# xinntao/EDVR

Hardware: AMD Instinct MI355X
Metric: EDVR-L x4 5-frame 720p clips/sec (higher is better)
Workload: dtype fp32 emulated as 2xf16 (hi+lo, 22-bit operands, 4 cross products), fp32 accumulate; 1 GPU; EDVR-L x4, 5 frames, 180x320 LR -> 720x1280, batch 10/GPU, inference; clips_per_gpu=10, global_clips=10, parallelism=clip-sharded x1, no data-path collective, world_size=1, backend=single process

## Files before the change

edvr_amd/_lib.py:

```python
import ctypes
import os

_HERE = os.path.dirname(os.path.abspath(__file__))
LIB_PATH = os.environ.get('EDVR_AMD_LIB') or os.path.join(_HERE, 'lib', 'libedvr_amd.so')

c_float_p = ctypes.c_void_p
i32, i64, f32, sz, u32 = ctypes.c_int, ctypes.c_int64, ctypes.c_float, ctypes.c_size_t, ctypes.c_uint32
vp = ctypes.c_void_p


class ConvDesc(ctypes.Structure):
    _fields_ = [
        ('x1', vp), ('x2', vp), ('c1', i32), ('c2', i32), ('x1_img_stride', i64), ('x2_img_stride', i64),
        ('x2_div', i32), ('x2_mul', i32), ('x2_add', i32), ('n', i32), ('h', i32), ('w', i32), ('wpk', vp),
        ('bias', vp), ('co', i32), ('ks', i32), ('stride', i32), ('act', i32), ('act_from', i32), ('res1', vp),
        ('res2', vp), ('res1_img_stride', i64), ('res2_img_stride', i64), ('y', vp), ('y_img_stride', i64),
        ('out_mode', i32), ('algo', i32), ('gate', vp), ('gate_img_stride', i64), ('gate_slope', f32), ('y_scale', f32),
        ('wpk_f4', vp), ('abs_sum', vp), ('abs_sum_channels', i32), ('wpk_f4s', vp), ('x_amax', vp), ('y_amax', vp),
        ('pre', vp), ('pre_img_stride', i64), ('pre_div', i32), ('pre_mul', i32), ('pre_add', i32), ('pre_n', i32), ('wpk_ds', vp),
    ]


PROTOTYPES = {
    'edvr_version': (ctypes.c_char_p, []),
    'edvr_last_error': (ctypes.c_char_p, []),
    'edvr_check_device': (i32, []),
    'edvr_conv2d_packed_weight_elems': (sz, [i32, i32, i32]),
    'edvr_conv2d_pack_weight_f32': (i32, [vp, vp, i32, i32, i32, i32, vp]),
    'edvr_conv2d_packed_weight_f4_elems': (sz, [i32, i32]),
    'edvr_conv2d_pack_weight_f4_f32': (i32, [vp, vp, i32, i32, i32, vp]),
    'edvr_conv2d_packed_weight_f4s_elems': (sz, [i32, i32]),
    'edvr_conv2d_pack_weight_f4s_f32': (i32, [vp, vp, i32, i32, i32, vp]),
    'edvr_conv2d_packed_weight_1x1s_elems': (sz, [i32, i32]),
    'edvr_conv2d_pack_weight_1x1s_f32': (i32, [vp, vp, i32, i32, vp]),
    'edvr_conv2d_packed_weight_ds_elems': (sz, [i32, i32, i32]),
    'edvr_conv2d_pack_weight_ds_f32': (i32, [vp, vp, i32, i32, i32, vp]),
    'edvr_amax_f32': (i32, [vp, vp, i32, i64, i64, vp]),
    'edvr_pack_job_bytes': (sz, []),
    'edvr_conv2d_pack_weights_multi': (i32, [vp, i32, i32, i32, vp]),
    'edvr_conv2d_f32': (i32, [ctypes.POINTER(ConvDesc), vp]),
    'edvr_conv2d_kernel': (i32, [ctypes.POINTER(ConvDesc)]),
    'edvr_conv2d_gate_supported': (i32, [ctypes.POINTER(ConvDesc)]),
    'edvr_conv2d_abs_sum_supported': (i32, [ctypes.POINTER(ConvDesc)]),
    'edvr_conv2d_y_amax_supported': (i32, [ctypes.POINTER(ConvDesc)]),
    'edvr_conv2d_pre_supported': (i32, [ctypes.POINTER(ConvDesc)]),
    'edvr_conv2d_f4s_set_lean': (i32, [i32]),
    'edvr_conv2d_f4s_lean_items': (i32, [ctypes.POINTER(ConvDesc)]),
    'edvr_conv2d_kernel_name': (i32, [ctypes.POINTER(ConvDesc), ctypes.c_char_p, sz]),
    'edvr_conv2d_executed_flops': (i32, [ctypes.POINTER(ConvDesc), ctypes.POINTER(ctypes.c_double)]),
    'edvr_dcnv2_fwd_ws_bytes': (sz, [i32] * 12),
    'edvr_dcnv2_fwd_f32': (i32, [vp] * 6 + [i32] * 12 + [i64, i64, i32, i32, vp, sz, vp]),
    'edvr_dcnv2_fwd_split_f32': (i32, [vp] * 6 + [i32] * 12 + [i64, i64, i32, i32, vp, sz, vp, vp]),
    'edvr_dcnv2_fwd_split_applies': (i32, [vp] + [i32] * 13),
    'edvr_dcnv2_fwd_kernel_name': (i32, [vp] + [i32] * 13 + [ctypes.c_char_p, sz]),
    'edvr_dcnv2_bwd_ws_bytes': (sz, [i32] * 12),
    'edvr_dcnv2_any_ws_bytes': (sz, [i32] * 13),
    'edvr_dcnv2_fwd_any': (i32, [i32] + [vp] * 6 + [i32] * 12 + [i64, i64, vp, sz, vp]),
    'edvr_dcnv2_bwd_any': (i32, [i32] + [vp] * 10 + [i32] * 12 + [i64, i64, i64, i64, vp, sz, vp]),
    'edvr_psnr_sse_f32': (i32, [vp, vp, vp, i32, i32, i32, i32, i64, i64, i32, i32, i32, vp]),
    'edvr_ssim_partials': (sz, [i32, i32, i32]),
    'edvr_ssim_f32': (i32, [vp, vp, vp, i32, i32, i32, i32, i64, i64, i32, i32, vp]),
    'edvr_niqe_blocks': (sz, [i32, i32, i32]),
    'edvr_niqe_moments_f32': (i32, [vp, vp, i32, i32, i32, i32, i64, i32, vp]),
    'edvr_niqe_moments_u8': (i32, [vp, vp, i32, i32, i32, i64, i32, vp]),
    'edvr_frames_u8_to_f32': (i32, [vp, vp, i32, i32, i32, i32, vp, i32, vp]),
    'edvr_gather_images_f32': (i32, [vp, vp, vp, vp, i32, vp, i32, i32, vp]),
    'edvr_upsample4x_add_u8': (i32, [vp, vp, vp, i32, i32, i32, vp]),
    'edvr_f32_to_u8_hwc': (i32, [vp, vp, i32, i32, i32, i64, vp]),
    'edvr_crop_pad_frames_u8': (i32, [vp, vp, i32, i32, i32, i32, i32, i32, i32, i32, vp]),
    'edvr_crop_pad_frames_f32': (i32, [vp, vp, i32, i32, i32, i64, i32, i32, i32, i32, i32, vp]),
    'edvr_upsample4x_add_rect_f32': (i32, [vp, vp, vp, i32, i32, i32, i32, i32, i32, i32, i64, i64, i64, vp]),
    'edvr_upsample4x_add_rect_u8': (i32, [vp, vp, vp, i32, i32, i32, i32, i32, i32, i32, i64, i64, vp]),
    'edvr_f32_to_u8_hwc_rect': (i32, [vp, vp, i32, i32, i32, i64, i32, i32, i32, i32, i64, i64, vp]),
    'edvr_copy_rect_f32': (i32, [vp, vp, i32, i32, i32, i64, i32, i32, i32, i32, i64, i64, i64, vp]),
    'edvr_crop_pad_frames_d4_u8': (i32, [vp, vp, i32, i32, i32, i32, i32, i32, i32, i32, i32, vp]),
    'edvr_crop_pad_frames_d4_f32': (i32, [vp, vp, i32, i32, i32, i64, i32, i32, i32, i32, i32, i32, vp]),
    'edvr_upsample4x_add_rect_d4_f32': (i32, [vp, vp, vp, i32, i32, i32, i32, i32, i32, i32, i64, i64, i64, i32, i32, f32, vp]),
    'edvr_upsample4x_add_rect_d4_u8': (i32, [vp, vp, vp, vp, i32, i32, i32, i32, i32, i32, i32, i64, i64, i64, i64, i64, i32, i32, f32, vp]),
    'edvr_f32_to_u8_hwc_rect_d4': (i32, [vp, vp, vp, i32, i32, i32, i64, i32, i32, i32, i32, i64, i64, i64, i64, i64, i32, i32, f32, vp]),
    'edvr_copy_rect_d4_f32': (i32, [vp, vp, i32, i32, i32, i64, i32, i32, i32, i32, i64, i64, i64, i32, i32, f32, vp]),
    'edvr_upsample4x_add_rect_blend_f32': (i32, [vp, vp, vp, i32, i32, i32, i32, i32, i32, i32, i64, i64, i64, i32, i32, f32, i32, i32, i32, i32, vp]),
    'edvr_upsample4x_add_rect_blend_u8': (i32, [vp, vp, vp, vp, i32, i32, i32, i32, i32, i32, i32, i64, i64, i64, i64, i64, i32, i32, f32, i32, i32, i32, i32, vp]),
    'edvr_f32_to_u8_hwc_rect_blend': (i32, [vp, vp, vp, i32, i32, i32, i64, i32, i32, i32, i32, i64, i64, i64, i64, i64, i32, i32, f32, i32, i32, i32, i32, vp]),
    'edvr_copy_rect_blend_f32': (i32, [vp, vp, i32, i32, i32, i64, i32, i32, i32, i32, i64, i64, i64, i32, i32, f32, i32, i32, i32, i32, vp]),
    'edvr_imresize_bicubic_u8': (i32, [vp, vp, i32, i32, i32, i32, i32, ctypes.c_double, i32, i32, vp]),
    'edvr_imresize_bicubic_f32': (i32, [vp, vp, i32, i32, i32, i64, i32, i32, ctypes.c_double, i32, i32, vp]),
    'edvr_bd_downsample_u8': (i32, [vp, vp, i32, i32, i32, i32, i32, i32, i32, vp]),
    'edvr_bd_downsample_f32': (i32, [vp, vp, i32, i32, i32, i64, i32, i32, i32, i32, vp]),
    'edvr_imresize_bicubic_u8_windows': (i32, [vp, vp, vp, vp, i32, i32, i32, i32, i32, i32, vp]),
    'edvr_bd_downsample_u8_windows': (i32, [vp, vp, vp, vp, i32, i32, i32, i32, i32, i32, vp]),
    'edvr_yuv420_to_rgb_f32': (i32, [vp, vp, i32, i32, i32, i64, i64, vp, i32, vp]),
    'edvr_yuv420_to_rgb_u8': (i32, [vp, vp, i32, i32, i32, i64, vp, i32, vp]),
    'edvr_rgb_to_yuv420_f32': (i32, [vp, vp, i32, i32, i32, i64, i64, vp, vp]),
    'edvr_rgb_to_yuv420_u8': (i32, [vp, vp, i32, i32, i32, i64, vp, vp]),
    'edvr_yuv_to_rgb_f32': (i32, [vp, vp, i32, i32, i32, i32, i32, i32, i64, i64, vp, i32, vp]),
    'edvr_rgb_to_yuv_f32': (i32, [vp, vp, i32, i32, i32, i32, i32, i32, i64, i64, vp, vp]),
    'edvr_yuv_to_rgb_sited_f32': (i32, [vp, vp, i32, i32, i32, i32, i32, i32, i64, i64, vp, i32, i32, i32, vp]),
    'edvr_rgb_to_yuv_sited_f32': (i32, [vp, vp, i32, i32, i32, i32, i32, i32, i64, i64, vp, i32, i32, vp]),
    'edvr_yuv420_to_rgb_sited_u8': (i32, [vp, vp, i32, i32, i32, i64, vp, i32, i32, i32, vp]),
    'edvr_rgb_to_yuv420_sited_u8': (i32, [vp, vp, i32, i32, i32, i64, vp, i32, i32, vp]),
    'edvr_frame_sad_rgb_u8': (i32, [vp, vp, vp, i32, i32, i32, i64, vp]),
    'edvr_frame_sad_rgb_f32': (i32, [vp, vp, vp, i32, i32, i32, i64, vp]),
    'edvr_jpeg_roundtrip_u8': (i32, [vp, vp, vp, i32, i32, i32, i32, i64, i64, i32, vp]),
    'edvr_mpeg_roundtrip_workspace': (sz, [i32, i32, i32, i32]),
    'edvr_mpeg_roundtrip_u8': (i32, [vp, vp, vp, i32, i32, i32, i32, i32, i64, i64, i64, i64, i32, i32, vp, sz, vp]),
    'edvr_degrade_u8': (i32, [vp, vp, vp, vp, i32, i32, i32, i64, i64, vp]),
    'edvr_philox_words_u32': (i32, [vp, u32, u32, u32, i32, i32, vp]),
    'edvr_adam_chunk_bytes': (sz, []),
    'edvr_adam_multi_f32': (i32, [vp, i32, ctypes.c_float, ctypes.c_float, ctypes.c_float, vp]),
    'edvr_dcnv1_fwd_ws_bytes': (sz, [i32] * 12),
    'edvr_dcnv1_fwd_f32': (i32, [vp] * 4 + [i32] * 12 + [i64, i32, vp, sz, vp]),
    'edvr_dcnv1_bwd_ws_bytes': (sz, [i32] * 12),
    'edvr_dcnv1_bwd_f32': (i32, [vp] * 7 + [i32] * 12 + [i64, i64, i32, vp, sz, vp]),
    'edvr_dcnv2_bwd_f32': (i32, [vp] * 10 + [i32] * 12 + [i64, i64, i64, i64, i32, vp, sz, vp]),
    'edvr_dcnv2_bwd_split_f32': (i32, [vp] * 10 + [i32] * 12 + [i64, i64, i64, i64, i32, vp, sz, vp, vp, vp]),
    'edvr_dcnv2_bwd_split_applies': (i32, []),
    'edvr_tsa_temporal_f32': (i32, [vp] * 5 + [i32] * 4 + [vp]),
    'edvr_tsa_temporal_pair_f32': (i32, [vp] * 5 + [i32] * 4 + [vp]),
    'edvr_pool_maxavg_3x3s2_f32': (i32, [vp, vp, i32, i32, i32, i32, vp]),
    'edvr_upsample2x_f32': (i32, [vp, vp, i32, i32, i32, f32, vp]),
    'edvr_tsa_combine_f32': (i32, [vp, vp, vp, vp, i64, vp]),
    'edvr_upsample4x_add_f32': (i32, [vp, vp, i32, i32, i32, vp]),
    'edvr_add_f32': (i32, [vp, vp, vp, i64, vp]),
    'edvr_act_bwd_f32': (i32, [vp, vp, vp, vp, vp, i32, i32, i64, i32, i32, vp]),
    'edvr_conv2d_wgrad_ws_bytes': (sz, [i32] * 7),
    'edvr_conv2d_wgrad_algo': (i32, [i32]),
    'edvr_conv2d_wgrad_kernel_name': (i32, [i32] * 8 + [ctypes.c_char_p, sz]),
    'edvr_conv2d_wgrad_f32': (i32, [vp] * 4 + [i32] * 8 + [i64, i64, i32, i32, i32, i64, i32, vp, vp, sz, vp]),
    'edvr_conv2d_wgrad_split_f32': (i32, [vp] * 4 + [i32] * 8 + [i64, i64, i32, i32, i32, i64, i32, vp, vp, sz, vp, vp, vp]),
    'edvr_conv2d_wgrad_split_applies': (i32, [i32] * 8),
    'edvr_conv2d_wgrad_split_is_direct': (i32, [i32] * 2),
    'edvr_channel_sum_f32': (i32, [vp, vp, i32, i32, i64, i64, vp, sz, vp]),
    'edvr_pixel_unshuffle2_f32': (i32, [vp, vp, i32, i32, i32, i32, vp]),
    'edvr_pixel_unshuffle2_act_bwd_f32': (i32, [vp, vp, vp, i32, i32, i32, i32, i32, vp]),
    'edvr_zero_stuff2_f32': (i32, [vp, vp, i32, i32, i32, i32, i32, vp]),
    'edvr_frame_reduce_add_f32': (i32, [vp, vp, i32, i32, i32, i64, vp]),
    'edvr_upsample2x_bwd_f32': (i32, [vp, vp, i32, i32, i32, f32, vp]),
    'edvr_pool_maxavg_3x3s2_bwd_f32': (i32, [vp, vp, vp, i32, i32, i32, i32, vp]),
    'edvr_tsa_temporal_bwd_f32': (i32, [vp] * 7 + [i32] * 4 + [vp, vp]),
    'edvr_tsa_combine_bwd_f32': (i32, [vp] * 5 + [i64, vp]),
    'edvr_charbonnier_f32': (i32, [vp, vp, vp, vp, i64, f32, f32, vp]),
    'edvr_abs_sum_f32': (i32, [vp, vp, i32, i64, i64, vp]),
    'edvr_abs_stats_f32': (i32, [vp, vp, i32, i64, i32, i64, vp]),
}

ACT_NONE, ACT_RELU, ACT_LRELU, ACT_SIGMOID = 0, 1, 2, 3
OUT_NCHW, OUT_PIXEL_SHUFFLE2 = 0, 1
CONV_AUTO, CONV_DIRECT, CONV_WINOGRAD, CONV_WINOGRAD_F4, CONV_WINOGRAD_F4S = 0, 1, 2, 3, 4
(CONV_KERNEL_SMALL, CONV_KERNEL_F4S, CONV_KERNEL_F4, CONV_KERNEL_F2, CONV_KERNEL_1X1_SPLIT, CONV_KERNEL_1X1_STREAM,
 CONV_KERNEL_DIRECT_SPLIT, CONV_KERNEL_DIRECT) = range(8)
DTYPE_F32, DTYPE_F64, DTYPE_F16 = 0, 1, 2
DCN_HALO_TAPWIN = 16
JPEG_SUBSAMPLINGS = {'420': 420, '444': 444}
DEGRADE_TILE, DEGRADE_MAX_KSIZE, DEGRADE_RECORD_INTS, DEGRADE_GRAY = 64, 21, 8, 1

_lib = None


class ExtensionMissing(RuntimeError):
    pass


def lib():
    global _lib
    if _lib is None:
        if not os.path.exists(LIB_PATH):
            raise ExtensionMissing(
                f'{LIB_PATH} not found: the HIP extension is not built (run `python -m edvr_amd.build`). '
                'edvr_amd has no CPU/PyTorch fallback.')
        handle = ctypes.CDLL(LIB_PATH)
        for name, (res, args) in PROTOTYPES.items():
            fn = getattr(handle, name)
            fn.restype, fn.argtypes = res, args
        _lib = handle
    return _lib


def check(rc, what):
    if rc != 0:
        msg = lib().edvr_last_error().decode()
        raise RuntimeError(f'{what} failed (code {rc}): {msg}')
```

edvr_amd/build.py:

```python
import os
import shutil
import subprocess
import sys
from concurrent.futures import ThreadPoolExecutor

HERE = os.path.dirname(os.path.abspath(__file__))
CSRC = os.path.join(HERE, 'csrc')
LIBDIR = os.path.join(HERE, 'lib')
LIB = os.path.join(LIBDIR, 'libedvr_amd.so')
OBJDIR = os.path.join(HERE, 'build')
SOURCES = ['api.hip', 'pack.hip', 'conv2d.hip', 'conv2d_s.hip', 'dcn.hip', 'dcn_any.hip', 'elementwise.hip', 'wgrad.hip', 'backward.hip', 'dcn_fused.hip', 'dcn_tapwin.hip', 'dcn_tapwin_s.hip', 'dcn_bwd_fused.hip', 'winograd.hip', 'winograd_f4.hip', 'winograd_f4s.hip', 'winograd_wgrad.hip', 'winograd_wgrad_s.hip', 'wgrad_direct_s.hip', 'gemm_nt_s.hip', 'optim.hip', 'metrics.hip', 'conv_small.hip', 'conv1x1.hip', 'conv1x1_s.hip', 'data.hip', 'video.hip', 'resize.hip', 'bd.hip', 'ensemble.hip', 'yuv.hip', 'niqe.hip', 'shots.hip', 'jpeg.hip', 'degrade.hip', 'mpeg.hip']
LINK = []
FLAGS = ['--offload-arch=gfx950', '-O3', '-std=c++17', '-fPIC', '-munsafe-fp-atomics', '-ffp-contract=fast']


def _hipcc():
    exe = shutil.which('hipcc') or '/opt/rocm/bin/hipcc'
    if not os.path.exists(exe):
        raise RuntimeError('hipcc not found: the HIP extension cannot be built')
    return exe


def _deps():
    return [os.path.join(CSRC, 'common.h'), os.path.join(CSRC, 'pack.h'), os.path.join(CSRC, 'conv_launch.h'), os.path.join(CSRC, 'dcn_tap.h'), os.path.join(CSRC, 'pixel.h'), os.path.join(CSRC, 'lq_window.h'), os.path.join(CSRC, 'jpeg_dct.h'), os.path.join(HERE, '..', 'include', 'edvr_amd.h')]


def _stale(target, sources):
    if not os.path.exists(target):
        return True
    t = os.path.getmtime(target)
    return any(os.path.getmtime(s) > t for s in sources)


def source_hash():
    import hashlib
    h = hashlib.sha256()
    files = sorted(os.path.join(CSRC, f) for f in os.listdir(CSRC) if f.endswith(('.hip', '.h', '.inc')))
    for path in files + [os.path.join(HERE, '..', 'include', 'edvr_amd.h')]:
        h.update(os.path.basename(path).encode() + b'\0')
        h.update(open(path, 'rb').read())
    return h.hexdigest()[:16]


def build(force=False, verbose=False):
    os.makedirs(OBJDIR, exist_ok=True)
    os.makedirs(LIBDIR, exist_ok=True)
    hipcc = _hipcc()
    objs, jobs = [], []
    for src in SOURCES:
        s = os.path.join(CSRC, src)
        o = os.path.join(OBJDIR, src.replace('.hip', '.o'))
        objs.append(o)
        if force or _stale(o, [s] + _deps()):
            jobs.append([hipcc] + FLAGS + ['-c', s, '-o', o])

    def run(cmd):
        if verbose:
            print(' '.join(cmd), flush=True)
        r = subprocess.run(cmd, capture_output=True, text=True)
        if r.returncode != 0:
            raise RuntimeError('hipcc failed:\n' + ' '.join(cmd) + '\n' + r.stdout + r.stderr)

    with ThreadPoolExecutor(max_workers=max(1, min(len(jobs), os.cpu_count() or 1))) as ex:
        list(ex.map(run, jobs))
    if force or jobs or _stale(LIB, objs):
        run([hipcc, '--offload-arch=gfx950', '-shared', '-fPIC', '-o', LIB] + objs + LINK)
    return LIB


if __name__ == '__main__':
    print(build(force='--force' in sys.argv, verbose=True))
```

edvr_amd/csrc/common.h:

```cpp
#pragma once
#include <hip/hip_runtime.h>

#include <cstdarg>
#include <cstdio>

#include "../../include/edvr_amd.h"

namespace edvr {

void set_error(const char *fmt, ...);

inline int check_launch(const char *what) {
  hipError_t e = hipGetLastError();
  if (e != hipSuccess) {
    set_error("%s: %s", what, hipGetErrorString(e));
    return EDVR_ERR_LAUNCH;
  }
  return EDVR_OK;
}

inline hipStream_t as_stream(edvr_stream_t s) { return reinterpret_cast<hipStream_t>(s); }

inline int cdiv(int a, int b) { return (a + b - 1) / b; }
inline int64_t cdiv64(int64_t a, int64_t b) { return (a + b - 1) / b; }

int conv2d_launch(const edvr_conv2d_desc &d, hipStream_t stream);
enum conv_kernel {
  CONV_SMALL = EDVR_CONV_KERNEL_SMALL,
  CONV_F4S = EDVR_CONV_KERNEL_F4S,
  CONV_F4 = EDVR_CONV_KERNEL_F4,
  CONV_F2 = EDVR_CONV_KERNEL_F2,
  CONV_1X1_SPLIT = EDVR_CONV_KERNEL_1X1_SPLIT,
  CONV_1X1_STREAM = EDVR_CONV_KERNEL_1X1_STREAM,
  CONV_DIRECT_SPLIT = EDVR_CONV_KERNEL_DIRECT_SPLIT,
  CONV_DIRECT = EDVR_CONV_KERNEL_DIRECT,
};
conv_kernel conv2d_select(const edvr_conv2d_desc &d);

size_t gemm_nt_ws_elems(int M, int N, int64_t K);
int gemm_nt_launch(const float *A, const float *B, float *C, int M, int N, int64_t K, int64_t lda, int64_t ldb,
                   bool accumulate, float *ws, hipStream_t stream);
size_t gemm_nt_ws_elems_b(int M, int N, int64_t K, int nb);
int gemm_nt_batched(const float *A, const float *B, float *C, int M, int N, int64_t K, int64_t lda, int64_t ldb, int nb, int64_t a_bs,
                    int64_t b_bs, bool accumulate, float *ws, hipStream_t stream);
bool gemm_nt_split_enabled();
int gemm_nt_split_batched(const float *A, const float *B, float *C, int M, int N, int64_t K, int64_t lda, int64_t ldb, int nb, int64_t a_bs,
                          int64_t b_bs, bool accumulate, float *ws, const float *a_amax, const float *b_amax, hipStream_t stream);

bool winograd_eligible(const edvr_conv2d_desc &d);
int winograd_launch(const edvr_conv2d_desc &d, const float *U, int cop64, hipStream_t stream);
double winograd_executed_flops(const edvr_conv2d_desc &d);
int winograd_pack(const float *w, float *U, int co, int ci, int cop64, int cip, int transpose_flip, float *wpk_direct, int cop32,
                  hipStream_t stream);

bool winograd_f4_eligible(const edvr_conv2d_desc &d);
int winograd_f4_launch(const edvr_conv2d_desc &d, hipStream_t stream);
double winograd_f4_executed_flops(const edvr_conv2d_desc &d);

bool winograd_f4s_eligible(const edvr_conv2d_desc &d);
int winograd_f4s_launch(const edvr_conv2d_desc &d, hipStream_t stream);
double winograd_f4s_executed_flops(const edvr_conv2d_desc &d);

bool conv_small_eligible(const edvr_conv2d_desc &d);
int conv_small_launch(const edvr_conv2d_desc &d, hipStream_t stream);
bool wgrad_small_plan(int n, int c1, int c2, int h, int w, int co, int ks, int stride, int *splits);
size_t wgrad_small_ws_bytes(int co, int ci, int splits);
int wgrad_small_launch(const float *x, const float *dz, float *ws, int ci, int co, int n, int h, int w, int64_t x_img_stride,
                       int64_t dz_img_stride, int splits, hipStream_t stream);

bool conv1x1_eligible(const edvr_conv2d_desc &d);
int conv1x1_launch(const edvr_conv2d_desc &d, hipStream_t stream);
bool conv1x1_split_eligible(const edvr_conv2d_desc &d);
int conv1x1_split_launch(const edvr_conv2d_desc &d, hipStream_t stream);

bool conv2d_split_eligible(const edvr_conv2d_desc &d);
int conv2d_split_launch(const edvr_conv2d_desc &d, hipStream_t stream);
int conv_split_pack(const float *w, unsigned *wq, int co, int ci, int kk, int cop, int quads, hipStream_t stream);

int reduce_partials_launch(const float *ws, float *out, int64_t total, int parts, int accumulate, hipStream_t stream,
                           const float *ws2 = nullptr, float *out2 = nullptr, int total2 = 0, int parts2 = 0);

bool winograd_wgrad_plan(int n, int c1, int c2, int h, int w, int co, int ks, int stride, int *splits);
size_t winograd_wgrad_ws_bytes(int co, int ci, int splits);
int winograd_wgrad_set_algo(int algo);
int winograd_wgrad_get_algo();
int winograd_wgrad_launch(const float *x1, const float *x2, const float *dz, float *ws, int c1, int c2, int n, int h, int w, int co,
                          int64_t x1_img_stride, int64_t x2_img_stride, int x2_div, int x2_mul, int x2_add, int64_t dz_img_stride,
                          int splits, int want_db, hipStream_t stream);

bool winograd_wgrad_split_enabled();
int winograd_wgrad_split_launch(const float *x1, const float *x2, const float *dz, float *ws, int c1, int c2, int n, int h, int w, int co,
                                int64_t x1_img_stride, int64_t x2_img_stride, int x2_div, int x2_mul, int x2_add, int64_t dz_img_stride,
                                int splits, int want_db, const float *x_amax, const float *dz_amax, hipStream_t stream);

bool wgrad_direct_split_enabled();
bool wgrad_direct_split_supported(const float *x1, const float *x2, const float *dz, int h, int w, int64_t x1_img_stride, int64_t x2_img_stride,
                                  int64_t dz_img_stride);
int wgrad_direct_split_launch(const float *x1, const float *x2, const float *dz, float *ws, int c1, int c2, int n, int h, int w, int co,
                              int64_t x1_img_stride, int64_t x2_img_stride, int x2_div, int x2_mul, int x2_add, int64_t dz_img_stride,
                              int splits, int want_db, const float *x_amax, const float *dz_amax, hipStream_t stream);

struct DcnShape {
  int B, C, H, W, Co, kh, kw, stride, pad, dil, groups, dg, Ho, Wo;
  int stride_w, pad_w, dil_w;
  int64_t off_bs, msk_bs;
  int64_t doff_bs, dmsk_bs;
};
int dcn_fill_shape(DcnShape &s, int B, int C, int H, int W, int Co, int kh, int kw, int stride, int pad, int dil, int groups, int dg,
                   int64_t off_bs, int64_t msk_bs);

bool dcn_fused_supported(int C, int Co, int H, int W, int kh, int kw, int stride, int pad, int dil, int groups, int dg);
int dcn_fused_pack(const float *weight, float *wpk, int Co, int C, hipStream_t stream);
int dcn_fused_forward(const float *x, const float *offset, const float *mask, const float *wpk, const float *bias, float *y, int B, int C,
                      int H, int W, int Co, int dg, int64_t off_bs, int64_t msk_bs, int act, int halo, hipStream_t stream);

bool dcn_tapwin_supported(int C, int Co, int H, int W, int kh, int kw, int stride, int pad, int dil, int groups, int dg);
int dcn_tapwin_forward(const float *x, const float *offset, const float *mask, const float *wpk, const float *bias, float *y, int B, int C,
                       int H, int W, int Co, int dg, int64_t off_bs, int64_t msk_bs, int act, hipStream_t stream);

bool dcn_tapwin_split_enabled();
int dcn_tapwin_split_forward(const float *x, const float *offset, const float *mask, const float *weight, unsigned *wpk, const float *bias, float *y,
                             int B, int C, int H, int W, int Co, int dg, int64_t off_bs, int64_t msk_bs, int act, const float *xm_amax,
                             hipStream_t stream);

bool dcn_bwd_fused_supported(const DcnShape &s);
size_t dcn_bwd_fused_wbk_elems(int dg);
int dcn_bwd_fused_launch(const DcnShape &s, const float *x, const float *offset, const float *mask, const float *weight, const float *dy,
                         float *wbk, float *col, float *dx, float *doffset, float *dmask, hipStream_t stream);

__device__ inline int xcd_remap(int linear, int total) {
  const int q = total >> 3, rem = total & 7, xcd = linear & 7;
  return xcd * q + (xcd < rem ? xcd : rem) + (linear >> 3);
}
__device__ inline void xcd_block_index(int &bx, int &by, int &bz) {
  const int gx = gridDim.x, gy = gridDim.y;
  const int lin = blockIdx.x + gx * (blockIdx.y + gy * blockIdx.z);
  const int lg = xcd_remap(lin, gx * gy * (int)gridDim.z);
  bx = lg % gx;
  by = (lg / gx) % gy;
  bz = lg / (gx * gy);
}

}

#define EDVR_REQUIRE(cond, ...)       \
  do {                                \
    if (!(cond)) {                    \
      ::edvr::set_error(__VA_ARGS__); \
      return EDVR_ERR_ARG;            \
    }                                 \
  } while (0)
```

edvr_amd/csrc/dcn.hip:

```cpp
#include <cstdlib>

#include "common.h"
#include "dcn_tap.h"

namespace edvr {

typedef float f32x16 __attribute__((ext_vector_type(16)));

__global__ void fill_kernel(float *__restrict__ p, float v, int64_t n) {
  for (int64_t i = (int64_t)blockIdx.x * blockDim.x + threadIdx.x; i < n; i += (int64_t)gridDim.x * blockDim.x) p[i] = v;
}

struct Merge {
  bool give01, give11;
  bool take00, take10;
};
__device__ __forceinline__ Merge merge_right(const Tap &t, bool same_plane_as_next) {
  Merge mg;
  const int lane = __lane_id();
  const int n_o00 = lane_next_i(t.o00), n_o10 = lane_next_i(t.o10);
  const int n_ok = lane_next_i((t.ok00 ? 1 : 0) | (t.ok10 ? 2 : 0));
  const bool has_next = lane < 63 && same_plane_as_next;
  mg.give01 = has_next && t.ok01 && (n_ok & 1) && n_o00 == t.o01;
  mg.give11 = has_next && t.ok11 && (n_ok & 2) && n_o10 == t.o11;
// ... 515 lines not shown
  EDVR_REQUIRE(s.Ho > 0 && s.Wo > 0, "dcnv2: convolution input is too small (output would be %dx%d)", s.Ho, s.Wo);
  const int64_t P = (int64_t)s.Ho * s.Wo, K = kh * kw;
  s.off_bs = off_bs ? off_bs : (int64_t)dg * 2 * K * P;
  s.msk_bs = msk_bs < 0 ? 0 : (msk_bs ? msk_bs : (int64_t)dg * K * P);
  s.doff_bs = (int64_t)dg * 2 * K * P;
  s.dmsk_bs = (int64_t)dg * K * P;
  return EDVR_OK;
}

static bool use_fused(const DcnShape &s) {
  const char *e = getenv("EDVR_DCN_FUSED");
  if (e && e[0] == '0') return false;
  if (s.stride != s.stride_w || s.pad != s.pad_w || s.dil != s.dil_w) return false;
  return dcn_fused_supported(s.C, s.Co, s.H, s.W, s.kh, s.kw, s.stride, s.pad, s.dil, s.groups, s.dg);
}

struct FwdWs { size_t col, wpk, total; };
static FwdWs fwd_ws(const DcnShape &s) {

  const size_t K = (size_t)s.kh * s.kw, P = (size_t)s.Ho * s.Wo;
  FwdWs w;
  w.col = 0;
  size_t off = align_up((size_t)s.B * s.C * K * P * 4, 256);
  w.wpk = off;
  size_t pk = edvr_conv2d_packed_weight_elems(s.Co / s.groups, (int)((s.C / s.groups) * K), 1) * 4 * s.groups;
  if (use_fused(s)) pk = std::max(pk, edvr_conv2d_packed_weight_elems(s.Co, s.C, 3) * 4);
  off += align_up(pk, 256);
  w.total = off;
  return w;
}

struct BwdWs { size_t col, wpk, gemm, total; };
static BwdWs bwd_ws(const DcnShape &s) {
  const size_t K = (size_t)s.kh * s.kw, P = (size_t)s.Ho * s.Wo;
  const int cig = s.C / s.groups, cog = s.Co / s.groups;
  BwdWs w;
  w.col = 0;
  size_t off = align_up((size_t)s.B * s.C * K * P * 4, 256);
  w.wpk = off;
  off += align_up(std::max(edvr_conv2d_packed_weight_elems((int)(cig * K), cog, 1) * s.groups, dcn_bwd_fused_wbk_elems(s.dg)) * 4, 256);
  w.gemm = off;
  off += align_up(std::max(gemm_nt_ws_elems_b(cog, (int)(cig * K), (int64_t)P, s.B), (size_t)s.B * s.Co * cig * K) * 4, 256);
  w.total = off;
  return w;
}

}

extern "C" {

size_t edvr_dcnv2_fwd_ws_bytes(int B, int C, int H, int W, int Co, int kh, int kw, int stride, int pad, int dil, int groups,
                               int dg) {
  edvr::DcnShape s;
  if (edvr::dcn_fill_shape(s, B, C, H, W, Co, kh, kw, stride, pad, dil, groups, dg, 0, 0)) return 0;
  return edvr::fwd_ws(s).total;
}

size_t edvr_dcnv2_bwd_ws_bytes(int B, int C, int H, int W, int Co, int kh, int kw, int stride, int pad, int dil, int groups,
                               int dg) {
  edvr::DcnShape s;
  if (edvr::dcn_fill_shape(s, B, C, H, W, Co, kh, kw, stride, pad, dil, groups, dg, 0, 0)) return 0;
  return edvr::bwd_ws(s).total;
}

static int dcnv2_fwd_impl(const float *x, const float *offset, const float *mask, const float *weight, const float *bias,
                          float *y, int B, int C, int H, int W, int Co, int kh, int kw, int stride, int pad, int dil, int groups,
                          int dg, int64_t offset_bstride, int64_t mask_bstride, int act, int halo_hint, void *ws, size_t ws_bytes,
                          const float *xm_amax, edvr_stream_t stream_) {
  using namespace edvr;
  EDVR_REQUIRE(x && offset && mask && weight && y, "dcnv2_fwd: null pointer");
  DcnShape s;
  int rc = dcn_fill_shape(s, B, C, H, W, Co, kh, kw, stride, pad, dil, groups, dg, offset_bstride, mask_bstride);
  if (rc) return rc;
  const FwdWs wsz = fwd_ws(s);
  if (!ws || ws_bytes < wsz.total) {
    set_error("dcnv2_fwd: workspace %zu < required %zu", ws_bytes, wsz.total);
    return EDVR_ERR_WORKSPACE;
  }
  hipStream_t stream = as_stream(stream_);
  const int K = kh * kw;
  const int64_t P = (int64_t)s.Ho * s.Wo;
  float *col = reinterpret_cast<float *>(static_cast<char *>(ws) + wsz.col);
  float *wpk = reinterpret_cast<float *>(static_cast<char *>(ws) + wsz.wpk);
  if (use_fused(s) && halo_hint == EDVR_DCN_HALO_TAPWIN && xm_amax && dcn_tapwin_split_enabled() &&
      dcn_tapwin_supported(C, Co, H, W, kh, kw, s.stride, s.pad, s.dil, groups, dg) && (reinterpret_cast<uintptr_t>(x) & 15) == 0)
    return dcn_tapwin_split_forward(x, offset, mask, weight, reinterpret_cast<unsigned *>(wpk), bias, y, B, C, H, W, Co, dg, s.off_bs, s.msk_bs, act,
                                    xm_amax, stream);
  if (use_fused(s) && halo_hint >= 0) {
    rc = dcn_fused_pack(weight, wpk, Co, C, stream);
    if (rc) return rc;
    if (halo_hint == EDVR_DCN_HALO_TAPWIN) {
      if (dcn_tapwin_supported(C, Co, H, W, kh, kw, s.stride, s.pad, s.dil, groups, dg) && (reinterpret_cast<uintptr_t>(x) & 15) == 0)
        return dcn_tapwin_forward(x, offset, mask, wpk, bias, y, B, C, H, W, Co, dg, s.off_bs, s.msk_bs, act, stream);
      halo_hint = 7;
    }
    return dcn_fused_forward(x, offset, mask, wpk, bias, y, B, C, H, W, Co, dg, s.off_bs, s.msk_bs, act, halo_hint, stream);
  }
  const int cig = C / groups, cog = Co / groups;
  const size_t wpk_g = edvr_conv2d_packed_weight_elems(cog, cig * K, 1);
  for (int g = 0; g < groups; ++g) {
    rc = edvr_conv2d_pack_weight_f32(weight + (size_t)g * cog * cig * K, wpk + g * wpk_g, cog, cig * K, 1, 0, stream_);
    if (rc) return rc;
  }
  const int64_t total = (int64_t)B * dg * K * P;
  hipLaunchKernelGGL(dcn_im2col_kernel, dim3((unsigned)std::min<int64_t>(cdiv64(total, 256), 1 << 20)), dim3(256), 0, stream, x,
                     offset, mask, col, s);
  rc = check_launch("dcn_im2col_kernel");
  if (rc) return rc;
  for (int g = 0; g < groups; ++g) {
    edvr_conv2d_desc d = {};
    d.x1 = col + (int64_t)g * cig * K * P;
    d.c1 = cig * K;
    d.x1_img_stride = (int64_t)C * K * P;
    d.n = B; d.h = s.Ho; d.w = s.Wo;
    d.wpk = wpk + g * wpk_g;
    d.bias = bias ? bias + g * cog : nullptr;
    d.co = cog; d.ks = 1; d.stride = 1;
    d.act = act;
    d.y = y + (int64_t)g * cog * P;
    d.y_img_stride = (int64_t)Co * P;
    d.out_mode = EDVR_OUT_NCHW;
    rc = conv2d_launch(d, stream);
    if (rc) return rc;
  }
  return EDVR_OK;
}

int edvr_dcnv2_fwd_f32(const float *x, const float *offset, const float *mask, const float *weight, const float *bias,
                       float *y, int B, int C, int H, int W, int Co, int kh, int kw, int stride, int pad, int dil, int groups,
                       int dg, int64_t offset_bstride, int64_t mask_bstride, int act, int halo_hint, void *ws, size_t ws_bytes,
                       edvr_stream_t stream) {
  return dcnv2_fwd_impl(x, offset, mask, weight, bias, y, B, C, H, W, Co, kh, kw, stride, pad, dil, groups, dg, offset_bstride, mask_bstride, act,
                        halo_hint, ws, ws_bytes, nullptr, stream);
}

int edvr_dcnv2_fwd_split_f32(const float *x, const float *offset, const float *mask, const float *weight, const float *bias,
                             float *y, int B, int C, int H, int W, int Co, int kh, int kw, int stride, int pad, int dil, int groups,
                             int dg, int64_t offset_bstride, int64_t mask_bstride, int act, int halo_hint, void *ws, size_t ws_bytes,
                             const float *xm_amax, edvr_stream_t stream) {
  EDVR_REQUIRE(xm_amax != nullptr, "dcnv2_fwd_split: null magnitude bound");
  return dcnv2_fwd_impl(x, offset, mask, weight, bias, y, B, C, H, W, Co, kh, kw, stride, pad, dil, groups, dg, offset_bstride, mask_bstride, act,
                        halo_hint, ws, ws_bytes, xm_amax, stream);
}

int edvr_dcnv2_fwd_split_applies(const float *x, int B, int C, int H, int W, int Co, int kh, int kw, int stride, int pad, int dil, int groups,
                                 int dg, int halo_hint) {
  using namespace edvr;
  DcnShape s;
  if (dcn_fill_shape(s, B, C, H, W, Co, kh, kw, stride, pad, dil, groups, dg, 0, 0)) return 0;
  return (use_fused(s) && halo_hint == EDVR_DCN_HALO_TAPWIN && dcn_tapwin_split_enabled() &&
          dcn_tapwin_supported(C, Co, H, W, kh, kw, s.stride, s.pad, s.dil, groups, dg) && (reinterpret_cast<uintptr_t>(x) & 15) == 0) ? 1 : 0;
}

int edvr_dcnv2_fwd_kernel_name(const float *x, int B, int C, int H, int W, int Co, int kh, int kw, int stride, int pad, int dil, int groups,
                               int dg, int halo_hint, char *buf, size_t buf_len) {
  using namespace edvr;
  EDVR_REQUIRE(buf && buf_len > 0, "dcnv2_fwd_kernel_name: null buffer");
  DcnShape s;
  int rc = dcn_fill_shape(s, B, C, H, W, Co, kh, kw, stride, pad, dil, groups, dg, 0, 0);
  if (rc) return rc;
  const char *name = "dcn_im2col_kernel";
  if (use_fused(s) && halo_hint >= 0) {
    const bool tapwin = halo_hint == EDVR_DCN_HALO_TAPWIN && dcn_tapwin_supported(C, Co, H, W, kh, kw, s.stride, s.pad, s.dil, groups, dg) &&
                        (reinterpret_cast<uintptr_t>(x) & 15) == 0;
    name = tapwin ? "dcn_tapwin_fwd_kernel" : "dcn_fused_fwd_kernel";
  }
  snprintf(buf, buf_len, "%s", name);
  return EDVR_OK;
}

static int dcnv2_bwd_impl(const float *x, const float *offset, const float *mask, const float *weight, const float *dy, float *dx,
                          float *doffset, float *dmask, float *dweight, float *dbias, int B, int C, int H, int W, int Co, int kh,
                          int kw, int stride, int pad, int dil, int groups, int dg, int64_t offset_bstride, int64_t mask_bstride,
                          int64_t doffset_bstride, int64_t dmask_bstride, int scatter_hint, void *ws, size_t ws_bytes,
                          const float *xm_amax, const float *dy_amax, edvr_stream_t stream_) {
  using namespace edvr;
  EDVR_REQUIRE(x && offset && mask && weight && dy && dx && doffset && dmask && dweight, "dcnv2_bwd: null pointer");
  DcnShape s;
  int rc = dcn_fill_shape(s, B, C, H, W, Co, kh, kw, stride, pad, dil, groups, dg, offset_bstride, mask_bstride);
  if (rc) return rc;
  if (doffset_bstride) s.doff_bs = doffset_bstride;
  if (dmask_bstride) s.dmsk_bs = dmask_bstride < 0 ? 0 : dmask_bstride;
  const BwdWs wsz = bwd_ws(s);
  if (!ws || ws_bytes < wsz.total) {
    set_error("dcnv2_bwd: workspace %zu < required %zu", ws_bytes, wsz.total);
    return EDVR_ERR_WORKSPACE;
  }
  hipStream_t stream = as_stream(stream_);
  const int K = kh * kw;
  const int64_t P = (int64_t)s.Ho * s.Wo;
  float *col = reinterpret_cast<float *>(static_cast<char *>(ws) + wsz.col);
  float *wpk = reinterpret_cast<float *>(static_cast<char *>(ws) + wsz.wpk);
  float *gws = reinterpret_cast<float *>(static_cast<char *>(ws) + wsz.gemm);
  const int cig = C / groups, cog = Co / groups;
  if (scatter_hint == EDVR_DCN_SCATTER_STRIP && dcn_bwd_fused_supported(s)) {
    if (hipMemsetAsync(dx, 0, (size_t)B * C * H * W * sizeof(float), stream) != hipSuccess) {
      set_error("dcnv2_bwd: hipMemsetAsync failed");
      return EDVR_ERR_LAUNCH;
    }
    rc = dcn_bwd_fused_launch(s, x, offset, mask, weight, dy, wpk, col, dx, doffset, dmask, stream);
    if (rc) return rc;
  } else {
    const size_t wpk_g = edvr_conv2d_packed_weight_elems(cig * K, cog, 1);
    for (int g = 0; g < groups; ++g) {
      const float *wg = weight + (size_t)g * cog * cig * K;
      const float *wuse = wg;
      if ((cog % 32) != 0 || ((cig * K) % 32) != 0) {
        rc = edvr_conv2d_pack_weight_f32(wg, wpk + g * wpk_g, cig * K, cog, 1, 1, stream_);
        if (rc) return rc;
        wuse = wpk + g * wpk_g;
      }
      edvr_conv2d_desc d = {};
      d.x1 = dy + (int64_t)g * cog * P;
      d.c1 = cog;
      d.x1_img_stride = (int64_t)Co * P;
      d.n = B; d.h = s.Ho; d.w = s.Wo;
      d.wpk = wuse;
      d.co = cig * K; d.ks = 1; d.stride = 1;
      d.y = col + (int64_t)g * cig * K * P;
      d.y_img_stride = (int64_t)C * K * P;
      rc = conv2d_launch(d, stream);
      if (rc) return rc;
    }
    if (hipMemsetAsync(dx, 0, (size_t)B * C * H * W * sizeof(float), stream) != hipSuccess) {
      set_error("dcnv2_bwd: hipMemsetAsync failed");
      return EDVR_ERR_LAUNCH;
    }
    static const bool use_tile = []() {
      const char *e = getenv("EDVR_DCN_BWD_TILE");
      return !(e && e[0] == '0');
    }();
    const bool edvr_sig = kh == 3 && kw == 3 && s.stride == 1 && s.pad == 1 && s.dil == 1 && s.stride_w == 1 && s.pad_w == 1 && s.dil_w == 1;
    if (scatter_hint == EDVR_DCN_SCATTER_STRIP && edvr_sig && dg * cdiv(W, 64) <= 65535) {
      hipLaunchKernelGGL(dcn_bwd_dx_strip_kernel, dim3(dg * cdiv(W, 64), B), dim3(256), 0, stream, offset, mask, col, dx, s);
      const int64_t total = (int64_t)B * dg * K * P;
      hipLaunchKernelGGL(dcn_bwd_coord_kernel<false>, dim3((unsigned)std::min<int64_t>(cdiv64(total, 256), 1 << 20)), dim3(256), 0, stream,
                         x, offset, mask, col, static_cast<float *>(nullptr), doffset, dmask, s);
      rc = check_launch("dcn_bwd_dx_strip_kernel + dcn_bwd_coord_kernel");
    } else if (use_tile && scatter_hint != EDVR_DCN_SCATTER_DEVICE && scatter_hint != EDVR_DCN_SCATTER_STRIP && edvr_sig && C / dg <= 16) {
      const int tiles_x = cdiv(s.Wo, 32), tiles_y = cdiv(s.Ho, 8);
      if (scatter_hint == EDVR_DCN_SCATTER_LDS_WIDE)
        hipLaunchKernelGGL((dcn_bwd_coord_tile_kernel<6>), dim3(tiles_x * tiles_y, dg, B), dim3(256), 0, stream, x, offset, mask, col, dx, doffset, dmask, s, tiles_x);
      else
        hipLaunchKernelGGL((dcn_bwd_coord_tile_kernel<3>), dim3(tiles_x * tiles_y, dg, B), dim3(256), 0, stream, x, offset, mask, col, dx, doffset, dmask, s, tiles_x);
      rc = check_launch("dcn_bwd_coord_tile_kernel");
    } else {
      const int64_t total = (int64_t)B * dg * K * P;
      hipLaunchKernelGGL(dcn_bwd_coord_kernel<true>, dim3((unsigned)std::min<int64_t>(cdiv64(total, 256), 1 << 20)), dim3(256), 0, stream, x,
                         offset, mask, col, dx, doffset, dmask, s);
      rc = check_launch("dcn_bwd_coord_kernel");
    }
    if (rc) return rc;
  }
  for (int g = 0; g < groups; ++g) {
    rc = (xm_amax && dy_amax && gemm_nt_split_enabled())
             ? gemm_nt_split_batched(dy + (int64_t)g * cog * P, col + (int64_t)g * cig * K * P, dweight + (size_t)g * cog * cig * K, cog, cig * K,
                                     P, P, P, B, (int64_t)Co * P, (int64_t)C * K * P, false, gws, dy_amax, xm_amax, stream)
             : gemm_nt_batched(dy + (int64_t)g * cog * P, col + (int64_t)g * cig * K * P, dweight + (size_t)g * cog * cig * K, cog, cig * K, P,
                               P, P, B, (int64_t)Co * P, (int64_t)C * K * P, false, gws, stream);
    if (rc) return rc;
  }
  if (dbias) {
    rc = edvr_channel_sum_f32(dy, dbias, B, Co, P, (int64_t)Co * P, gws, (size_t)64 * Co * sizeof(float), stream_);
    if (rc) return rc;
  }
  return EDVR_OK;
}

int edvr_dcnv2_bwd_f32(const float *x, const float *offset, const float *mask, const float *weight, const float *dy, float *dx,
                       float *doffset, float *dmask, float *dweight, float *dbias, int B, int C, int H, int W, int Co, int kh,
                       int kw, int stride, int pad, int dil, int groups, int dg, int64_t offset_bstride, int64_t mask_bstride,
                       int64_t doffset_bstride, int64_t dmask_bstride, int scatter_hint, void *ws, size_t ws_bytes,
                       edvr_stream_t stream) {
  return dcnv2_bwd_impl(x, offset, mask, weight, dy, dx, doffset, dmask, dweight, dbias, B, C, H, W, Co, kh, kw, stride, pad, dil, groups, dg,
                        offset_bstride, mask_bstride, doffset_bstride, dmask_bstride, scatter_hint, ws, ws_bytes, nullptr, nullptr, stream);
}

int edvr_dcnv2_bwd_split_f32(const float *x, const float *offset, const float *mask, const float *weight, const float *dy, float *dx,
                             float *doffset, float *dmask, float *dweight, float *dbias, int B, int C, int H, int W, int Co, int kh,
                             int kw, int stride, int pad, int dil, int groups, int dg, int64_t offset_bstride, int64_t mask_bstride,
                             int64_t doffset_bstride, int64_t dmask_bstride, int scatter_hint, void *ws, size_t ws_bytes,
                             const float *xm_amax, const float *dy_amax, edvr_stream_t stream) {
  EDVR_REQUIRE(xm_amax && dy_amax, "dcnv2_bwd_split: null magnitude bound");
  return dcnv2_bwd_impl(x, offset, mask, weight, dy, dx, doffset, dmask, dweight, dbias, B, C, H, W, Co, kh, kw, stride, pad, dil, groups, dg,
                        offset_bstride, mask_bstride, doffset_bstride, dmask_bstride, scatter_hint, ws, ws_bytes, xm_amax, dy_amax, stream);
}

int edvr_dcnv2_bwd_split_applies(void) { return edvr::gemm_nt_split_enabled() ? 1 : 0; }


size_t edvr_dcnv1_fwd_ws_bytes(int B, int C, int H, int W, int Co, int kh, int kw, int stride, int pad, int dil, int groups, int dg) {
  edvr::DcnShape s;
  if (edvr::dcn_fill_shape(s, B, C, H, W, Co, kh, kw, stride, pad, dil, groups, dg, 0, 0)) return 0;
  return edvr::fwd_ws(s).total + edvr::align_up((size_t)dg * kh * kw * s.Ho * s.Wo * 4, 256);
}

int edvr_dcnv1_fwd_f32(const float *x, const float *offset, const float *weight, float *y, int B, int C, int H, int W, int Co, int kh,
                       int kw, int stride, int pad, int dil, int groups, int dg, int64_t offset_bstride, int halo_hint, void *ws,
                       size_t ws_bytes, edvr_stream_t stream_) {
  using namespace edvr;
  const size_t v2 = edvr_dcnv2_fwd_ws_bytes(B, C, H, W, Co, kh, kw, stride, pad, dil, groups, dg);
  const size_t need = edvr_dcnv1_fwd_ws_bytes(B, C, H, W, Co, kh, kw, stride, pad, dil, groups, dg);
  EDVR_REQUIRE(v2 && need, "dcnv1: bad shape");
  if (!ws || ws_bytes < need) {
    set_error("dcnv1_fwd: workspace %zu < required %zu", ws_bytes, need);
    return EDVR_ERR_WORKSPACE;
// ... 41 lines not shown
```

edvr_amd/csrc/dcn_tapwin_s.hip:

```cpp
#include <type_traits>

#include "common.h"
#include <cstdlib>

#include "dcn_tap.h"
#include "pack.h"

namespace edvr {

typedef float f32x16 __attribute__((ext_vector_type(16)));
typedef float f32x4 __attribute__((ext_vector_type(4)));
typedef float f32x2 __attribute__((ext_vector_type(2)));

namespace {
constexpr int TWS_TH = 8, TWS_TW = 32, TWS_RY = 2, TWS_RX = 2;
constexpr int TWS_IH = TWS_TH + 2 * TWS_RY;
constexpr int TWS_IW = (TWS_TW + 2 * TWS_RX + 3 + 3) / 4 * 4;
constexpr int TWS_PPR = TWS_IW / 4;
constexpr int TWS_HR = TWS_IH / 2;
constexpr int TWS_HB = TWS_HR * TWS_IW;
constexpr int TWS_CHS = TWS_IH * TWS_IW;
static_assert(TWS_HR * TWS_PPR <= 64 && TWS_IH == 2 * TWS_HR && TWS_CHS % 64 == 32, "window halves must fit one wave instruction");
constexpr int TWS_MAX_DG = 8;
constexpr int TWS_OOB = (int)0x80000000;
// ... 287 lines not shown
        for (int s = 0; s < 2; ++s)
#pragma unroll
          for (int m = 0; m < MT; ++m)
            acc[s][m] = __builtin_amdgcn_mfma_f32_32x32x16_f16(__builtin_bit_cast(f16x8, aw[m]), __builtin_bit_cast(f16x8, bq[s]), acc[s][m], 0, 0, 0);
        if (kg == 0 || KG == 1) {
          state_half(nxt, 0, tn, ny0, nx0, tnv);
#pragma unroll
          for (int i = 0; i < 4; ++i) asm volatile("" : "+v"(nxt.bw[0][i]));
          asm volatile("" : "+v"(nxt.addr[0]), "+v"(nxt.slow));
        }
        if (kg == KG - 1) {
          state_half(nxt, 1, tn, ny0, nx0, tnv);
#pragma unroll
          for (int i = 0; i < 4; ++i) asm volatile("" : "+v"(nxt.bw[1][i]));
          asm volatile("" : "+v"(nxt.addr[1]), "+v"(nxt.slow));
          state_any(nxt);
          asm volatile("" : "+s"(nxt.slow_any));
        }
#pragma unroll
        for (int s = 0; s < 2; ++s)
          asm volatile("v_alignbit_b32 %0, %0, %0, 16\n\tv_alignbit_b32 %1, %1, %1, 16\n\tv_alignbit_b32 %2, %2, %2, 16\n\tv_alignbit_b32 %3, %3, %3, 16"
                       : "+v"(bq[s][0]), "+v"(bq[s][1]), "+v"(bq[s][2]), "+v"(bq[s][3]));
#pragma unroll
        for (int s = 0; s < 2; ++s)
#pragma unroll
          for (int m = 0; m < MT; ++m)
            acc[s][m] = __builtin_amdgcn_mfma_f32_32x32x16_f16(__builtin_bit_cast(f16x8, aw[m]), __builtin_bit_cast(f16x8, bq[s]), acc[s][m], 0, 0, 0);
        __builtin_amdgcn_sched_barrier(0);
      }
    }
  };

  __syncthreads();
  const int n_steps = a.dg * KK;
  St cur, nxt;
  float tnv[6];
  int o1y, o1x;
  origin(0, 0, o1y, o1x);
  dma_x(0, 0, o1y, o1x);
  dma_w(0, 0, 0);
  dma_taps(0, 0);
  asm volatile("s_waitcnt vmcnt(0)" ::: "memory");
  read_taps(tnv);
  make_state(cur, 0, o1y, o1x, tnv);
  asm volatile("s_waitcnt lgkmcnt(0)" ::: "memory");
  int g = 0, t = 0, g1 = 0, t1 = 1;
  if (n_steps > 1) {
    origin(g1, t1, o1y, o1x);
    dma_taps(g1, t1);
    asm volatile("s_waitcnt vmcnt(0)" ::: "memory");
  }
  for (int k = 0; k < n_steps; ++k) {
    __syncthreads();
    const int g2 = (t1 == KK - 1) ? g1 + 1 : g1, t2 = (t1 == KK - 1) ? 0 : t1 + 1;
    int o2y = 0, o2x = 0;
    if (k + 1 < n_steps) {
      read_taps(tnv);
      asm volatile("s_waitcnt lgkmcnt(0)" ::: "memory");
      dma_x((k + 1) & 1, g1, o1y, o1x);
      dma_w((k + 1) & 1, g1, t1);
      if (k + 2 < n_steps) {
        origin(g2, t2, o2y, o2x);
        dma_taps(g2, t2);
      }
    }
    const float *xb = xw + (k & 1) * XW;
    const unsigned *wb = wsl + (k & 1) * WS;
    run_step(std::false_type{}, cur, xb, wb, g, t, nxt, t1, o1y, o1x, tnv);
    if (cur.slow_any) run_step(std::true_type{}, cur, xb, wb, g, t, nxt, t1, o1y, o1x, tnv);
    asm volatile("s_waitcnt vmcnt(0)" ::: "memory");
    cur = nxt;
    g = g1; t = t1; g1 = g2; t1 = t2; o1y = o2y; o1x = o2x;
  }

  const __amdgpu_buffer_rsrc_t y_rsrc = tws_rsrc(a.y + (int64_t)img * a.Co * P, a.Co * P * 4);
  const __amdgpu_buffer_rsrc_t b_rsrc = tws_rsrc(a.bias ? a.bias : a.x, a.bias ? a.Co * 4 : 0);
#pragma unroll
  for (int m = 0; m < MT; ++m) {
#pragma unroll
    for (int r4 = 0; r4 < 4; ++r4) {
      const int cob = co_blk + m * 32 + 8 * r4;
      float bias4[4];
#pragma unroll
      for (int r = 0; r < 4; ++r) {
        const bool cok = cob + 4 * half + r < a.Co;
        bias4[r] = a.bias ? __builtin_bit_cast(float, __builtin_amdgcn_raw_buffer_load_b32(b_rsrc, cok ? (4 * half + r) * 4 : OOB, cob * 4, 0)) : 0.f;
      }
#pragma unroll
      for (int s = 0; s < 2; ++s) {
        const bool pix_ok = s ? ok1 : ok0;
        const int pv = (p0 + s * a.W + 4 * half * P) * 4;
#pragma unroll
        for (int r = 0; r < 4; ++r) {
          float v = __builtin_fmaf(acc[s][m][4 * r4 + r], unscale, bias4[r]);
          if (a.act == EDVR_ACT_LRELU) v = v > 0.f ? v : 0.1f * v;
          else if (a.act == EDVR_ACT_RELU) v = fmaxf(v, 0.f);
          else if (a.act == EDVR_ACT_SIGMOID) v = __builtin_amdgcn_rcpf(1.f + __expf(-v));
          const bool cok = cob + 4 * half + r < a.Co;
          __builtin_amdgcn_raw_buffer_store_b32(__builtin_bit_cast(unsigned, v), y_rsrc, (pix_ok && cok) ? pv : OOB, (cob + r) * P * 4, 0);
        }
      }
    }
  }
}

__global__ __launch_bounds__(1024) void dcn_tapwin_split_scale_kernel(const float *__restrict__ w, unsigned *__restrict__ wpk, int64_t total) {
  __shared__ float red[16];
  float m = 0.f;
  for (int64_t i = threadIdx.x; i < total; i += 1024) m = fmaxf(m, fabsf(w[i]));
#pragma unroll
  for (int sh = 32; sh > 0; sh >>= 1) m = fmaxf(m, __shfl_xor(m, sh));
  if ((threadIdx.x & 63) == 0) red[threadIdx.x >> 6] = m;
  __syncthreads();
  if (threadIdx.x == 0) {
    for (int i = 1; i < 16; ++i) m = fmaxf(m, red[i]);
    const unsigned field = f4s_weight_scale_field(__builtin_bit_cast(unsigned, m));
    wpk[0] = field << 23;
    wpk[1] = (254u - field) << 23;
    for (int i = 2; i < 16; ++i) wpk[i] = 0u;
  }
}

__global__ void dcn_tapwin_split_pack_kernel(const float *__restrict__ w, unsigned *__restrict__ wpk, int Co, int C, int cop) {
  const float s_w = __builtin_bit_cast(float, wpk[0]);
  const int64_t total = (int64_t)(C / 4) * 9 * cop;
  const int full = Co / 128, rem_tiles = (Co - full * 128 + 31) / 32;
  for (int64_t i = (int64_t)blockIdx.x * blockDim.x + threadIdx.x; i < total; i += (int64_t)gridDim.x * blockDim.x) {
    const int pos = (int)(i % cop), t = (int)((i / cop) % 9), c4 = (int)(i / ((int64_t)cop * 9));
    const int blk = pos / 128 < full ? pos / 128 : full, start = blk * 128, mt = blk < full ? 4 : rem_tiles;
    const int r = pos - start, co = pos;
    const bool live = mt > 0 && r < 32 * mt && co < Co;
#pragma unroll
    for (int q = 0; q < 4; ++q) wpk[16 + i * 4 + q] = live ? split_f16x2(w[((int64_t)co * C + 8 * (c4 >> 1) + 2 * q + (c4 & 1)) * 9 + t], s_w) : 0u;
  }
}

template <int MT>
static int launch_tapwin_s(DcnTapwinSArgs a, int co_start, int co_blocks, hipStream_t stream) {
  a.co_start = co_start;
  dim3 grid(a.tiles_x * a.tiles_y, co_blocks, a.B);
  if (a.C / a.dg == 16) hipLaunchKernelGGL((dcn_tapwin_split_fwd_kernel<MT, 16>), grid, dim3(256), 0, stream, a);
  else hipLaunchKernelGGL((dcn_tapwin_split_fwd_kernel<MT, 8>), grid, dim3(256), 0, stream, a);
  return check_launch("dcn_tapwin_split_fwd_kernel");
}

bool dcn_tapwin_split_enabled() {
  static const bool on = []() {
    const char *e = getenv("EDVR_DCN_SPLIT");
    return !(e && e[0] == '0');
  }();
  return on;
}

int dcn_tapwin_split_forward(const float *x, const float *offset, const float *mask, const float *weight, unsigned *wpk, const float *bias, float *y,
                             int B, int C, int H, int W, int Co, int dg, int64_t off_bs, int64_t msk_bs, int act, const float *xm_amax,
                             hipStream_t stream) {
  EDVR_REQUIRE(B <= 65535, "dcn_tapwin_split: batch %d exceeds grid.z", B);
  EDVR_REQUIRE((reinterpret_cast<uintptr_t>(x) & 15) == 0 && (reinterpret_cast<uintptr_t>(wpk) & 15) == 0, "dcn_tapwin_split: x / wpk must be 16-byte aligned");
  const int cop = (Co + 31) / 32 * 32;
  hipLaunchKernelGGL(dcn_tapwin_split_scale_kernel, dim3(1), dim3(1024), 0, stream, weight, wpk, (int64_t)Co * C * 9);
  const int64_t total = (int64_t)(C / 4) * 9 * cop;
  hipLaunchKernelGGL(dcn_tapwin_split_pack_kernel, dim3((unsigned)std::min<int64_t>(cdiv64(total, 256), 2048)), dim3(256), 0, stream, weight, wpk, Co, C, cop);
  DcnTapwinSArgs a;
  a.xm_amax = xm_amax;
  a.x = x; a.offset = offset; a.mask = mask; a.wpk = wpk; a.bias = bias; a.y = y;
  a.B = B; a.C = C; a.H = H; a.W = W; a.Co = Co; a.dg = dg; a.act = act;
  a.cop = cop;
  a.off_bs = off_bs; a.msk_bs = msk_bs;
  a.tiles_x = cdiv(W, TWS_TW);
  a.tiles_y = cdiv(H, TWS_TH);
  a.co_start = 0;
  const int full = Co / 128, rem_tiles = cdiv(Co - full * 128, 32);
  int rc = EDVR_OK;
  if (full > 0) rc = launch_tapwin_s<4>(a, 0, full, stream);
  if (rc || rem_tiles == 0) return rc;
  switch (rem_tiles) {
    case 1: return launch_tapwin_s<1>(a, full * 128, 1, stream);
    case 2: return launch_tapwin_s<2>(a, full * 128, 1, stream);
    case 3: return launch_tapwin_s<3>(a, full * 128, 1, stream);
    default: return launch_tapwin_s<4>(a, full * 128, 1, stream);
  }
}

}
```

edvr_amd/edvr_arch.py:

```python
import torch
from torch import nn

from . import functional as F_
from .arch_util import DCNv2Pack, ResidualBlockNoBN, make_layer, warn_offset_absmean

LRELU = F_.ACT_LRELU


def _conv3(cin, cout, stride=1):
    return nn.Conv2d(cin, cout, 3, stride, 1)


class PCDAlignment(nn.Module):

    def __init__(self, num_feat=64, deformable_groups=8):
        super().__init__()
        self.offset_conv1, self.offset_conv2, self.offset_conv3 = nn.ModuleDict(), nn.ModuleDict(), nn.ModuleDict()
        self.dcn_pack, self.feat_conv = nn.ModuleDict(), nn.ModuleDict()
        for lv in (3, 2, 1):
            key = f'l{lv}'
            self.offset_conv1[key] = _conv3(2 * num_feat, num_feat)
            if lv == 3:
                self.offset_conv2[key] = _conv3(num_feat, num_feat)
            else:
                self.offset_conv2[key] = _conv3(2 * num_feat, num_feat)
                self.offset_conv3[key] = _conv3(num_feat, num_feat)
            self.dcn_pack[key] = DCNv2Pack(num_feat, num_feat, 3, padding=1, deformable_groups=deformable_groups)
            if lv < 3:
                self.feat_conv[key] = _conv3(2 * num_feat, num_feat)
        self.cas_offset_conv1 = _conv3(2 * num_feat, num_feat)
        self.cas_offset_conv2 = _conv3(num_feat, num_feat)
        self.cas_dcnpack = DCNv2Pack(num_feat, num_feat, 3, padding=1, deformable_groups=deformable_groups)
        self.upsample = nn.Upsample(scale_factor=2, mode='bilinear', align_corners=False)
        self.lrelu = nn.LeakyReLU(negative_slope=0.1, inplace=True)

    def dcn_modules(self):
        return [self.dcn_pack['l3'], self.dcn_pack['l2'], self.dcn_pack['l1'], self.cas_dcnpack]

    def align(self, nbr, ref, ref_map=None):
        up_off = up_feat = feat = None
        for lv in (3, 2, 1):
            key, x = f'l{lv}', nbr[lv - 1]
            off = F_.conv_shared_x2(self.offset_conv1[key], x, ref[lv - 1], ref_map, act=LRELU)
            if lv == 3:
                off = F_.conv(self.offset_conv2[key], off, act=LRELU)
            else:
                off = F_.conv(self.offset_conv2[key], off, x2=up_off, act=LRELU)
                off = F_.conv(self.offset_conv3[key], off, act=LRELU)
            feat = self.dcn_pack[key](x, off, act=LRELU if lv == 3 else F_.ACT_NONE)
            if lv < 3:
                feat = F_.conv(self.feat_conv[key], feat, x2=up_feat, act=LRELU if lv > 1 else F_.ACT_NONE)
            if lv > 1:
                up_off = F_.upsample2x(off, 2.0)
                up_feat = F_.upsample2x(feat)
        off = F_.conv_shared_x2(self.cas_offset_conv1, feat, ref[0], ref_map, act=LRELU)
        off = F_.conv(self.cas_offset_conv2, off, act=LRELU)
        return self.cas_dcnpack(feat, off, act=LRELU)

    def forward(self, nbr_feat_l, ref_feat_l):
        return self.align(nbr_feat_l, ref_feat_l)


class TSAFusion(nn.Module):

    def __init__(self, num_feat=64, num_frame=5, center_frame_idx=2):
        super().__init__()
        self.center_frame_idx = center_frame_idx
        self.temporal_attn1 = _conv3(num_feat, num_feat)
        self.temporal_attn2 = _conv3(num_feat, num_feat)
        self.feat_fusion = nn.Conv2d(num_frame * num_feat, num_feat, 1, 1)
        self.max_pool = nn.MaxPool2d(3, stride=2, padding=1)
        self.avg_pool = nn.AvgPool2d(3, stride=2, padding=1)
        self.spatial_attn1 = nn.Conv2d(num_frame * num_feat, num_feat, 1)
        self.spatial_attn2 = nn.Conv2d(num_feat * 2, num_feat, 1)
        self.spatial_attn3 = _conv3(num_feat, num_feat)
        self.spatial_attn4 = nn.Conv2d(num_feat, num_feat, 1)
        self.spatial_attn5 = _conv3(num_feat, num_feat)
        self.spatial_attn_l1 = nn.Conv2d(num_feat, num_feat, 1)
        self.spatial_attn_l2 = _conv3(num_feat * 2, num_feat)
        self.spatial_attn_l3 = _conv3(num_feat, num_feat)
        self.spatial_attn_add1 = nn.Conv2d(num_feat, num_feat, 1)
        self.spatial_attn_add2 = nn.Conv2d(num_feat, num_feat, 1)
        self.lrelu = nn.LeakyReLU(negative_slope=0.1, inplace=True)
        self.upsample = nn.Upsample(scale_factor=2, mode='bilinear', align_corners=False)

    def forward(self, aligned_feat):
        return self.spatial(self.temporal(aligned_feat))

    def temporal(self, aligned_feat, pair=False):
        b, t, c, h, w = aligned_feat.shape
        alias = F_.ops.carry_bound
        emb_ref = F_.conv(self.temporal_attn1, alias(aligned_feat[:, self.center_frame_idx], aligned_feat))
        emb = F_.conv(self.temporal_attn2, alias(aligned_feat.reshape(b * t, c, h, w), aligned_feat)).view(b, t, -1, h, w)
        if pair:
            mod, mod_rev = F_.tsa_temporal_pair(emb, emb_ref, aligned_feat)
            return alias(mod.view(b, t * c, h, w), mod), alias(mod_rev.view(b, t * c, h, w), mod_rev)
        mod = F_.tsa_temporal(emb, emb_ref, aligned_feat)
        return alias(mod.view(b, t * c, h, w), mod)

    def spatial(self, mod):
        feat = F_.conv(self.feat_fusion, mod, act=LRELU)
        attn = F_.conv(self.spatial_attn1, mod, act=LRELU)
        attn = F_.conv(self.spatial_attn2, F_.pool_maxavg(attn), act=LRELU)
        lvl = F_.conv(self.spatial_attn_l1, attn, act=LRELU)
        lvl = F_.conv(self.spatial_attn_l2, F_.pool_maxavg(lvl), act=LRELU)
        lvl = F_.upsample2x(F_.conv(self.spatial_attn_l3, lvl, act=LRELU))
        attn = F_.conv(self.spatial_attn3, attn, act=LRELU, res1=lvl)
        attn = F_.upsample2x(F_.conv(self.spatial_attn4, attn, act=LRELU))
        attn = F_.conv(self.spatial_attn5, attn)
        attn_add = F_.conv(self.spatial_attn_add2, F_.conv(self.spatial_attn_add1, attn, act=LRELU))
        return F_.tsa_combine(feat, attn, attn_add)


class PredeblurModule(nn.Module):

    def __init__(self, num_in_ch=3, num_feat=64, hr_in=False):
        super().__init__()
        self.hr_in = hr_in
        self.conv_first = _conv3(num_in_ch, num_feat)
        if hr_in:
            self.stride_conv_hr1 = _conv3(num_feat, num_feat, 2)
            self.stride_conv_hr2 = _conv3(num_feat, num_feat, 2)
        self.stride_conv_l2 = _conv3(num_feat, num_feat, 2)
        self.stride_conv_l3 = _conv3(num_feat, num_feat, 2)
        self.resblock_l3 = ResidualBlockNoBN(num_feat=num_feat)
        self.resblock_l2_1 = ResidualBlockNoBN(num_feat=num_feat)
        self.resblock_l2_2 = ResidualBlockNoBN(num_feat=num_feat)
        self.resblock_l1 = nn.ModuleList([ResidualBlockNoBN(num_feat=num_feat) for _ in range(5)])
        self.upsample = nn.Upsample(scale_factor=2, mode='bilinear', align_corners=False)
        self.lrelu = nn.LeakyReLU(negative_slope=0.1, inplace=True)

    def forward(self, x):
        f1 = F_.conv(self.conv_first, x, act=LRELU)
        if self.hr_in:
            f1 = F_.conv(self.stride_conv_hr2, F_.conv(self.stride_conv_hr1, f1, act=LRELU), act=LRELU)
        f2 = F_.conv(self.stride_conv_l2, f1, act=LRELU)
        f3 = F_.conv(self.stride_conv_l3, f2, act=LRELU)
        f3 = F_.upsample2x(self.resblock_l3(f3))
        rb = self.resblock_l2_1
        f2 = F_.conv(rb.conv2, F_.conv(rb.conv1, f2, act=F_.ACT_RELU), res1=f2, res2=f3)
        f2 = F_.upsample2x(self.resblock_l2_2(f2))
        f1 = self.resblock_l1[0](f1)
        rb = self.resblock_l1[1]
        f1 = F_.conv(rb.conv2, F_.conv(rb.conv1, f1, act=F_.ACT_RELU), res1=f1, res2=f2)
        for i in range(2, 5):
            f1 = self.resblock_l1[i](f1)
        return f1


class EDVR(nn.Module):

    def __init__(self, num_in_ch=3, num_out_ch=3, num_feat=64, num_frame=5, deformable_groups=8, num_extract_block=5,
                 num_reconstruct_block=10, center_frame_idx=2, hr_in=False, with_predeblur=False, with_tsa=True):
        super().__init__()
        self.center_frame_idx = num_frame // 2 if center_frame_idx is None else center_frame_idx
        self.hr_in, self.with_predeblur, self.with_tsa = hr_in, with_predeblur, with_tsa
        if with_predeblur:
            self.predeblur = PredeblurModule(num_feat=num_feat, hr_in=hr_in)
            self.conv_1x1 = nn.Conv2d(num_feat, num_feat, 1, 1)
        else:
            self.conv_first = _conv3(num_in_ch, num_feat)
        self.feature_extraction = make_layer(ResidualBlockNoBN, num_extract_block, num_feat=num_feat)
        self.conv_l2_1 = _conv3(num_feat, num_feat, 2)
        self.conv_l2_2 = _conv3(num_feat, num_feat)
        self.conv_l3_1 = _conv3(num_feat, num_feat, 2)
        self.conv_l3_2 = _conv3(num_feat, num_feat)
        self.pcd_align = PCDAlignment(num_feat=num_feat, deformable_groups=deformable_groups)
        if with_tsa:
            self.fusion = TSAFusion(num_feat=num_feat, num_frame=num_frame, center_frame_idx=self.center_frame_idx)
        else:
            self.fusion = nn.Conv2d(num_frame * num_feat, num_feat, 1, 1)
        self.reconstruction = make_layer(ResidualBlockNoBN, num_reconstruct_block, num_feat=num_feat)
        self.upconv1 = _conv3(num_feat, num_feat * 4)
        self.upconv2 = _conv3(num_feat, 64 * 4)
        self.pixel_shuffle = nn.PixelShuffle(2)
        self.conv_hr = _conv3(64, 64)
        self.conv_last = _conv3(64, 3)
        self.lrelu = nn.LeakyReLU(negative_slope=0.1, inplace=True)
        self.taps = None
        self._conv_weights = None
        self._conv_meta = None
        self._captured_offset_stats = None

    _PENDING = __import__('weakref').WeakKeyDictionary()

    @property
    def _pending_offset_stats(self):
        q = EDVR._PENDING.get(self)
        if q is None:
            q = EDVR._PENDING[self] = []
        return q

    def train(self, mode=True):
        self.check_offsets(wait=True)
        return super().train(mode)

    def forward(self, x):
        b, t, c, h, w = x.shape
        if self.hr_in:
            assert h % 16 == 0 and w % 16 == 0, 'The height and width must be multiple of 16.'
        else:
            assert h % 4 == 0 and w % 4 == 0, 'The height and width must be multiple of 4.'
        x = x.contiguous()
        ctr = self.center_frame_idx
        self.check_offsets(wait=False)
        if x.is_cuda:
            F_.ops.split_guard_check(wait=False)
        if torch.is_grad_enabled() and x.is_cuda:
            if self._conv_weights is None:
                convs = [m for m in self.modules() if isinstance(m, nn.Conv2d)]
                self._conv_weights = [m.weight for m in convs]
                first = self.predeblur.conv_first if self.with_predeblur else self.conv_first
                self._conv_meta = [(m.stride[0] == 1, m is not first) for m in convs]
            F_.ops.prepack_conv_weights(self._conv_weights, self._conv_meta)
        pyr = self.extract_features(x.view(b * t, c, h, w))
        return self.restore_from_features(pyr, x[:, ctr], b, t)

    def extract_features(self, frames, out=None):
        if F_.ops.F4S_INFERENCE or F_.ops.F4S_TRAINING:
            F_.ops.input_bound(frames)
        o1, o2, o3 = out if out is not None else (None, None, None)
        blocks = list(self.feature_extraction) if out is not None else []
        head = None if blocks else o1
        if self.with_predeblur:
            f1 = F_.conv(self.conv_1x1, self.predeblur(frames), out=head)
        else:
            f1 = F_.conv(self.conv_first, frames, act=LRELU, out=head)
        if out is None:
            f1 = self.feature_extraction(f1)
        else:
            for i, blk in enumerate(blocks):
                f1 = blk(f1, out=o1 if i == len(blocks) - 1 else None)
        f2 = F_.conv(self.conv_l2_2, F_.conv(self.conv_l2_1, f1, act=LRELU), act=LRELU, out=o2)
        f3 = F_.conv(self.conv_l3_2, F_.conv(self.conv_l3_1, f2, act=LRELU), act=LRELU, out=o3)
        return [f1, f2, f3]

    def restore_from_features(self, pyr, x_center, b, t, out_dtype=torch.float32, out=None, keep=None, elem=None, accumulate='only', scale=1.0,
                              acc=None, bands=None):
        self._check_tail_args(out_dtype, out, keep, elem, accumulate, scale, acc, bands)
        operand, sink = self.align_windows(pyr, b, t)
        return self._restore_aligned(operand, x_center, b, t, out_dtype, out, keep, elem, accumulate, scale, acc, bands, sink)

    def align_windows(self, pyr, b, t, pair=False):
        f1, f2, f3 = pyr
        ctr = self.center_frame_idx
        h, w = f1.shape[2], f1.shape[3]
        if pair and 2 * ctr != t - 1:
            raise ValueError(f'align_windows(pair=True): the reversed clip keeps its centre only when it is the middle frame, got {ctr} of {t}')
        sink = []
        dcns = self.pcd_align.dcn_modules()
        for m in dcns:
            m.stats_sink = sink
        try:
            aligned = self.pcd_align.align([f1, f2, f3], [f1, f2, f3], ref_map=(t, t, ctr))
        finally:
            for m in dcns:
                m.stats_sink = None
        flat = aligned
        aligned = F_.ops.carry_bound(aligned.view(b, t, -1, h, w), aligned)
        if self.taps is not None:
            self.taps['aligned'] = aligned
        if self.with_tsa:
            operand = self.fusion.temporal(aligned, pair=pair)
            return (*operand, sink) if pair else (operand, sink)
        operand = F_.ops.carry_bound(aligned.view(b, -1, h, w), aligned)
        if not pair:
            return operand, sink
        if torch.is_grad_enabled():
            raise RuntimeError('align_windows(pair=True) has no backward: call it under torch.no_grad()')
        table = torch.arange(b * t, dtype=torch.int32, device=flat.device).view(b, t).flip(1).reshape(-1)
        rev = F_.ops.gather_images([flat], table)[0]
        return operand, F_.ops.carry_bound(rev.view(b, -1, h, w), rev), sink

    def restore_from_aligned(self, operand, x_center, b, t, out_dtype=torch.float32, out=None, keep=None, elem=None, accumulate='only', scale=1.0,
                             acc=None, bands=None, sink=None):
        self._check_tail_args(out_dtype, out, keep, elem, accumulate, scale, acc, bands)
        return self._restore_aligned(operand, x_center, b, t, out_dtype, out, keep, elem, accumulate, scale, acc, bands, sink)

    @staticmethod
    def _check_tail_args(out_dtype, out, keep, elem, accumulate, scale, acc, bands):
        if out_dtype not in (torch.float32, torch.uint8):
            raise ValueError(f'out_dtype must be torch.float32 or torch.uint8, got {out_dtype}')
        if out_dtype == torch.uint8 and torch.is_grad_enabled():
            raise RuntimeError('the uint8 output of EDVR.restore_from_features has no backward: call it under torch.no_grad()')
        if out is None and keep is not None:
            raise ValueError('keep= names a rectangle of the result to store into out=: it needs out')
        if out is not None and torch.is_grad_enabled():
            raise RuntimeError('EDVR.restore_from_features(out=) writes in place and has no backward: call it under torch.no_grad()')
        if elem is None and (accumulate != 'only' or scale != 1.0 or (acc is not None and bands is None)):
            raise ValueError('accumulate=, scale= and acc= belong to a self-ensemble element: they need elem')
        if (elem is not None or bands is not None) and (out is None or (out_dtype == torch.uint8) != (acc is not None)):
            raise ValueError('elem= and bands= store into out= (and, with uint8 output, accumulate in acc=)')

    def _restore_aligned(self, operand, x_center, b, t, out_dtype, out, keep, elem, accumulate, scale, acc, bands, sink):
        dst = out
        taps = self.taps
        feat = self.fusion.spatial(operand) if self.with_tsa else F_.conv(self.fusion, operand)
        if taps is not None:
            taps['fused'] = feat
        out = self.reconstruction(feat)
        if taps is not None:
            taps['trunk'] = out
        out = F_.conv(self.upconv1, out, act=LRELU, out_mode=F_.OUT_PIXEL_SHUFFLE2)
        out = F_.conv(self.upconv2, out, act=LRELU, out_mode=F_.OUT_PIXEL_SHUFFLE2)
        out = F_.conv(self.conv_hr, out, act=LRELU)
        if dst is not None:
            ky, kx = keep if keep is not None else (0, 0)
            if bands is not None:
                how = dict(bands=bands, elem=0 if elem is None else elem, mode=accumulate, scale=scale)
                if self.hr_in:
                    last = F_.conv(self.conv_last, out, res1=x_center)
                    out = (F_.ops.f32_to_u8_hwc_rect_blend(last, dst, acc, ky, kx, **how) if acc is not None
                           else F_.ops.copy_rect_blend(last, dst, ky, kx, **how))
                else:
                    last = F_.conv(self.conv_last, out)
                    out = (F_.ops.upsample4x_add_u8_rect_blend(last, x_center, dst, acc, ky, kx, **how) if acc is not None
                           else F_.ops.upsample4x_add_rect_blend(last, x_center, dst, ky, kx, **how))
            elif elem is not None:
                how = dict(elem=elem, mode=accumulate, scale=scale)
                if self.hr_in:
                    last = F_.conv(self.conv_last, out, res1=x_center)
                    out = F_.ops.f32_to_u8_hwc_rect_d4(last, dst, acc, ky, kx, **how) if acc is not None else F_.ops.copy_rect_d4(last, dst, ky, kx, **how)
                else:
                    last = F_.conv(self.conv_last, out)
                    out = (F_.ops.upsample4x_add_u8_rect_d4(last, x_center, dst, acc, ky, kx, **how) if acc is not None
                           else F_.ops.upsample4x_add_rect_d4(last, x_center, dst, ky, kx, **how))
            elif self.hr_in:
                tail = F_.ops.f32_to_u8_hwc_rect if out_dtype == torch.uint8 else F_.ops.copy_rect
                out = tail(F_.conv(self.conv_last, out, res1=x_center), dst, ky, kx)
            else:
                tail = F_.ops.upsample4x_add_u8_rect if out_dtype == torch.uint8 else F_.ops.upsample4x_add_rect
                out = tail(F_.conv(self.conv_last, out), x_center, dst, ky, kx)
        elif self.hr_in:
            out = F_.conv(self.conv_last, out, res1=x_center)
            if out_dtype == torch.uint8:
                out = F_.ops.f32_to_u8_hwc(out)
        elif out_dtype == torch.uint8:
            out = F_.ops.upsample4x_add_u8(F_.conv(self.conv_last, out), x_center)
        else:
            out = F_.upsample4x_add(F_.conv(self.conv_last, out), x_center)
        if sink:
            self._queue_offset_check(sink, b, t)
        F_.ops.split_guard_submit(operand.device)
        return out

    def _queue_offset_check(self, sink, b, t):
        if not sink:
            return
        import torch
        sums = torch.stack([e[0] for e in sink]).view(len(sink), 2, b, t).sum(2)
        recs = [(per_img * b, module) for _, per_img, module in sink]
        if torch.cuda.is_current_stream_capturing():
            self._captured_offset_stats = (sums, recs)
            return
        if torch.is_grad_enabled() and F_.ops.HINT_WAIT:
            self._examine_offsets(sums.cpu(), recs)
            return
        host = torch.empty(sums.shape, dtype=sums.dtype, pin_memory=True)
        host.copy_(sums, non_blocking=True)
        done = torch.cuda.Event()
        done.record()
        self._pending_offset_stats.append((host, done, recs))
        if len(self._pending_offset_stats) > 64:
            self.check_offsets(wait=True)

    def check_offsets(self, wait=True):
        while self._pending_offset_stats:
            host, done, recs = self._pending_offset_stats[0]
            if wait:
                done.synchronize()
            elif not done.query():
                return
            self._pending_offset_stats.pop(0)
            self._examine_offsets(host, recs)

    @staticmethod
    def _examine_offsets(sums, recs):
        for li, (count, module) in enumerate(recs):
            per_frame = (sums[li, 0] / count).tolist()
            module.last_offset_absmean = sum(per_frame) / len(per_frame)
            rough = float(sums[li, 1].sum())
            module.last_offset_rough = rough / (0.75 * count * len(per_frame)) if rough >= 0 else None
            for v in per_frame:
                warn_offset_absmean(v)
```

edvr_amd/functional.py:

```python
import math
import os

import torch

from . import ops
from .ops import ACT_LRELU, ACT_NONE, ACT_RELU, ACT_SIGMOID, OUT_NCHW, OUT_PIXEL_SHUFFLE2


def _conv_geometry(m):
    ks, st = m.kernel_size, m.stride
    if (ks[0] != ks[1] or ks[0] not in (1, 3) or st[0] != st[1] or st[0] not in (1, 2) or (ks[0] == 1 and st[0] != 1)
            or tuple(m.padding) != (ks[0] // 2, ks[0] // 2) or tuple(m.dilation) != (1, 1) or m.groups != 1):
        raise NotImplementedError(
            f'edvr_amd conv kernel supports 3x3 (stride 1/2, pad 1) and 1x1 convolutions, dilation 1, groups 1; got {m}')
    return ks[0], st[0]


def _needs_grad(*ts):
    return torch.is_grad_enabled() and any(t is not None and t.requires_grad for t in ts)


def conv(m, x, *, x2=None, x2_map=None, act=ACT_NONE, act_from=0, res1=None, res2=None, out_mode=OUT_NCHW, y_scale=1.0,
         abs_sum_channels=0, ci_range=None, use_bias=True, pre=None, pre_map=None, out=None):
    ks, stride = _conv_geometry(m)
    if x.dim() != 4:
        raise ValueError(f'expected a 4-D input, got {tuple(x.shape)}')
    cin = x.shape[1] + (x2.shape[1] if x2 is not None else 0)
    want = m.in_channels if ci_range is None else ci_range[1] - ci_range[0]
    if cin != want:
        raise RuntimeError(f'expected {want} input channels, got {cin}')
    ops.require_gpu(x, x2, m.weight)
    if _needs_grad(x, x2, m.weight, m.bias, res1, res2, pre):
        from . import autograd as ag
        assert abs_sum_channels == 0
        if ci_range is not None or not use_bias or pre is not None or out is not None:
            raise NotImplementedError('ci_range / use_bias / pre / out are inference-only arguments of conv()')
        return ag.conv(m, x, x2, x2_map, act, act_from, res1, res2, out_mode, ks, stride, y_scale)
    wpk = ops.pack_conv_weight(m.weight, ci_range=ci_range)
    f4 = ops.F4_INFERENCE and ks == 3 and stride == 1 and cin >= 32 and m.out_channels >= 48
    f4s = f4 and ops.F4S_INFERENCE and x.shape[3] % 4 == 0
    wf4 = ops.pack_conv_weight(m.weight, f4=True, ci_range=ci_range) if (f4 and not f4s) else None
    wf4s = ops.pack_conv_weight(m.weight, f4s=True, ci_range=ci_range) if f4s else None
    if ops.F4S_INFERENCE and ks == 1 and stride == 1 and cin >= 320 and x.shape[1] % 8 == 0 and cin % 8 == 0:
        wf4s = ops.pack_conv_weight(m.weight, f4s=True, ci_range=ci_range)
    wds = None
    if ops.F4S_INFERENCE and m.out_channels > 4 and (x2 is None or x.shape[1] % 4 == 0) and (
            (ks == 3 and (stride == 2 or cin <= 8)) or (ks == 1 and cin < 320)):
        wds = ops.pack_conv_weight(m.weight, ds=True, ci_range=ci_range)
    bias = m.bias.detach() if (m.bias is not None and use_bias) else None
    r = ops.conv2d(x, wpk, bias, m.out_channels, ks, x2=x2, x2_map=x2_map, stride=stride, act=act, act_from=act_from,
                   res1=res1, res2=res2, out_mode=out_mode, y_scale=y_scale, wpk_f4=wf4, abs_sum_channels=abs_sum_channels,
                   wpk_f4s=wf4s, pre=pre, pre_map=pre_map, out=out, wpk_ds=wds)
    y = r[0] if abs_sum_channels > 0 else r
    if ops.F4S_INFERENCE and ops.get_bound(y) is None:
        ops.linear_bound(y, m.weight, m.bias, (x, x2), (res1, res2, pre), scale=y_scale, floor=1.0 if act == ACT_SIGMOID else 0.0)
    return r


PRE_SPLIT = os.environ.get('EDVR_CONV_PRE', '1') != '0'
PRE_SPLIT_MIN_ITEMS = None


def _conv_items(n, h, w, co):
    return n * -(-co // 64) * min(-(-w // 64) * -(-h // 8), -(-w // 32) * -(-h // 16))


def conv_shared_x2(m, x, x2, x2_map, act=ACT_NONE):
    if PRE_SPLIT and x2_map is not None and x2_map[0] > 1 and not _needs_grad(x, x2, m.weight, m.bias):
        ks, stride = _conv_geometry(m)
        (n, c1, h, w), c2, co = x.shape, x2.shape[1], m.out_channels
        f4 = ops.F4_INFERENCE and ks == 3 and stride == 1 and min(c1, c2) >= 32 and co >= 48
        min_items = PRE_SPLIT_MIN_ITEMS if PRE_SPLIT_MIN_ITEMS is not None else torch.cuda.get_device_properties(x.device).multi_processor_count
        if f4 and _conv_items(n, h, w, co) > min_items and ops.conv_pre_supported(n, c1, h, w, co, ops.F4S_INFERENCE and w % 4 == 0):
            div, mul, add = x2_map
            shared = (n - 1) // div + 1
            sel = x2[add:add + 1] if (mul == 0 or shared == 1) else x2[add:add + (shared - 1) * mul + 1:mul]
            p = conv(m, ops.carry_bound(sel, x2), ci_range=(c1, c1 + c2), use_bias=False)
            return conv(m, x, act=act, ci_range=(0, c1), pre=p, pre_map=(div, 0 if sel.shape[0] == 1 else 1, 0))
    return conv(m, x, x2=x2, x2_map=x2_map, act=act)


def offset_mask_conv_stats(conv_offset, feat):
    co = conv_offset.out_channels
    if _needs_grad(feat, conv_offset.weight, conv_offset.bias):
        om = offset_mask_conv(conv_offset, feat)
        return om, ops.abs_stats_per_image(om.detach()[:, :2 * co // 3])
    return conv(conv_offset, feat, act=ACT_SIGMOID, act_from=2 * co // 3, abs_sum_channels=2 * co // 3)


def offset_mask_conv(conv_offset, feat):
    co = conv_offset.out_channels
    return conv(conv_offset, feat, act=ACT_SIGMOID, act_from=2 * co // 3)


def tapwin_takes(x, m):
    c, w, dg = x.shape[1], x.shape[3], m.deformable_groups
    return (w % 4 == 0 and w >= 32 and dg <= 8 and c % dg == 0 and c // dg in (8, 16) and tuple(m.kernel_size) == (3, 3)
            and _one(m.stride) == 1 and _one(m.padding) == 1 and _one(m.dilation) == 1 and m.groups == 1)


def _one(v):
    return v if isinstance(v, int) else (v[0] if v[0] == v[1] else -1)


def halo_hint_from_stats(absmean, rough, tapwin_ok=True):
    if absmean is not None and not math.isfinite(absmean):
        absmean = None
    if rough is not None and not math.isfinite(rough):
        rough = None
    if not tapwin_ok:
        return 3 if (absmean is None or absmean < 1.2) else (7 if absmean < 3.0 else -1)
    if absmean is None:
        return ops.DCN_HALO_TAPWIN
    if rough is None:
        return 3 if absmean < 1.2 else (7 if absmean < 3.0 else -1)
    if rough >= 0.85 and absmean < 2.0:
        return 7
    if rough >= 40.0 and absmean >= 30.0:
        return -1
    return ops.DCN_HALO_TAPWIN


def halo_hint_from_absmean(absmean):
    return halo_hint_from_stats(absmean, None)


def scatter_hint_from_stats(absmean, rough):
    if absmean is None:
        return ops.DCN_SCATTER_LDS
    if absmean >= 4.0:
        return ops.DCN_SCATTER_LDS_WIDE
    if absmean < 0.4:
        return ops.DCN_SCATTER_STRIP
    if rough is not None and rough < 0.45:
        return ops.DCN_SCATTER_STRIP if absmean < 0.6 else ops.DCN_SCATTER_LDS
    return ops.DCN_SCATTER_DEVICE if absmean < 0.75 else ops.DCN_SCATTER_LDS


def scatter_hint_from_absmean(absmean):
    return scatter_hint_from_stats(absmean, None)


def dcn_from_packed(m, x, om, act=ACT_NONE):
    cfg = (m.stride, m.padding, m.dilation, m.groups, m.deformable_groups)
    hint = halo_hint_from_stats(getattr(m, 'last_offset_absmean', None), getattr(m, 'last_offset_rough', None), tapwin_takes(x, m))
    if _needs_grad(x, om, m.weight, m.bias):
        from . import autograd as ag
        return ag.DcnFromPackedFn.apply(x, om, m.weight, m.bias, (*cfg, act, hint, m))
    split = 2 * om.shape[1] // 3
    bias = m.bias.detach() if m.bias is not None else None
    xb = ops.input_bound(x) if (ops.F4S_INFERENCE and hint == ops.DCN_HALO_TAPWIN and tapwin_takes(x, m)) else None
    y = ops.dcnv2_forward(x, om[:, :split], om[:, split:], m.weight.detach(), bias, *cfg, act=act, halo_hint=hint, xm_bound=xb)
    if ops.F4S_INFERENCE:
        ops.linear_bound(y, m.weight, m.bias, (x,))
    return y


def upsample2x(x, scale=1.0):
    if _needs_grad(x):
        from . import autograd as ag
        return ag.Upsample2x.apply(x, scale)
    return ops.upsample2x(x, scale)


def pool_maxavg(x):
    if _needs_grad(x):
        from . import autograd as ag
        return ag.PoolMaxAvg.apply(x)
    return ops.pool_maxavg(x)


def tsa_temporal(emb, emb_ref, aligned):
    if _needs_grad(emb, emb_ref, aligned):
        from . import autograd as ag
        return ag.TsaTemporal.apply(emb, emb_ref, aligned)
    return ops.tsa_temporal(emb, emb_ref, aligned)


def tsa_temporal_pair(emb, emb_ref, aligned):
    if torch.is_grad_enabled():
        raise RuntimeError('tsa_temporal_pair has no backward: call it under torch.no_grad()')
    return ops.tsa_temporal_pair(emb, emb_ref, aligned)


def tsa_combine(feat, attn, attn_add):
    if _needs_grad(feat, attn, attn_add):
        from . import autograd as ag
        return ag.TsaCombine.apply(feat, attn, attn_add)
    return ops.tsa_combine(feat, attn, attn_add)


def add(a, b):
    if _needs_grad(a, b):
        from . import autograd as ag
        return ag.Add.apply(a, b)
    return ops.add(a, b)


def upsample4x_add(y, base):
    if _needs_grad(y, base):
        from . import autograd as ag
        return ag.Upsample4xAdd.apply(y, base)
    return ops.upsample4x_add_(y, base)
```

edvr_amd/ops.py:

```python
import ctypes
import os
import weakref

import torch

from . import _lib
from ._lib import (ACT_LRELU, ACT_NONE, ACT_RELU, ACT_SIGMOID, CONV_AUTO, CONV_DIRECT, CONV_WINOGRAD, CONV_WINOGRAD_F4, CONV_WINOGRAD_F4S, OUT_NCHW,
                   OUT_PIXEL_SHUFFLE2)


def _stream():
    return ctypes.c_void_p(torch.cuda.current_stream().cuda_stream)


def _ptr(t):
    return ctypes.c_void_p(t.data_ptr()) if t is not None else ctypes.c_void_p(0)


def require_gpu(*tensors, dtypes=(torch.float32,)):
    seen = None
    for t in tensors:
        if t is None:
            continue
        if not t.is_cuda:
            raise NotImplementedError('edvr_amd ops run on the GPU only (HIP/gfx950); got a CPU tensor')
        if t.dtype not in dtypes:
            raise NotImplementedError(f'edvr_amd: {t.dtype} is not supported here (supported: {", ".join(map(str, dtypes))})')
        if seen is not None and t.dtype != seen:
            raise RuntimeError(f'expected every tensor of the call to be {seen}, got {t.dtype}')
        seen = t.dtype
    return seen


DCN_DTYPES = {torch.float32: _lib.DTYPE_F32, torch.float64: _lib.DTYPE_F64, torch.float16: _lib.DTYPE_F16}


def _plane_contig(t):
    n, c, h, w = t.shape
    return t.stride(3) == 1 and t.stride(2) == w and t.stride(1) == h * w and (n == 1 or t.stride(0) >= c * h * w)


def _as_planes(t):
    return t if _plane_contig(t) else t.contiguous()


def _img_stride(t):
    return t.stride(0) if t.shape[0] > 1 else t.shape[1] * t.shape[2] * t.shape[3]


def _run(name, launch, flops=0.0, nbytes=0.0, executed=None):
    if LAUNCH_HOOK is not None:
        LAUNCH_HOOK(name, float(flops), launch, float(nbytes), executed)
    else:
        launch()


def _nb(*ts):
    return 4.0 * sum(t.numel() for t in ts if t is not None)


_WS = {}


def workspace(nbytes, device, tag=None):
    key = (device.index, torch.cuda.current_stream(device).cuda_stream) if tag is None else (device.index, torch.cuda.current_stream(device).cuda_stream, tag)
    buf = _WS.get(key)
    if buf is None or buf.numel() < nbytes:
        buf = None
        _WS.pop(key, None)
        buf = torch.empty(max(int(nbytes), 1), dtype=torch.uint8, device=device)
        _WS[key] = buf
    return buf


_PACKED = {}


def pack_conv_weight(weight, transpose_flip=False, f4=False, f4s=False, ci_range=None, ds=False):
    require_gpu(weight)
    assert not (ds and (f4 or f4s or transpose_flip)), 'ds is a layout of its own, of the forward orientation'
    key, wid, ver = (bool(transpose_flip), 3 if ds else (2 if f4s else bool(f4))), id(weight), weight._version
    if ci_range is not None:
        assert not transpose_flip, 'input-channel ranges serve forward convs'
        key = key + ((int(ci_range[0]), int(ci_range[1])),)
    ent = _PACKED.get(wid)
    if ent is not None and ent[0]() is weight:
        hit = ent[1].get(key)
        if hit is not None and hit[0] == ver and hit[2] == weight.data_ptr():
            return hit[1]
    else:
        ent = (weakref.ref(weight, lambda _r, wid=wid: _PACKED.pop(wid, None)), {})
        _PACKED[wid] = ent
    L = _lib.lib()
    w = weight.detach()
    if ci_range is not None:
        w = w[:, ci_range[0]:ci_range[1]]
    if not w.is_contiguous():
        w = w.contiguous()
    o, i, k, k2 = w.shape
    assert k == k2, 'square kernels only'
    co, ci = (i, o) if transpose_flip else (o, i)
    if ds:
        out = torch.empty(L.edvr_conv2d_packed_weight_ds_elems(co, ci, k), dtype=torch.int32, device=w.device)
        _lib.check(L.edvr_conv2d_pack_weight_ds_f32(_ptr(w), _ptr(out), co, ci, k, _stream()), 'edvr_conv2d_pack_weight_ds_f32')
    elif f4s and k == 1:
        assert not transpose_flip, 'the split 1x1 kernel serves forward convs'
        n_el = L.edvr_conv2d_packed_weight_1x1s_elems(co, ci)
        stale = ent[1].get(key)
        if stale is not None and stale[1].numel() == n_el and stale[1].device == w.device and _sole_owner(stale):
            out = stale[1]
        else:
            out = torch.empty(n_el, dtype=torch.int32, device=w.device)
        _lib.check(L.edvr_conv2d_pack_weight_1x1s_f32(_ptr(w), _ptr(out), co, ci, _stream()), 'edvr_conv2d_pack_weight_1x1s_f32')
    elif f4s:
        assert k == 3, 'F(4x4,3x3) weights are for 3x3 kernels'
        out = torch.empty(L.edvr_conv2d_packed_weight_f4s_elems(co, ci), dtype=torch.int32, device=w.device)
        _lib.check(L.edvr_conv2d_pack_weight_f4s_f32(_ptr(w), _ptr(out), co, ci, 1 if transpose_flip else 0, _stream()),
                   'edvr_conv2d_pack_weight_f4s_f32')
    elif f4:
        assert k == 3, 'F(4x4,3x3) weights are for 3x3 kernels'
        out = torch.empty(L.edvr_conv2d_packed_weight_f4_elems(co, ci), dtype=torch.float32, device=w.device)
        _lib.check(L.edvr_conv2d_pack_weight_f4_f32(_ptr(w), _ptr(out), co, ci, 1 if transpose_flip else 0, _stream()),
                   'edvr_conv2d_pack_weight_f4_f32')
    else:
        out = torch.empty(L.edvr_conv2d_packed_weight_elems(co, ci, k), dtype=torch.float32, device=w.device)
        _lib.check(L.edvr_conv2d_pack_weight_f32(_ptr(w), _ptr(out), co, ci, k, 1 if transpose_flip else 0, _stream()),
                   'edvr_conv2d_pack_weight_f32')
    ent[1][key] = (ver, out, weight.data_ptr())
    return out


_PACK_CALLS = 0
_PACK_TABLES = {}


_PINNED_PACKED = set()


def pin_packed_weights(weights):
    bufs = []
    for w in weights:
        ent = _PACKED.get(id(w))
        if ent is not None and ent[0]() is w:
            bufs.extend(hit[1] for hit in ent[1].values())
    _PINNED_PACKED.update(b.data_ptr() for b in bufs)
    return bufs


def unpin_packed_weights(bufs):
    for b in bufs:
        _PINNED_PACKED.discard(b.data_ptr())


def _sole_owner(hit):
    import sys
    return hit[1]._use_count() == 1 and sys.getrefcount(hit[1]) == 2 and hit[1].data_ptr() not in _PINNED_PACKED


def prepack_conv_weights(weights, meta=None):
    import numpy as np
    global _PACK_CALLS
    L = _lib.lib()
    jobs, sig, filled = [], [], []
    meta = list(meta) if meta is not None else None
    for wi, w in enumerate(weights):
        fwd_f4, dgrad = meta[wi] if meta is not None else (True, True)
        if not w.is_cuda or w.dtype != torch.float32 or w.dim() != 4 or w.shape[2] != w.shape[3] or w.shape[2] not in (1, 3) or not w.is_contiguous():
            continue
        wid, ver, k = id(w), w._version, w.shape[2]
        ent = _PACKED.get(wid)
        if ent is None or ent[0]() is not w:
            ent = (weakref.ref(w, lambda _r, wid=wid: _PACKED.pop(wid, None)), {})
            _PACKED[wid] = ent
        for flip in ((False, True) if dgrad else (False,)):
            co, ci = (w.shape[1], w.shape[0]) if flip else (w.shape[0], w.shape[1])
            want_f4 = F4_TRAINING and k == 3 and ci >= 32 and co >= 48 and (flip or fwd_f4)
            kinds = [False] + ([2 if F4S_TRAINING else True] if want_f4 else [])
            outs = []
            for f4 in kinds:
                hit = ent[1].get((flip, f4))
                if hit is not None and hit[0] == ver and hit[2] == w.data_ptr():
                    outs.append(None)
                    continue
                if f4 == 2:
                    n, dt = L.edvr_conv2d_packed_weight_f4s_elems(co, ci), torch.int32
                else:
                    n, dt = (L.edvr_conv2d_packed_weight_f4_elems(co, ci) if f4 else L.edvr_conv2d_packed_weight_elems(co, ci, k)), torch.float32
                if hit is not None and hit[1].numel() == n and hit[1].dtype == dt and hit[1].device == w.device and _sole_owner(hit):
                    buf = hit[1]
                    if f4 == 2 and len(hit) > 3 and hit[3] != _PACK_CALLS:
                        buf[2:4].zero_()
                else:
                    buf = torch.empty(n, dtype=dt, device=w.device)
                    if f4 == 2:
                        buf[:16].zero_()
                outs.append(buf)
                filled.append((ent, (flip, f4), ver, buf, w.data_ptr()))
            wpk = outs[0]
            wf4 = outs[1] if (want_f4 and not F4S_TRAINING) else None
            wf4s = outs[1] if (want_f4 and F4S_TRAINING) else None
            if wpk is None and wf4 is None and wf4s is None:
                continue
            wq = wf4 if wf4 is not None else wf4s
            work = max((wpk.numel() if wpk is not None else 0), (wq.numel() // 36 if wq is not None else 0))
            jobs.append((w.data_ptr(), wpk.data_ptr() if wpk is not None else 0, wf4.data_ptr() if wf4 is not None else 0, co, ci, k,
                         int(flip), max(1, min(64, (work + 255) // 256)), wf4s.data_ptr() if wf4s is not None else 0))
    if not jobs:
        return 0
    key = tuple(jobs)
    tab = _PACK_TABLES.get(key)
    if tab is None:
        rec = np.zeros(len(jobs), dtype=np.dtype([('w', '<u8'), ('wpk', '<u8'), ('f4', '<u8'), ('co', '<i4'), ('ci', '<i4'), ('ks', '<i4'),
                                                  ('flip', '<i4'), ('first', '<i4'), ('nb', '<i4'), ('f4s', '<u8'), ('pad', '<i4', (2,))]))
        assert rec.dtype.itemsize == L.edvr_pack_job_bytes()
        first = 0
        for i, (pw, pk, pf, co, ci, k, flip, nb, ps) in enumerate(jobs):
            rec[i] = (pw, pk, pf, co, ci, k, flip, first, nb, ps, (0, 0))
            first += nb
        dev = filled[0][3].device
        tab = (torch.from_numpy(rec.view(np.uint8).copy()).to(dev), first)
        if len(_PACK_TABLES) > 8:
            _PACK_TABLES.clear()
        _PACK_TABLES[key] = tab
    _PACK_CALLS += 1
    parity = _PACK_CALLS if any(j[8] for j in jobs) else -1
    _lib.check(L.edvr_conv2d_pack_weights_multi(_ptr(tab[0]), len(jobs), tab[1], parity, _stream()), 'edvr_conv2d_pack_weights_multi')
    for ent, k2, ver, buf, ptr in filled:
        ent[1][k2] = (ver, buf, ptr, _PACK_CALLS)
    return len(jobs)


def f4_weight(weight, ks, transpose_flip=False):
    if not F4_TRAINING or ks != 3:
        return None
    co, ci = (weight.shape[1], weight.shape[0]) if transpose_flip else (weight.shape[0], weight.shape[1])
    return pack_conv_weight(weight, transpose_flip=transpose_flip, f4=True) if (ci >= 32 and co >= 48) else None


def f4_kwargs(weight, ks, transpose_flip=False):
    if ks == 1 and F4S_TRAINING and not transpose_flip and weight.shape[1] >= 320 and weight.shape[1] % 8 == 0:
        return {'wpk_f4s': pack_conv_weight(weight, f4s=True)}
    if not F4_TRAINING or ks != 3:
        return {}
    co, ci = (weight.shape[1], weight.shape[0]) if transpose_flip else (weight.shape[0], weight.shape[1])
    if not (ci >= 32 and co >= 48):
        return {}
    if F4S_TRAINING:
        return {'wpk_f4s': pack_conv_weight(weight, transpose_flip=transpose_flip, f4s=True)}
    return {'wpk_f4': pack_conv_weight(weight, transpose_flip=transpose_flip, f4=True)}


def invalidate_packed_weights():
    _PACKED.clear()
    _W_L1.clear()


DCN_SCATTER_AUTO, DCN_SCATTER_DEVICE, DCN_SCATTER_LDS, DCN_SCATTER_STRIP, DCN_SCATTER_LDS_WIDE = 0, 1, 2, 3, 4
_SCATTER_NAMES = {0: '[auto]', 1: '[device atomics]', 2: '[lds window]', 3: '[strip / fused]', 4: '[lds window]'}
DCN_HALO_TAPWIN = _lib.DCN_HALO_TAPWIN
LAUNCH_HOOK = None
CONV_ALGO = CONV_AUTO
F4_INFERENCE = os.environ.get('EDVR_WINOGRAD_F4', '1') != '0'
F4S_INFERENCE = os.environ.get('EDVR_WINOGRAD_F4S', '1') != '0'
F4S_TRAINING = os.environ.get('EDVR_WINOGRAD_F4S_TRAIN', os.environ.get('EDVR_WINOGRAD_F4S', '1')) != '0'
F4_TRAINING = os.environ.get('EDVR_WINOGRAD_F4_TRAIN', '1') != '0'


def set_f4(inference=None, training=None):
    global F4_INFERENCE, F4_TRAINING
    prev = (F4_INFERENCE, F4_TRAINING)
    if inference is not None:
        F4_INFERENCE = bool(inference)
    if training is not None:
        F4_TRAINING = bool(training)
    return prev


def set_f4s(inference=None, training=None):
    global F4S_INFERENCE, F4S_TRAINING
    prev = (F4S_INFERENCE, F4S_TRAINING)
# ... 251 lines not shown
        require_gpu(pre)
        pre = _as_planes(pre)
        if tuple(pre.shape[1:]) != (co, ho, wo):
            raise RuntimeError(f'pre shape {tuple(pre.shape)}: expected (n_pre, {co}, {ho}, {wo})')
        d.pre, d.pre_img_stride, d.pre_n = _ptr(pre), _img_stride(pre), pre.shape[0]
        if pre_map is not None:
            d.pre_div, d.pre_mul, d.pre_add = pre_map
    d.y, d.y_img_stride, d.out_mode = _ptr(out), _img_stride(out), out_mode
    d.y_scale = float(y_scale)
    if wpk_f4 is not None:
        require_gpu(wpk_f4)
        d.wpk_f4 = _ptr(wpk_f4)
    d.algo = CONV_ALGO if algo is None else algo
    split = False
    if wpk_f4s is not None or wpk_ds is not None:
        require_gpu(wpk_f4s, wpk_ds, dtypes=(torch.int32,))
        d.wpk_f4s, d.wpk_ds = _ptr(wpk_f4s), _ptr(wpk_ds)
        d.x_amax = _ptr(wpk_f4s if wpk_f4s is not None else wpk_ds)
        split = bool(L.edvr_conv2d_y_amax_supported(ctypes.byref(d)))
        if split:
            if x_amax is None:
                x_amax = input_bound(x1_in, x1)
                if x2 is not None:
                    x_amax = torch.maximum(x_amax, input_bound(x2_in, x2))
            require_gpu(x_amax)
            if BOUND_CHECK:
                true = amax(x1).item() if x2 is None else max(amax(x1).item(), amax(x2).item())
                if not (x_amax.item() >= true):
                    raise AssertionError(f'magnitude bound {x_amax.item():.6g} < max |x| = {true:.6g} for a conv input of shape {tuple(x1.shape)}')
                direct = L.edvr_conv2d_kernel(ctypes.byref(d)) == _lib.CONV_KERNEL_DIRECT_SPLIT
                (BOUND_CHECK_LOG_DIRECT if direct else BOUND_CHECK_LOG).append((tuple(x1.shape), x_amax.item() / max(true, 1e-30)))
            d.x_amax = _ptr(x_amax)
            if want_y_amax:
                y_bound = _arena(x1.device).slot(x1.device)
                d.y_amax = _ptr(y_bound)
        else:
            d.wpk_f4s, d.wpk_ds, d.x_amax = None, None, None
    sums = None
    if abs_sum_channels > 0 and L.edvr_conv2d_abs_sum_supported(ctypes.byref(d)):
        sums = torch.zeros(2, n, dtype=torch.float32, device=x1.device)
        d.abs_sum, d.abs_sum_channels = _ptr(sums), int(abs_sum_channels)
    name, flops, nbytes, executed = 'conv2d', 0.0, 0.0, None
    if LAUNCH_HOOK is not None:
        buf = ctypes.create_string_buffer(96)
        L.edvr_conv2d_kernel_name(ctypes.byref(d), buf, 96)
        name = buf.value.decode()
        ex = ctypes.c_double(0.0)
        if L.edvr_conv2d_executed_flops(ctypes.byref(d), ctypes.byref(ex)) == 0:
            executed = ex.value
        flops = 2.0 * n * ho * wo * co * (c1 + d.c2) * ks * ks
        nbytes = 4.0 * (n * (c1 + d.c2) * h * w + n * co * ho * wo * (1 + (res1 is not None) + (res2 is not None) + (gate is not None) + (pre is not None))
                        + co * (c1 + d.c2) * ks * ks)
    _run(name, lambda: _lib.check(L.edvr_conv2d_f32(ctypes.byref(d), _stream()), 'edvr_conv2d_f32'), flops, nbytes, executed)
    if y_bound is not None:
        set_bound(out, y_bound)
    else:
        void_bound(out)
    if abs_sum_channels > 0:
        if sums is None:
            return out, abs_stats_per_image(out[:, :abs_sum_channels])
        step = max(1, n // 4)
        sel = out[::step, :abs_sum_channels]
        r = abs_stats_per_image(sel)
        sums[1, ::step] = r[1] * (float(n) / sel.shape[0])
        return out, sums
    return out


def conv_pre_supported(n, c, h, w, co, f4s, algo=None):
    d = _lib.ConvDesc()
    d.c1, d.n, d.h, d.w, d.co, d.ks, d.stride = c, n, h, w, co, 3, 1
    d.algo = CONV_ALGO if algo is None else algo
    any_ptr = ctypes.addressof(d) & ~15
    if f4s:
        d.wpk_f4s = d.x_amax = any_ptr
    else:
        d.wpk_f4 = any_ptr
    return bool(_lib.lib().edvr_conv2d_pre_supported(ctypes.byref(d)))


def conv_gate_supported(n, c, h, w, co, algo=None):
    d = _lib.ConvDesc()
    d.c1, d.n, d.h, d.w, d.co, d.ks, d.stride = c, n, h, w, co, 3, 1
    d.algo = CONV_ALGO if algo is None else algo
    return bool(_lib.lib().edvr_conv2d_gate_supported(ctypes.byref(d)))


def _ones_mask(offset):
    return torch.ones(offset.shape[0], offset.shape[1] // 2, offset.shape[2], offset.shape[3], dtype=offset.dtype, device=offset.device)


def dcnv1_forward(x, offset, weight, stride, pad, dil, groups, dg, halo_hint=0, out=None):
    if require_gpu(x, offset, weight, dtypes=tuple(DCN_DTYPES)) != torch.float32:
        return dcnv2_forward(x, offset, _ones_mask(offset), weight, None, stride, pad, dil, groups, dg, out=out)
    L = _lib.lib()
    offset = _as_planes(offset)
    dims = _dcn_dims(x, weight, stride, pad, dil, groups, dg)
    B, C, H, W, Co, kh, kw = dims[:7]
    ho, wo = offset.shape[2], offset.shape[3]
    if out is not None:
        if tuple(out.shape) != (B, Co, ho, wo) or out.dtype != torch.float32 or not out.is_contiguous() or out.device != x.device:
            raise RuntimeError(f'out must be a contiguous float32 tensor of shape {(B, Co, ho, wo)} on {x.device}')
        y = out
    else:
        y = torch.empty(B, Co, ho, wo, dtype=torch.float32, device=x.device)
    nbytes = L.edvr_dcnv1_fwd_ws_bytes(*dims)
    ws = workspace(nbytes, x.device)
    _run('dcnv1_fwd', lambda: _lib.check(L.edvr_dcnv1_fwd_f32(_ptr(x), _ptr(offset), _ptr(weight), _ptr(y), *dims, _bstride(offset), halo_hint, _ptr(ws), nbytes,
                                    _stream()),
                                       'edvr_dcnv1_fwd_f32'), 2.0 * B * Co * ho * wo * weight.shape[1] * kh * kw, _nb(x, offset, weight, y))
    void_bound(y)
    return y


def dcnv1_backward(x, offset, weight, dy, stride, pad, dil, groups, dg, scatter_hint=0):
    if require_gpu(x, offset, weight, dy, dtypes=tuple(DCN_DTYPES)) != torch.float32:
        dx, doff, _, dw, _ = dcnv2_backward(x, offset, _ones_mask(offset), weight, dy, False, stride, pad, dil, groups, dg)
        return dx, doff, dw
    L = _lib.lib()
    offset = _as_planes(offset)
    dy = dy.contiguous()
    dims = _dcn_dims(x, weight, stride, pad, dil, groups, dg)
    dx = torch.empty_like(x)
    doff = torch.empty(offset.shape, dtype=torch.float32, device=x.device)
    dw = torch.empty_like(weight)
    nbytes = L.edvr_dcnv1_bwd_ws_bytes(*dims)
    ws = workspace(nbytes, x.device)
    _run('dcnv1_bwd', lambda: _lib.check(L.edvr_dcnv1_bwd_f32(_ptr(x), _ptr(offset), _ptr(weight), _ptr(dy), _ptr(dx), _ptr(doff), _ptr(dw), *dims,
                                    _bstride(offset), _bstride(doff), int(scatter_hint), _ptr(ws), nbytes, _stream()),
                                       'edvr_dcnv1_bwd_f32'), 4.0 * dy.numel() * weight[0].numel(),
                                       _nb(x, offset, weight, dy, dx, doff, dw))
    return dx, doff, dw


def _hw(v):
    return (int(v[0]), int(v[1])) if isinstance(v, (tuple, list)) else (int(v), int(v))


def _enc_hw(v):
    h, w = _hw(v)
    return h if h == w else (h | ((w + 1) << 16))


def _dcn_dims(x, weight, stride, pad, dil, groups, dg):
    B, C, H, W = x.shape
    Co, cig, kh, kw = weight.shape
    return [B, C, H, W, Co, kh, kw, _enc_hw(stride), _enc_hw(pad), _enc_hw(dil), groups, dg]


def _bstride(t):
    return t.stride(0) if t.shape[0] > 1 else 0


def dcnv2_forward(x, offset, mask, weight, bias, stride, pad, dil, groups, dg, act=ACT_NONE, halo_hint=0, out=None, xm_bound=None):
    dt = require_gpu(x, offset, mask, weight, bias, dtypes=tuple(DCN_DTYPES))
    L = _lib.lib()
    if not x.is_contiguous() or not weight.is_contiguous():
        raise RuntimeError('input tensor has to be contiguous')
    offset, mask = _as_planes(offset), _as_planes(mask)
    dims = _dcn_dims(x, weight, stride, pad, dil, groups, dg)
    B, C, H, W, Co, kh, kw = dims[:7]
    if C != weight.shape[1] * groups:
        raise RuntimeError(f'Input shape and kernel channels wont match: ({C} vs {weight.shape[1] * groups}).')
    (sh, sw), (ph, pw), (dh, dw) = _hw(stride), _hw(pad), _hw(dil)
    Ho = (H + 2 * ph - (dh * (kh - 1) + 1)) // sh + 1
    Wo = (W + 2 * pw - (dw * (kw - 1) + 1)) // sw + 1
    if Ho <= 0 or Wo <= 0:
        raise ValueError(f'convolution input is too small (output would be {Ho}x{Wo})')
    if tuple(offset.shape[1:]) != (dg * 2 * kh * kw, Ho, Wo):
        raise RuntimeError(f'invalid spatial size / channels of offset: got {tuple(offset.shape)}, expected (B, {dg * 2 * kh * kw}, {Ho}, {Wo})')
    if tuple(mask.shape[1:]) != (dg * kh * kw, Ho, Wo):
        raise RuntimeError(f'invalid spatial size / channels of mask: got {tuple(mask.shape)}, expected (B, {dg * kh * kw}, {Ho}, {Wo})')
    if out is not None:
        if tuple(out.shape) != (B, Co, Ho, Wo) or out.dtype != dt or not out.is_contiguous() or out.device != x.device:
            raise RuntimeError(f'out must be a contiguous {dt} tensor of shape {(B, Co, Ho, Wo)} on {x.device}')
        y = out
    else:
        y = torch.empty(B, Co, Ho, Wo, dtype=dt, device=x.device)
    if dt != torch.float32:
        if act != ACT_NONE:
            raise NotImplementedError('the fused activation of dcnv2_forward exists in fp32 only')
        nbytes = L.edvr_dcnv2_any_ws_bytes(DCN_DTYPES[dt], *dims)
        ws = workspace(nbytes, x.device)
        _lib.check(L.edvr_dcnv2_fwd_any(DCN_DTYPES[dt], _ptr(x), _ptr(offset), _ptr(mask), _ptr(weight), _ptr(bias), _ptr(y), *dims,
                                        _bstride(offset), _bstride(mask), _ptr(ws), nbytes, _stream()), 'edvr_dcnv2_fwd_any')
        void_bound(y)
        return y
    nbytes = L.edvr_dcnv2_fwd_ws_bytes(*dims)
    ws = workspace(nbytes, x.device)
    name = 'dcnv2_fwd'
    split = xm_bound is not None and bool(L.edvr_dcnv2_fwd_split_applies(_ptr(x), *dims, int(halo_hint)))
    if LAUNCH_HOOK is not None:
        buf = ctypes.create_string_buffer(64)
        if L.edvr_dcnv2_fwd_kernel_name(_ptr(x), *dims, int(halo_hint), buf, 64) == 0:
            name = f'dcnv2_fwd[{"dcn_tapwin_split_fwd_kernel" if split else buf.value.decode()}]'
    common = (_ptr(x), _ptr(offset), _ptr(mask), _ptr(weight), _ptr(bias), _ptr(y), *dims, _bstride(offset), _bstride(mask), act, halo_hint, _ptr(ws), nbytes)
    if split:
        require_gpu(xm_bound)
        launch = lambda: _lib.check(L.edvr_dcnv2_fwd_split_f32(*common, _ptr(xm_bound), _stream()), 'edvr_dcnv2_fwd_split_f32')
    else:
        launch = lambda: _lib.check(L.edvr_dcnv2_fwd_f32(*common, _stream()), 'edvr_dcnv2_fwd_f32')
    _run(name, launch, 2.0 * B * Co * Ho * Wo * weight.shape[1] * kh * kw, _nb(x, offset, mask, weight, y))
    void_bound(y)
    return y


def dcnv2_backward(x, offset, mask, weight, dy, with_bias, stride, pad, dil, groups, dg, doffset=None, dmask=None,
                   scatter_hint=0, xm_bound=None, dy_bound=None):
    dt = require_gpu(x, offset, mask, weight, dy, dtypes=tuple(DCN_DTYPES))
    L = _lib.lib()
    offset, mask = _as_planes(offset), _as_planes(mask)
    dy = dy.contiguous()
    dims = _dcn_dims(x, weight, stride, pad, dil, groups, dg)
    dx = torch.empty_like(x)
    doff = doffset if doffset is not None else torch.empty(offset.shape, dtype=dt, device=x.device)
    dmsk = dmask if dmask is not None else torch.empty(mask.shape, dtype=dt, device=x.device)
    assert _plane_contig(doff) and _plane_contig(dmsk)
    dw = torch.empty_like(weight)
    db = torch.empty(weight.shape[0], dtype=dt, device=x.device) if with_bias else None
    if dt != torch.float32:
        nbytes = L.edvr_dcnv2_any_ws_bytes(DCN_DTYPES[dt], *dims)
        ws = workspace(nbytes, x.device)
        _lib.check(L.edvr_dcnv2_bwd_any(DCN_DTYPES[dt], _ptr(x), _ptr(offset), _ptr(mask), _ptr(weight), _ptr(dy), _ptr(dx), _ptr(doff),
                                        _ptr(dmsk), _ptr(dw), _ptr(db), *dims, _bstride(offset), _bstride(mask), _bstride(doff),
                                        _bstride(dmsk), _ptr(ws), nbytes, _stream()), 'edvr_dcnv2_bwd_any')
        void_bound(doff, dmsk)
        return dx, doff, dmsk, dw, db
    nbytes = L.edvr_dcnv2_bwd_ws_bytes(*dims)
    ws = workspace(nbytes, x.device)
    common = (_ptr(x), _ptr(offset), _ptr(mask), _ptr(weight), _ptr(dy), _ptr(dx), _ptr(doff), _ptr(dmsk), _ptr(dw), _ptr(db), *dims,
              _bstride(offset), _bstride(mask), _bstride(doff), _bstride(dmsk), int(scatter_hint), _ptr(ws), nbytes)
    if xm_bound is not None and dy_bound is not None and L.edvr_dcnv2_bwd_split_applies():
        require_gpu(xm_bound, dy_bound)
        launch = lambda: _lib.check(L.edvr_dcnv2_bwd_split_f32(*common, _ptr(xm_bound), _ptr(dy_bound), _stream()), 'edvr_dcnv2_bwd_split_f32')
    else:
        launch = lambda: _lib.check(L.edvr_dcnv2_bwd_f32(*common, _stream()), 'edvr_dcnv2_bwd_f32')
    _run('dcnv2_bwd' + _SCATTER_NAMES.get(int(scatter_hint), ''), launch, 4.0 * dy.numel() * weight[0].numel(),
         _nb(x, offset, mask, weight, dy, dx, doff, dmsk, dw))
    void_bound(doff, dmsk)
    return dx, doff, dmsk, dw, db


def tsa_temporal(emb, emb_ref, aligned, want_prob=False):
    require_gpu(emb, emb_ref, aligned)
    b, t, c, h, w = aligned.shape
    al_in = aligned
    emb, emb_ref, aligned = emb.contiguous(), emb_ref.contiguous(), aligned.contiguous()
    out = torch.empty_like(aligned)
    prob = torch.empty(b, t, h, w, dtype=torch.float32, device=aligned.device) if want_prob else None
    _run('tsa_temporal', lambda: _lib.check(_lib.lib().edvr_tsa_temporal_f32(_ptr(emb), _ptr(emb_ref), _ptr(aligned), _ptr(out), _ptr(prob), b, t, c, h * w,
                                                _stream()),
                                       'edvr_tsa_temporal_f32'), 0, _nb(emb, emb_ref, aligned, out, prob))
    carry_bound(out, al_in)
    return (out, prob) if want_prob else out


def tsa_temporal_pair(emb, emb_ref, aligned, out=None, out_rev=None):
    if torch.is_grad_enabled():
        raise RuntimeError('tsa_temporal_pair has no backward: call it under torch.no_grad()')
    require_gpu(emb, emb_ref, aligned, out, out_rev)
    b, t, c, h, w = aligned.shape
    al_in = aligned
    emb, emb_ref, aligned = emb.contiguous(), emb_ref.contiguous(), aligned.contiguous()
    if tuple(emb.shape) != (b, t, c, h, w) or tuple(emb_ref.shape) != (b, c, h, w):
        raise ValueError(f'tsa_temporal_pair: emb {tuple(emb.shape)} / emb_ref {tuple(emb_ref.shape)} do not match aligned {tuple(aligned.shape)}')
    out = torch.empty_like(aligned) if out is None else out
    out_rev = torch.empty_like(aligned) if out_rev is None else out_rev
    nbytes = 4 * aligned.numel()
    for o in (out, out_rev):
        if tuple(o.shape) != (b, t, c, h, w) or not o.is_contiguous():
            raise ValueError(f'tsa_temporal_pair: outputs are contiguous {(b, t, c, h, w)} tensors, got {tuple(o.shape)} / strides {o.stride()}')
    spans = [(v.data_ptr(), v.data_ptr() + nbytes) for v in (out, out_rev, aligned)]
    if any(a0 < b1 and b0 < a1 for i, (a0, a1) in enumerate(spans) for b0, b1 in spans[i + 1:]):
        raise ValueError('tsa_temporal_pair: out, out_rev and aligned must be distinct buffers (every frame is read and written at two places)')
    _run('tsa_temporal_pair', lambda: _lib.check(_lib.lib().edvr_tsa_temporal_pair_f32(_ptr(emb), _ptr(emb_ref), _ptr(aligned), _ptr(out), _ptr(out_rev), b, t, c,
                                                     h * w, _stream()),
                                            'edvr_tsa_temporal_pair_f32'), 0, _nb(emb, emb_ref, aligned, out, out_rev))
    void_bound(out, out_rev)
    carry_bound(out, al_in)
    carry_bound(out_rev, al_in)
    return out, out_rev


def pool_maxavg(x):
    require_gpu(x)
    x_in, x = x, x.contiguous()
    n, c, h, w = x.shape
    y = torch.empty(n, 2 * c, (h - 1) // 2 + 1, (w - 1) // 2 + 1, dtype=torch.float32, device=x.device)
    _run('pool_maxavg_3x3s2', lambda: _lib.check(_lib.lib().edvr_pool_maxavg_3x3s2_f32(_ptr(x), _ptr(y), n, c, h, w, _stream()),
                                       'edvr_pool_maxavg_3x3s2_f32'), 0, _nb(x, y))
    return carry_bound(y, x_in)


def upsample2x(x, scale=1.0):
    require_gpu(x)
    x_in, x = x, x.contiguous()
    n, c, h, w = x.shape
    y = torch.empty(n, c, 2 * h, 2 * w, dtype=torch.float32, device=x.device)
    _run('upsample2x', lambda: _lib.check(_lib.lib().edvr_upsample2x_f32(_ptr(x), _ptr(y), n * c, h, w, float(scale), _stream()),
                                       'edvr_upsample2x_f32'), 0, _nb(x, y))
    return carry_bound(y, x_in, scale=abs(scale))


def tsa_combine(feat, attn, attn_add):
    require_gpu(feat, attn, attn_add)
    f_in, a_in = feat, attn_add
    feat, attn, attn_add = feat.contiguous(), attn.contiguous(), attn_add.contiguous()
    y = torch.empty_like(feat)
    _run('tsa_combine', lambda: _lib.check(_lib.lib().edvr_tsa_combine_f32(_ptr(feat), _ptr(attn), _ptr(attn_add), _ptr(y), feat.numel(), _stream()),
                                       'edvr_tsa_combine_f32'), 0, _nb(feat, attn, attn_add, y))
    bf, ba = get_bound(f_in), get_bound(a_in)
    if bf is not None and ba is not None:
        set_bound(y, bf * 2.0 + ba, max(_bound_depth(f_in), _bound_depth(a_in)))
    return y


def upsample4x_add_(y, base):
    require_gpu(y, base)
    base = base.contiguous()
    n, c, h, w = base.shape
    assert y.is_contiguous() and tuple(y.shape) == (n, c, 4 * h, 4 * w)
    by, bb = get_bound(y), get_bound(base)
    depth = max(_bound_depth(y), _bound_depth(base)) if (by is not None and bb is not None) else 0
    _run('upsample4x_add', lambda: _lib.check(_lib.lib().edvr_upsample4x_add_f32(_ptr(base), _ptr(y), n * c, h, w, _stream()),
                                       'edvr_upsample4x_add_f32'), 0, _nb(base, y, y))
    void_bound(y)
    if by is not None and bb is not None:
        set_bound(y, by + bb, depth)
    return y


def add(a, b):
    require_gpu(a, b)
    a_in, b_in = a, b
    a, b = a.contiguous(), b.contiguous()
    assert a.shape == b.shape
    y = torch.empty_like(a)
    _run('add', lambda: _lib.check(_lib.lib().edvr_add_f32(_ptr(a), _ptr(b), _ptr(y), a.numel(), _stream()),
                                       'edvr_add_f32'), 0, _nb(a, b, y))
    return carry_bound(y, a_in, b_in)


def act_backward(dy, y, act, act_from=0, res1=None, res2=None):
    require_gpu(dy, y, res1, res2)
    dy_in = dy
    dy, y = dy.contiguous(), y.contiguous()
    res1 = res1.contiguous() if res1 is not None else None
    res2 = res2.contiguous() if res2 is not None else None
    n, c = y.shape[:2]
    dz = torch.empty_like(dy)
    _run('act_bwd', lambda: _lib.check(_lib.lib().edvr_act_bwd_f32(_ptr(dy), _ptr(y), _ptr(res1), _ptr(res2), _ptr(dz), n, c, y[0, 0].numel(), act, act_from,
                                           _stream()),
                                       'edvr_act_bwd_f32'), 0, _nb(dy, y, res1, res2, dz))
    return carry_bound(dz, dy_in)


def set_wgrad_algo(algo):
    prev = _lib.lib().edvr_conv2d_wgrad_algo(int(algo))
    if prev < 0:
        _lib.check(prev, 'edvr_conv2d_wgrad_algo')
    return prev


def conv2d_wgrad(x1, x2, x2_map, dz, co, ks, stride, want_db=False, into=None):
    require_gpu(x1, x2, dz)
    L = _lib.lib()
    x1_in, x2_in, dz_in = x1, x2, dz
    x1, dz = _as_planes(x1), _as_planes(dz)
    n, c1, h, w = x1.shape
    c2 = 0
    if x2 is not None:
        x2 = _as_planes(x2)
        c2 = x2.shape[1]
    div, mul, add = x2_map if x2_map is not None else (0, 0, 0)
    if into is None:
        dw = torch.empty(co, c1 + c2, ks, ks, dtype=torch.float32, device=x1.device)
    else:
        require_gpu(into)
        assert into.is_contiguous() and tuple(into.shape) == (co, c1 + c2, ks, ks), \
            f'into {tuple(into.shape)} / strides {into.stride()}: expected a contiguous {(co, c1 + c2, ks, ks)}'
        dw = into
    nbytes = L.edvr_conv2d_wgrad_ws_bytes(n, c1 + c2, h, w, co, ks, stride)
    ws = workspace(nbytes, x1.device)
    db = torch.empty(co, dtype=torch.float32, device=x1.device) if want_db else None
    name = 'conv2d_wgrad'
    split = F4S_TRAINING and bool(L.edvr_conv2d_wgrad_split_applies(n, c1, c2, h, w, co, ks, stride))
    if LAUNCH_HOOK is not None:
        buf = ctypes.create_string_buffer(96)
        L.edvr_conv2d_wgrad_kernel_name(n, c1, c2, h, w, co, ks, stride, buf, 96)
        name = buf.value.decode()
        if split and name == 'conv3x3_winograd_wgrad_kernel':
            name = 'conv3x3_wgrad_direct_split_kernel' if L.edvr_conv2d_wgrad_split_is_direct(h, w) else 'conv3x3_winograd_wgrad_split_kernel'
    pad = ks // 2
    ho, wo = (h + 2 * pad - ks) // stride + 1, (w + 2 * pad - ks) // stride + 1
    common = (_ptr(x1), _ptr(x2), _ptr(dz), _ptr(dw), c1, c2, n, h, w, co, ks, stride, _img_stride(x1), _img_stride(x2) if x2 is not None else 0,
              div, mul, add, _img_stride(dz), 0 if into is None else 1, _ptr(db), _ptr(ws), nbytes)
    if split and ks == 1:
        bx, bz = get_bound(x1_in), get_bound(dz_in)
        split = bx is not None and bz is not None
        if split and name == 'gemm_nt_kernel':
            name = 'gemm_nt_split_kernel'
    elif split:
        bx = input_bound(x1_in, x1)
        if x2 is not None:
            bx = torch.maximum(bx, input_bound(x2_in, x2))
        bz = input_bound(dz_in, dz)
    if split:
# ... 1223 lines not shown
```

include/edvr_amd.h:

```cpp
#ifndef EDVR_AMD_H
#define EDVR_AMD_H

#include <stddef.h>
#include <stdint.h>

#ifdef __cplusplus
extern "C" {
#endif

#define EDVR_OK 0
#define EDVR_ERR_ARG (-1)
#define EDVR_ERR_UNSUPPORTED (-2)
#define EDVR_ERR_LAUNCH (-3)
#define EDVR_ERR_WORKSPACE (-4)

typedef void *edvr_stream_t;

const char *edvr_version(void);
const char *edvr_last_error(void);
int edvr_check_device(void);

#define EDVR_ACT_NONE 0
#define EDVR_ACT_RELU 1
#define EDVR_ACT_LRELU 2
#define EDVR_ACT_SIGMOID 3

#define EDVR_DCN_HALO_TAPWIN 16
#define EDVR_DCN_SCATTER_AUTO 0
#define EDVR_DCN_SCATTER_DEVICE 1
#define EDVR_DCN_SCATTER_LDS 2
#define EDVR_DCN_SCATTER_STRIP 3
#define EDVR_DCN_SCATTER_LDS_WIDE 4
#define EDVR_CONV_AUTO 0
#define EDVR_CONV_DIRECT 1
#define EDVR_CONV_WINOGRAD 2
#define EDVR_CONV_WINOGRAD_F4 3
#define EDVR_CONV_WINOGRAD_F4S 4

#define EDVR_OUT_NCHW 0
#define EDVR_OUT_PIXEL_SHUFFLE2 1

typedef struct edvr_conv2d_desc {
  const float *x1;
  const float *x2;
  int c1, c2;
  int64_t x1_img_stride;
  int64_t x2_img_stride;
  int x2_div, x2_mul, x2_add;
  int n, h, w;
  const float *wpk;
  const float *bias;
  int co, ks, stride;
  int act;
  int act_from;
  const float *res1;
  const float *res2;
  int64_t res1_img_stride, res2_img_stride;
  float *y;
  int64_t y_img_stride;
  int out_mode;
  int algo;
  const float *gate;
  int64_t gate_img_stride;
  float gate_slope;
  float y_scale;
  const float *wpk_f4;
  float *abs_sum;
  int abs_sum_channels;
  const void *wpk_f4s;
  const float *x_amax;
  float *y_amax;
  const float *pre;
  int64_t pre_img_stride;
  int pre_div, pre_mul, pre_add;
  int pre_n;
  const void *wpk_ds;
} edvr_conv2d_desc;

size_t edvr_conv2d_packed_weight_elems(int co, int ci, int ks);
int edvr_conv2d_pack_weight_f32(const float *w, float *wpk, int co, int ci, int ks, int transpose_flip,
                                edvr_stream_t stream);
size_t edvr_conv2d_packed_weight_f4_elems(int co, int ci);
int edvr_conv2d_pack_weight_f4_f32(const float *w, float *wpk_f4, int co, int ci, int transpose_flip, edvr_stream_t stream);
size_t edvr_conv2d_packed_weight_f4s_elems(int co, int ci);
int edvr_conv2d_pack_weight_f4s_f32(const float *w, void *wpk_f4s, int co, int ci, int transpose_flip, edvr_stream_t stream);
size_t edvr_conv2d_packed_weight_1x1s_elems(int co, int ci);
int edvr_conv2d_pack_weight_1x1s_f32(const float *w, void *wpk_1x1s, int co, int ci, edvr_stream_t stream);
size_t edvr_conv2d_packed_weight_ds_elems(int co, int ci, int ks);
int edvr_conv2d_pack_weight_ds_f32(const float *w, void *wpk_ds, int co, int ci, int ks, edvr_stream_t stream);
int edvr_amax_f32(const float *x, float *amax, int n, int64_t per_img, int64_t img_stride, edvr_stream_t stream);
size_t edvr_pack_job_bytes(void);
int edvr_conv2d_pack_weights_multi(const void *jobs, int n_jobs, int total_blocks, int split_parity, edvr_stream_t stream);
int edvr_conv2d_f32(const edvr_conv2d_desc *d, edvr_stream_t stream);
#define EDVR_CONV_KERNEL_SMALL 0
#define EDVR_CONV_KERNEL_F4S 1
#define EDVR_CONV_KERNEL_F4 2
#define EDVR_CONV_KERNEL_F2 3
#define EDVR_CONV_KERNEL_1X1_SPLIT 4
#define EDVR_CONV_KERNEL_1X1_STREAM 5
#define EDVR_CONV_KERNEL_DIRECT_SPLIT 6
#define EDVR_CONV_KERNEL_DIRECT 7
int edvr_conv2d_kernel(const edvr_conv2d_desc *d);
int edvr_conv2d_gate_supported(const edvr_conv2d_desc *d);
int edvr_conv2d_y_amax_supported(const edvr_conv2d_desc *d);
int edvr_conv2d_abs_sum_supported(const edvr_conv2d_desc *d);
int edvr_conv2d_pre_supported(const edvr_conv2d_desc *d);
int edvr_conv2d_f4s_set_lean(int on);
int edvr_conv2d_f4s_lean_items(const edvr_conv2d_desc *d);
int edvr_conv2d_kernel_name(const edvr_conv2d_desc *d, char *buf, size_t buf_len);
int edvr_conv2d_executed_flops(const edvr_conv2d_desc *d, double *flops);

#define EDVR_HW(h, w) ((int)(h) | (((int)(w) + 1) << 16))

size_t edvr_dcnv2_fwd_ws_bytes(int B, int C, int H, int W, int Co, int kh, int kw, int stride, int pad, int dil,
                               int groups, int dg);
int edvr_dcnv2_fwd_f32(const float *x, const float *offset, const float *mask, const float *weight,
                       const float *bias, float *y, int B, int C, int H, int W, int Co, int kh, int kw, int stride,
                       int pad, int dil, int groups, int dg, int64_t offset_bstride, int64_t mask_bstride, int act,
                       int halo_hint, void *ws, size_t ws_bytes, edvr_stream_t stream);

int edvr_dcnv2_fwd_split_f32(const float *x, const float *offset, const float *mask, const float *weight, const float *bias,
                             float *y, int B, int C, int H, int W, int Co, int kh, int kw, int stride, int pad, int dil, int groups,
                             int dg, int64_t offset_bstride, int64_t mask_bstride, int act, int halo_hint, void *ws, size_t ws_bytes,
                             const float *xm_amax, edvr_stream_t stream);
int edvr_dcnv2_fwd_split_applies(const float *x, int B, int C, int H, int W, int Co, int kh, int kw, int stride, int pad, int dil, int groups,
                                 int dg, int halo_hint);
int edvr_dcnv2_fwd_kernel_name(const float *x, int B, int C, int H, int W, int Co, int kh, int kw, int stride, int pad, int dil,
                               int groups, int dg, int halo_hint, char *buf, size_t buf_len);

size_t edvr_dcnv2_bwd_ws_bytes(int B, int C, int H, int W, int Co, int kh, int kw, int stride, int pad, int dil,
                               int groups, int dg);
int edvr_dcnv2_bwd_f32(const float *x, const float *offset, const float *mask, const float *weight, const float *dy,
                       float *dx, float *doffset, float *dmask, float *dweight, float *dbias, int B, int C, int H,
                       int W, int Co, int kh, int kw, int stride, int pad, int dil, int groups, int dg,
                       int64_t offset_bstride, int64_t mask_bstride, int64_t doffset_bstride, int64_t dmask_bstride,
                       int scatter_hint, void *ws, size_t ws_bytes, edvr_stream_t stream);
int edvr_dcnv2_bwd_split_f32(const float *x, const float *offset, const float *mask, const float *weight, const float *dy,
                             float *dx, float *doffset, float *dmask, float *dweight, float *dbias, int B, int C, int H,
                             int W, int Co, int kh, int kw, int stride, int pad, int dil, int groups, int dg,
                             int64_t offset_bstride, int64_t mask_bstride, int64_t doffset_bstride, int64_t dmask_bstride,
                             int scatter_hint, void *ws, size_t ws_bytes, const float *xm_amax, const float *dy_amax,
                             edvr_stream_t stream);
int edvr_dcnv2_bwd_split_applies(void);

#define EDVR_DTYPE_F32 0
#define EDVR_DTYPE_F64 1
#define EDVR_DTYPE_F16 2
size_t edvr_dcnv2_any_ws_bytes(int dtype, int B, int C, int H, int W, int Co, int kh, int kw, int stride, int pad, int dil, int groups,
                               int dg);
int edvr_dcnv2_fwd_any(int dtype, const void *x, const void *offset, const void *mask, const void *weight, const void *bias, void *y, int B,
                       int C, int H, int W, int Co, int kh, int kw, int stride, int pad, int dil, int groups, int dg,
                       int64_t offset_bstride, int64_t mask_bstride, void *ws, size_t ws_bytes, edvr_stream_t stream);
int edvr_dcnv2_bwd_any(int dtype, const void *x, const void *offset, const void *mask, const void *weight, const void *dy, void *dx,
                       void *doffset, void *dmask, void *dweight, void *dbias, int B, int C, int H, int W, int Co, int kh, int kw, int stride,
                       int pad, int dil, int groups, int dg, int64_t offset_bstride, int64_t mask_bstride, int64_t doffset_bstride,
                       int64_t dmask_bstride, void *ws, size_t ws_bytes, edvr_stream_t stream);

size_t edvr_dcnv1_fwd_ws_bytes(int B, int C, int H, int W, int Co, int kh, int kw, int stride, int pad, int dil,
                               int groups, int dg);
int edvr_dcnv1_fwd_f32(const float *x, const float *offset, const float *weight, float *y, int B, int C, int H, int W,
                       int Co, int kh, int kw, int stride, int pad, int dil, int groups, int dg, int64_t offset_bstride,
                       int halo_hint, void *ws, size_t ws_bytes, edvr_stream_t stream);
size_t edvr_dcnv1_bwd_ws_bytes(int B, int C, int H, int W, int Co, int kh, int kw, int stride, int pad, int dil,
                               int groups, int dg);
int edvr_dcnv1_bwd_f32(const float *x, const float *offset, const float *weight, const float *dy, float *dx,
                       float *doffset, float *dweight, int B, int C, int H, int W, int Co, int kh, int kw, int stride,
                       int pad, int dil, int groups, int dg, int64_t offset_bstride, int64_t doffset_bstride,
                       int scatter_hint, void *ws, size_t ws_bytes, edvr_stream_t stream);

int edvr_tsa_temporal_f32(const float *emb, const float *emb_ref, const float *aligned, float *out, float *prob_out,
                          int b, int t, int c, int hw, edvr_stream_t stream);
int edvr_tsa_temporal_pair_f32(const float *emb, const float *emb_ref, const float *aligned, float *out, float *out_rev,
                               int b, int t, int c, int hw, edvr_stream_t stream);
int edvr_pool_maxavg_3x3s2_f32(const float *x, float *y, int n, int c, int h, int w, edvr_stream_t stream);
int edvr_upsample2x_f32(const float *x, float *y, int nc, int h, int w, float scale, edvr_stream_t stream);
int edvr_tsa_combine_f32(const float *feat, const float *attn, const float *attn_add, float *y, int64_t numel,
                         edvr_stream_t stream);
int edvr_upsample4x_add_f32(const float *base, float *y, int nc, int h, int w, edvr_stream_t stream);
int edvr_add_f32(const float *a, const float *b, float *y, int64_t numel, edvr_stream_t stream);
int edvr_act_bwd_f32(const float *dy, const float *y, const float *res1, const float *res2, float *dz, int n, int c,
                     int64_t hw, int act, int act_from, edvr_stream_t stream);
int edvr_abs_sum_f32(const float *x, float *out, int n, int64_t per_img, int64_t img_stride, edvr_stream_t stream);
int edvr_abs_stats_f32(const float *x, float *out, int n, int64_t per_img, int w, int64_t img_stride, edvr_stream_t stream);

size_t edvr_conv2d_wgrad_ws_bytes(int n, int ci, int h, int w, int co, int ks, int stride);
int edvr_conv2d_wgrad_f32(const float *x1, const float *x2, const float *dz, float *dw, int c1, int c2, int n, int h, int w,
                          int co, int ks, int stride, int64_t x1_img_stride, int64_t x2_img_stride, int x2_div, int x2_mul,
                          int x2_add, int64_t dz_img_stride, int accumulate, float *dbias, void *ws, size_t ws_bytes,
                          edvr_stream_t stream);
int edvr_conv2d_wgrad_split_f32(const float *x1, const float *x2, const float *dz, float *dw, int c1, int c2, int n, int h, int w,
                                int co, int ks, int stride, int64_t x1_img_stride, int64_t x2_img_stride, int x2_div, int x2_mul,
                                int x2_add, int64_t dz_img_stride, int accumulate, float *dbias, void *ws, size_t ws_bytes,
                                const float *x_amax, const float *dz_amax, edvr_stream_t stream);
int edvr_conv2d_wgrad_split_applies(int n, int c1, int c2, int h, int w, int co, int ks, int stride);
int edvr_conv2d_wgrad_split_is_direct(int h, int w);
int edvr_conv2d_wgrad_kernel_name(int n, int c1, int c2, int h, int w, int co, int ks, int stride, char *buf, size_t buf_len);

int edvr_conv2d_wgrad_algo(int algo);
int edvr_channel_sum_f32(const float *x, float *out, int n, int c, int64_t hw, int64_t img_stride, void *ws, size_t ws_bytes,
                         edvr_stream_t stream);
int edvr_pixel_unshuffle2_f32(const float *x, float *y, int n, int c, int h, int w, edvr_stream_t stream);
int edvr_pixel_unshuffle2_act_bwd_f32(const float *dy, const float *y, float *dz, int n, int c, int h, int w, int act, edvr_stream_t stream);
int edvr_zero_stuff2_f32(const float *dz, float *z, int nc, int H, int W, int ho, int wo, edvr_stream_t stream);
int edvr_frame_reduce_add_f32(const float *src, float *dst, int b, int t, int center, int64_t chw, edvr_stream_t stream);
int edvr_upsample2x_bwd_f32(const float *dy, float *dx, int nc, int h, int w, float scale, edvr_stream_t stream);
int edvr_pool_maxavg_3x3s2_bwd_f32(const float *x, const float *dy, float *dx, int n, int c, int h, int w, edvr_stream_t stream);
int edvr_tsa_temporal_bwd_f32(const float *emb, const float *emb_ref, const float *aligned, const float *dout, float *d_emb,
                              float *d_emb_ref, float *d_aligned, int b, int t, int c, int hw, float *ws, edvr_stream_t stream);
int edvr_tsa_combine_bwd_f32(const float *feat, const float *attn, const float *dy, float *dfeat, float *dattn, int64_t numel,
                             edvr_stream_t stream);
int edvr_charbonnier_f32(const float *pred, const float *target, float *loss, float *dpred, int64_t numel, float eps,
                         float grad_scale, edvr_stream_t stream);

int edvr_psnr_sse_f32(const float *a, const float *b, double *partial, int n, int c, int h, int w, int64_t a_img_stride,
                      int64_t b_img_stride, int crop_border, int y_channel, int blocks, edvr_stream_t stream);

size_t edvr_ssim_partials(int h, int w, int crop_border);
int edvr_ssim_f32(const float *a, const float *b, double *partial, int n, int c, int h, int w, int64_t a_img_stride,
                  int64_t b_img_stride, int crop_border, int y_channel, edvr_stream_t stream);

size_t edvr_niqe_blocks(int h, int w, int crop_border);
int edvr_niqe_moments_f32(const float *x, double *out, int n, int c, int h, int w, int64_t img_stride, int crop_border, edvr_stream_t stream);
int edvr_niqe_moments_u8(const uint8_t *x, double *out, int n, int h, int w, int64_t img_stride, int crop_border, edvr_stream_t stream);

#define EDVR_AUG_HFLIP 1
#define EDVR_AUG_VFLIP 2
#define EDVR_AUG_ROT90 4
int edvr_frames_u8_to_f32(const uint8_t *src, float *dst, int n_clips, int frames_per_clip, int h, int w,
                          const uint8_t *clip_flags, int swap_rb, edvr_stream_t stream);

#define EDVR_GATHER_MAX_LEVELS 3
int edvr_gather_images_f32(const float *const *src, float *const *dst, const int64_t *src_img_stride, const int64_t *per_img, int levels,
                           const int *table, int n_out, int n_src, edvr_stream_t stream);
int edvr_upsample4x_add_u8(const float *y, const float *base, uint8_t *out, int n, int h, int w, edvr_stream_t stream);
int edvr_f32_to_u8_hwc(const float *x, uint8_t *out, int n, int h, int w, int64_t x_img_stride, edvr_stream_t stream);

#define EDVR_PAD_REFLECT 0
#define EDVR_PAD_REPLICATE 1
int edvr_crop_pad_frames_u8(const uint8_t *src, float *dst, int n, int H, int W, int y0, int x0, int th, int tw, int pad_mode,
                            edvr_stream_t stream);
int edvr_crop_pad_frames_f32(const float *src, float *dst, int n, int H, int W, int64_t src_img_stride, int y0, int x0, int th, int tw,
                             int pad_mode, edvr_stream_t stream);
int edvr_upsample4x_add_rect_f32(const float *y, const float *base, float *dst, int n, int h, int w, int ky, int kx, int kh, int kw,
                                 int64_t dst_row_stride, int64_t dst_plane_stride, int64_t dst_img_stride, edvr_stream_t stream);
int edvr_upsample4x_add_rect_u8(const float *y, const float *base, uint8_t *dst, int n, int h, int w, int ky, int kx, int kh, int kw,
                                int64_t dst_row_stride, int64_t dst_img_stride, edvr_stream_t stream);
int edvr_f32_to_u8_hwc_rect(const float *x, uint8_t *dst, int n, int h, int w, int64_t x_img_stride, int ky, int kx, int kh, int kw,
                            int64_t dst_row_stride, int64_t dst_img_stride, edvr_stream_t stream);
int edvr_copy_rect_f32(const float *x, float *dst, int n, int h, int w, int64_t x_img_stride, int ky, int kx, int kh, int kw,
                       int64_t dst_row_stride, int64_t dst_plane_stride, int64_t dst_img_stride, edvr_stream_t stream);

#define EDVR_D4_FIRST 1
#define EDVR_D4_LAST 2
int edvr_crop_pad_frames_d4_u8(const uint8_t *src, float *dst, int n, int H, int W, int y0, int x0, int th, int tw, int pad_mode, int elem,
                               edvr_stream_t stream);
int edvr_crop_pad_frames_d4_f32(const float *src, float *dst, int n, int H, int W, int64_t src_img_stride, int y0, int x0, int th, int tw,
                                int pad_mode, int elem, edvr_stream_t stream);
int edvr_upsample4x_add_rect_d4_f32(const float *y, const float *base, float *acc, int n, int h, int w, int ky, int kx, int kh, int kw,
                                    int64_t acc_row_stride, int64_t acc_plane_stride, int64_t acc_img_stride, int elem, int mode, float scale,
                                    edvr_stream_t stream);
int edvr_upsample4x_add_rect_d4_u8(const float *y, const float *base, float *acc, uint8_t *dst, int n, int h, int w, int ky, int kx, int kh,
                                   int kw, int64_t acc_row_stride, int64_t acc_plane_stride, int64_t acc_img_stride, int64_t dst_row_stride,
                                   int64_t dst_img_stride, int elem, int mode, float scale, edvr_stream_t stream);
int edvr_f32_to_u8_hwc_rect_d4(const float *x, float *acc, uint8_t *dst, int n, int h, int w, int64_t x_img_stride, int ky, int kx, int kh,
                               int kw, int64_t acc_row_stride, int64_t acc_plane_stride, int64_t acc_img_stride, int64_t dst_row_stride,
                               int64_t dst_img_stride, int elem, int mode, float scale, edvr_stream_t stream);
int edvr_copy_rect_d4_f32(const float *x, float *acc, int n, int h, int w, int64_t x_img_stride, int ky, int kx, int kh, int kw,
                          int64_t acc_row_stride, int64_t acc_plane_stride, int64_t acc_img_stride, int elem, int mode, float scale,
                          edvr_stream_t stream);

int edvr_upsample4x_add_rect_blend_f32(const float *y, const float *base, float *acc, int n, int h, int w, int ky, int kx, int kh, int kw,
                                       int64_t acc_row_stride, int64_t acc_plane_stride, int64_t acc_img_stride, int elem, int mode, float scale,
                                       int band_y_lo, int band_y_hi, int band_x_lo, int band_x_hi, edvr_stream_t stream);
int edvr_upsample4x_add_rect_blend_u8(const float *y, const float *base, float *acc, uint8_t *dst, int n, int h, int w, int ky, int kx, int kh,
                                      int kw, int64_t acc_row_stride, int64_t acc_plane_stride, int64_t acc_img_stride, int64_t dst_row_stride,
                                      int64_t dst_img_stride, int elem, int mode, float scale, int band_y_lo, int band_y_hi, int band_x_lo,
                                      int band_x_hi, edvr_stream_t stream);
int edvr_f32_to_u8_hwc_rect_blend(const float *x, float *acc, uint8_t *dst, int n, int h, int w, int64_t x_img_stride, int ky, int kx, int kh,
                                  int kw, int64_t acc_row_stride, int64_t acc_plane_stride, int64_t acc_img_stride, int64_t dst_row_stride,
                                  int64_t dst_img_stride, int elem, int mode, float scale, int band_y_lo, int band_y_hi, int band_x_lo,
                                  int band_x_hi, edvr_stream_t stream);
int edvr_copy_rect_blend_f32(const float *x, float *acc, int n, int h, int w, int64_t x_img_stride, int ky, int kx, int kh, int kw,
                             int64_t acc_row_stride, int64_t acc_plane_stride, int64_t acc_img_stride, int elem, int mode, float scale,
                             int band_y_lo, int band_y_hi, int band_x_lo, int band_x_hi, edvr_stream_t stream);

#define EDVR_RESIZE_OUT_F32 0
#define EDVR_RESIZE_OUT_U8 1
int edvr_imresize_bicubic_u8(const uint8_t *src, void *dst, int n, int H, int W, int ho, int wo, double scale, int antialiasing,
                             int out_kind, edvr_stream_t stream);
int edvr_imresize_bicubic_f32(const float *src, void *dst, int n, int H, int W, int64_t src_img_stride, int ho, int wo, double scale,
                              int antialiasing, int out_kind, edvr_stream_t stream);

int edvr_bd_downsample_u8(const uint8_t *src, void *dst, int n, int H, int W, int ho, int wo, int scale, int out_u8, edvr_stream_t stream);
int edvr_bd_downsample_f32(const float *src, void *dst, int n, int H, int W, int64_t src_img_stride, int ho, int wo, int scale, int out_u8,
                           edvr_stream_t stream);

#define EDVR_LQ_WINDOW_RECORD_INTS 8
int edvr_imresize_bicubic_u8_windows(const uint8_t *src, const int32_t *table, const int32_t *table_host, uint8_t *dst, int n, int p, int wh,
                                     int ww, int pitch, int scale, edvr_stream_t stream);
int edvr_bd_downsample_u8_windows(const uint8_t *src, const int32_t *table, const int32_t *table_host, uint8_t *dst, int n, int p, int wh, int ww,
                                  int pitch, int scale, edvr_stream_t stream);

int edvr_yuv420_to_rgb_f32(const uint8_t *yuv, float *rgb, int n, int H, int W, int64_t yuv_stride, int64_t rgb_img_stride, const float *coef,
                           int bilinear, edvr_stream_t stream);
int edvr_yuv420_to_rgb_u8(const uint8_t *yuv, uint8_t *rgb, int n, int H, int W, int64_t yuv_stride, const float *coef, int bilinear,
                          edvr_stream_t stream);
int edvr_rgb_to_yuv420_f32(const float *rgb, uint8_t *yuv, int n, int H, int W, int64_t rgb_img_stride, int64_t yuv_stride, const float *coef,
                           edvr_stream_t stream);
int edvr_rgb_to_yuv420_u8(const uint8_t *rgb, uint8_t *yuv, int n, int H, int W, int64_t yuv_stride, const float *coef, edvr_stream_t stream);
int edvr_yuv_to_rgb_f32(const uint8_t *yuv, float *rgb, int n, int H, int W, int sub_x, int sub_y, int depth, int64_t yuv_stride,
                        int64_t rgb_img_stride, const float *coef, int bilinear, edvr_stream_t stream);
int edvr_rgb_to_yuv_f32(const float *rgb, uint8_t *yuv, int n, int H, int W, int sub_x, int sub_y, int depth, int64_t rgb_img_stride,
                        int64_t yuv_stride, const float *coef, edvr_stream_t stream);

int edvr_yuv_to_rgb_sited_f32(const uint8_t *yuv, float *rgb, int n, int H, int W, int sub_x, int sub_y, int depth, int64_t yuv_stride,
                              int64_t rgb_img_stride, const float *coef, int bilinear, int siting_x, int siting_y, edvr_stream_t stream);
int edvr_rgb_to_yuv_sited_f32(const float *rgb, uint8_t *yuv, int n, int H, int W, int sub_x, int sub_y, int depth, int64_t rgb_img_stride,
                              int64_t yuv_stride, const float *coef, int siting_x, int siting_y, edvr_stream_t stream);
int edvr_yuv420_to_rgb_sited_u8(const uint8_t *yuv, uint8_t *rgb, int n, int H, int W, int64_t yuv_stride, const float *coef, int bilinear,
                                int siting_x, int siting_y, edvr_stream_t stream);
int edvr_rgb_to_yuv420_sited_u8(const uint8_t *rgb, uint8_t *yuv, int n, int H, int W, int64_t yuv_stride, const float *coef, int siting_x,
                                int siting_y, edvr_stream_t stream);

int edvr_frame_sad_rgb_u8(const uint8_t *x, const uint8_t *prev, uint64_t *sad, int n, int H, int W, int64_t img_stride, edvr_stream_t stream);
int edvr_frame_sad_rgb_f32(const float *x, const float *prev, uint64_t *sad, int n, int H, int W, int64_t img_stride, edvr_stream_t stream);

// ... 26 lines not shown
```

Before: 105.9 clips/s.

## Fuse TSA temporal attention with dual 1x1 heads; cache packed DCN split weights

Adds a fused TSA front kernel. It computes the per-frame sigmoid correlation probabilities, then applies them to the aligned features on the fly while running the feature-fusion and spatial-attention 1x1 convolutions together, using the split-f16 matrix path. This removes the materialized weighted tensor and a separate pass over it. It also lets the DCN split forward reuse pre-packed weights tied to the parameter, instead of repacking on every call. The cost is new kernel complexity, and the fused path only covers inference with t<=16, c%8==0 and co<=128.

After: 107.1 clips/s, median of 6. 1.01x the previous value.

```diff
diff --git a/edvr_amd/_lib.py b/edvr_amd/_lib.py
--- a/edvr_amd/_lib.py
+++ b/edvr_amd/_lib.py
@@ -52,6 +52,9 @@
     'edvr_dcnv2_fwd_f32': (i32, [vp] * 6 + [i32] * 12 + [i64, i64, i32, i32, vp, sz, vp]),
     'edvr_dcnv2_fwd_split_f32': (i32, [vp] * 6 + [i32] * 12 + [i64, i64, i32, i32, vp, sz, vp, vp]),
     'edvr_dcnv2_fwd_split_applies': (i32, [vp] + [i32] * 13),
+    'edvr_dcnv2_split_packed_weight_elems': (sz, [i32, i32]),
+    'edvr_dcnv2_split_pack_weight_f32': (i32, [vp, vp, i32, i32, vp]),
+    'edvr_dcnv2_fwd_split_packed_f32': (i32, [vp] * 6 + [i32] * 12 + [i64, i64, i32, i32, vp, vp]),
     'edvr_dcnv2_fwd_kernel_name': (i32, [vp] + [i32] * 13 + [ctypes.c_char_p, sz]),
     'edvr_dcnv2_bwd_ws_bytes': (sz, [i32] * 12),
     'edvr_dcnv2_any_ws_bytes': (sz, [i32] * 13),
@@ -117,6 +120,9 @@
     'edvr_dcnv2_bwd_split_applies': (i32, []),
     'edvr_tsa_temporal_f32': (i32, [vp] * 5 + [i32] * 4 + [vp]),
     'edvr_tsa_temporal_pair_f32': (i32, [vp] * 5 + [i32] * 4 + [vp]),
+    'edvr_tsa_front_supported': (i32, [i32] * 6),
+    'edvr_tsa_front_applies': (i32, [i32] * 12 + [vp, vp, vp]),
+    'edvr_tsa_front_f32': (i32, [vp, vp, i64, vp, vp] + [vp, vp, i32, vp, vp] * 2 + [i32] * 6 + [vp]),
     'edvr_pool_maxavg_3x3s2_f32': (i32, [vp, vp, i32, i32, i32, i32, vp]),
     'edvr_upsample2x_f32': (i32, [vp, vp, i32, i32, i32, f32, vp]),
     'edvr_tsa_combine_f32': (i32, [vp, vp, vp, vp, i64, vp]),
diff --git a/edvr_amd/build.py b/edvr_amd/build.py
--- a/edvr_amd/build.py
+++ b/edvr_amd/build.py
@@ -9,7 +9,7 @@
 LIBDIR = os.path.join(HERE, 'lib')
 LIB = os.path.join(LIBDIR, 'libedvr_amd.so')
 OBJDIR = os.path.join(HERE, 'build')
-SOURCES = ['api.hip', 'pack.hip', 'conv2d.hip', 'conv2d_s.hip', 'dcn.hip', 'dcn_any.hip', 'elementwise.hip', 'wgrad.hip', 'backward.hip', 'dcn_fused.hip', 'dcn_tapwin.hip', 'dcn_tapwin_s.hip', 'dcn_bwd_fused.hip', 'winograd.hip', 'winograd_f4.hip', 'winograd_f4s.hip', 'winograd_wgrad.hip', 'winograd_wgrad_s.hip', 'wgrad_direct_s.hip', 'gemm_nt_s.hip', 'optim.hip', 'metrics.hip', 'conv_small.hip', 'conv1x1.hip', 'conv1x1_s.hip', 'data.hip', 'video.hip', 'resize.hip', 'bd.hip', 'ensemble.hip', 'yuv.hip', 'niqe.hip', 'shots.hip', 'jpeg.hip', 'degrade.hip', 'mpeg.hip']
+SOURCES = ['api.hip', 'pack.hip', 'conv2d.hip', 'conv2d_s.hip', 'dcn.hip', 'dcn_any.hip', 'elementwise.hip', 'wgrad.hip', 'backward.hip', 'dcn_fused.hip', 'dcn_tapwin.hip', 'dcn_tapwin_s.hip', 'dcn_bwd_fused.hip', 'winograd.hip', 'winograd_f4.hip', 'winograd_f4s.hip', 'winograd_wgrad.hip', 'winograd_wgrad_s.hip', 'wgrad_direct_s.hip', 'gemm_nt_s.hip', 'optim.hip', 'metrics.hip', 'conv_small.hip', 'conv1x1.hip', 'conv1x1_s.hip', 'tsa_front_s.hip', 'data.hip', 'video.hip', 'resize.hip', 'bd.hip', 'ensemble.hip', 'yuv.hip', 'niqe.hip', 'shots.hip', 'jpeg.hip', 'degrade.hip', 'mpeg.hip']
 LINK = []
 FLAGS = ['--offload-arch=gfx950', '-O3', '-std=c++17', '-fPIC', '-munsafe-fp-atomics', '-ffp-contract=fast']
 
diff --git a/edvr_amd/csrc/common.h b/edvr_amd/csrc/common.h
--- a/edvr_amd/csrc/common.h
+++ b/edvr_amd/csrc/common.h
@@ -119,6 +119,11 @@
                        int H, int W, int Co, int dg, int64_t off_bs, int64_t msk_bs, int act, hipStream_t stream);
 
 bool dcn_tapwin_split_enabled();
+size_t dcn_tapwin_split_wpk_elems(int Co, int C);
+int dcn_tapwin_split_pack(const float *weight, unsigned *wpk, int Co, int C, hipStream_t stream);
+int dcn_tapwin_split_forward_packed(const float *x, const float *offset, const float *mask, const unsigned *wpk, const float *bias, float *y,
+                                    int B, int C, int H, int W, int Co, int dg, int64_t off_bs, int64_t msk_bs, int act, const float *xm_amax,
+                                    hipStream_t stream);
 int dcn_tapwin_split_forward(const float *x, const float *offset, const float *mask, const float *weight, unsigned *wpk, const float *bias, float *y,
                              int B, int C, int H, int W, int Co, int dg, int64_t off_bs, int64_t msk_bs, int act, const float *xm_amax,
                              hipStream_t stream);
diff --git a/edvr_amd/csrc/dcn.hip b/edvr_amd/csrc/dcn.hip
--- a/edvr_amd/csrc/dcn.hip
+++ b/edvr_amd/csrc/dcn.hip
@@ -691,6 +691,27 @@
           dcn_tapwin_supported(C, Co, H, W, kh, kw, s.stride, s.pad, s.dil, groups, dg) && (reinterpret_cast<uintptr_t>(x) & 15) == 0) ? 1 : 0;
 }
 
+size_t edvr_dcnv2_split_packed_weight_elems(int Co, int C) { return (Co > 0 && C > 0) ? edvr::dcn_tapwin_split_wpk_elems(Co, C) : 0; }
+
+int edvr_dcnv2_split_pack_weight_f32(const float *weight, void *wpk, int Co, int C, edvr_stream_t stream) {
+  return edvr::dcn_tapwin_split_pack(weight, static_cast<unsigned *>(wpk), Co, C, edvr::as_stream(stream));
+}
+
+int edvr_dcnv2_fwd_split_packed_f32(const float *x, const float *offset, const float *mask, const void *wpk, const float *bias,
+                                    float *y, int B, int C, int H, int W, int Co, int kh, int kw, int stride, int pad, int dil, int groups,
+                                    int dg, int64_t offset_bstride, int64_t mask_bstride, int act, int halo_hint, const float *xm_amax,
+                                    edvr_stream_t stream) {
+  using namespace edvr;
+  EDVR_REQUIRE(x && offset && mask && wpk && y && xm_amax, "dcnv2_fwd_split_packed: null pointer");
+  EDVR_REQUIRE(edvr_dcnv2_fwd_split_applies(x, B, C, H, W, Co, kh, kw, stride, pad, dil, groups, dg, halo_hint),
+               "dcnv2_fwd_split_packed: the split tap-window kernel does not take this call");
+  DcnShape s;
+  const int rc = dcn_fill_shape(s, B, C, H, W, Co, kh, kw, stride, pad, dil, groups, dg, offset_bstride, mask_bstride);
+  if (rc) return rc;
+  return dcn_tapwin_split_forward_packed(x, offset, mask, static_cast<const unsigned *>(wpk), bias, y, B, C, H, W, Co, dg, s.off_bs, s.msk_bs, act,
+                                         xm_amax, as_stream(stream));
+}
+
 int edvr_dcnv2_fwd_kernel_name(const float *x, int B, int C, int H, int W, int Co, int kh, int kw, int stride, int pad, int dil, int groups,
                                int dg, int halo_hint, char *buf, size_t buf_len) {
   using namespace edvr;
diff --git a/edvr_amd/csrc/dcn_tapwin_s.hip b/edvr_amd/csrc/dcn_tapwin_s.hip
--- a/edvr_amd/csrc/dcn_tapwin_s.hip
+++ b/edvr_amd/csrc/dcn_tapwin_s.hip
@@ -463,15 +463,32 @@
   return on;
 }
 
-int dcn_tapwin_split_forward(const float *x, const float *offset, const float *mask, const float *weight, unsigned *wpk, const float *bias, float *y,
-                             int B, int C, int H, int W, int Co, int dg, int64_t off_bs, int64_t msk_bs, int act, const float *xm_amax,
-                             hipStream_t stream) {
-  EDVR_REQUIRE(B <= 65535, "dcn_tapwin_split: batch %d exceeds grid.z", B);
-  EDVR_REQUIRE((reinterpret_cast<uintptr_t>(x) & 15) == 0 && (reinterpret_cast<uintptr_t>(wpk) & 15) == 0, "dcn_tapwin_split: x / wpk must be 16-byte aligned");
+size_t dcn_tapwin_split_wpk_elems(int Co, int C) { return 16 + (size_t)C * 9 * ((Co + 31) / 32 * 32); }
+
+int dcn_tapwin_split_pack(const float *weight, unsigned *wpk, int Co, int C, hipStream_t stream) {
+  EDVR_REQUIRE(weight && wpk && Co > 0 && C > 0 && (C & 3) == 0, "dcn_tapwin_split_pack: bad arguments");
+  EDVR_REQUIRE((reinterpret_cast<uintptr_t>(wpk) & 15) == 0, "dcn_tapwin_split_pack: wpk must be 16-byte aligned");
   const int cop = (Co + 31) / 32 * 32;
   hipLaunchKernelGGL(dcn_tapwin_split_scale_kernel, dim3(1), dim3(1024), 0, stream, weight, wpk, (int64_t)Co * C * 9);
   const int64_t total = (int64_t)(C / 4) * 9 * cop;
   hipLaunchKernelGGL(dcn_tapwin_split_pack_kernel, dim3((unsigned)std::min<int64_t>(cdiv64(total, 256), 2048)), dim3(256), 0, stream, weight, wpk, Co, C, cop);
+  return check_launch("dcn_tapwin_split_pack_kernel");
+}
+
+int dcn_tapwin_split_forward(const float *x, const float *offset, const float *mask, const float *weight, unsigned *wpk, const float *bias, float *y,
+                             int B, int C, int H, int W, int Co, int dg, int64_t off_bs, int64_t msk_bs, int act, const float *xm_amax,
+                             hipStream_t stream) {
+  const int rc = dcn_tapwin_split_pack(weight, wpk, Co, C, stream);
+  if (rc) return rc;
+  return dcn_tapwin_split_forward_packed(x, offset, mask, wpk, bias, y, B, C, H, W, Co, dg, off_bs, msk_bs, act, xm_amax, stream);
+}
+
+int dcn_tapwin_split_forward_packed(const float *x, const float *offset, const float *mask, const unsigned *wpk, const float *bias, float *y,
+                                    int B, int C, int H, int W, int Co, int dg, int64_t off_bs, int64_t msk_bs, int act, const float *xm_amax,
+                                    hipStream_t stream) {
+  EDVR_REQUIRE(B <= 65535, "dcn_tapwin_split: batch %d exceeds grid.z", B);
+  EDVR_REQUIRE((reinterpret_cast<uintptr_t>(x) & 15) == 0 && (reinterpret_cast<uintptr_t>(wpk) & 15) == 0, "dcn_tapwin_split: x / wpk must be 16-byte aligned");
+  const int cop = (Co + 31) / 32 * 32;
   DcnTapwinSArgs a;
   a.xm_amax = xm_amax;
   a.x = x; a.offset = offset; a.mask = mask; a.wpk = wpk; a.bias = bias; a.y = y;
diff --git a/edvr_amd/csrc/tsa_front_s.hip b/edvr_amd/csrc/tsa_front_s.hip
--- /dev/null
+++ b/edvr_amd/csrc/tsa_front_s.hip
@@ -0,0 +1,334 @@
+#include <cstdlib>
+#include <type_traits>
+
+#include "common.h"
+#include "pack.h"
+
+namespace edvr {
+
+typedef float tf_f32x16 __attribute__((ext_vector_type(16)));
+typedef int tf_i32x4 __attribute__((ext_vector_type(4)));
+typedef _Float16 tf_f16x8 __attribute__((ext_vector_type(8)));
+
+__device__ __forceinline__ float tf_sigmoidf(float v) { return 1.f / (1.f + __expf(-v)); }
+
+constexpr int TF_MAX_T = 16;
+
+struct TsaFrontArgs {
+  const float *emb, *emb_ref, *aligned;
+  int64_t ref_img_stride;
+  const float *x_amax;
+  const unsigned *wq[2];
+  const float *bias[2];
+  float *y[2];
+  float *y_amax[2];
+  int act[2];
+  int t, c, hw, co;
+  int ci;
+  int seg_shift;
+};
+
+template <int MT, bool V4>
+__global__ __launch_bounds__(256, 2) void tsa_front_split_kernel(const TsaFrontArgs a) {
+  constexpr int CK = 32, MB = 32 * MT, MB2 = 2 * MB, DEPTH = 8, COP = 128;
+  constexpr int NW = (CK / 4) * MB2 / 256;
+  constexpr int RSRC_FLAGS = 0x00020000;
+  constexpr int OOB = (int)0x80000000;
+  __shared__ __attribute__((aligned(16))) unsigned wsm[2][CK * MB2];
+  __shared__ __attribute__((aligned(16))) float prob_s[TF_MAX_T][128];
+  const float s_x = split_scale(__builtin_bit_cast(float, __builtin_amdgcn_readfirstlane(__builtin_bit_cast(int, *a.x_amax))));
+  const int tid = threadIdx.x, lane = tid & 63, half = lane >> 5, j = lane & 31;
+  const int wave = __builtin_amdgcn_readfirstlane(tid >> 6);
+  const int hw = a.hw, t = a.t, c = a.c;
+  const int img = blockIdx.z;
+  const int p = (blockIdx.x * 4 + wave) * 32 + j;
+  const bool p_ok = p < hw;
+
+  auto uniform_ptr = [&](const float *ptr) {
+    const uint64_t pv = reinterpret_cast<uint64_t>(ptr);
+    return ((uint64_t)(uint32_t)__builtin_amdgcn_readfirstlane((int)(pv >> 32)) << 32) | (uint32_t)__builtin_amdgcn_readfirstlane((int)(uint32_t)pv);
+  };
+  auto rsrc_at = [&](uint64_t base) { return __builtin_amdgcn_make_buffer_rsrc(reinterpret_cast<void *>(base), (short)0, 0x7fffffff, RSRC_FLAGS); };
+  const int64_t plane_bytes = (int64_t)hw * 4;
+  const int64_t frame_bytes = (int64_t)c * plane_bytes;
+
+  tf_i32x4 wr[NW];
+  auto w_load = [&](int c0) {
+#pragma unroll
+    for (int i = 0; i < NW; ++i) {
+      const int e = tid + i * 256, q = e / MB2, col = e - q * MB2, hd = col / MB, cc = col - hd * MB;
+      wr[i] = *reinterpret_cast<const tf_i32x4 *>(a.wq[hd] + 16 + ((int64_t)(c0 / 4 + q) * COP + cc) * 4);
+    }
+  };
+  auto w_commit = [&](int buf) {
+#pragma unroll
+    for (int i = 0; i < NW; ++i) *reinterpret_cast<tf_i32x4 *>(&wsm[buf][(tid + i * 256) * 4]) = wr[i];
+  };
+
+  const uint64_t eb = uniform_ptr(a.emb + (int64_t)img * t * c * hw);
+  const __amdgpu_buffer_rsrc_t ref_rs = rsrc_at(uniform_ptr(a.emb_ref + (int64_t)img * a.ref_img_stride));
+  if constexpr (V4) {
+    typedef float tf_f32x4 __attribute__((ext_vector_type(4)));
+    const int px = blockIdx.x * 128 + 4 * j;
+    const bool q_ok = px < hw;
+    const int v_ref = q_ok ? px * 4 : OOB;
+    for (int f0 = 2 * wave; f0 < t; f0 += 8) {
+      const __amdgpu_buffer_rsrc_t rs = rsrc_at(eb + (uint64_t)(f0 * frame_bytes));
+      const bool f_ok = f0 + half < t;
+      const int v_emb = (q_ok && f_ok) ? (int)(half * frame_bytes) + px * 4 : OOB;
+      tf_f32x4 dot = {0.f, 0.f, 0.f, 0.f};
+      tf_f32x4 ra[8], ea[8], rb[8], eb2[8];
+      auto load_grp = [&](int ch, tf_f32x4 (&r)[8], tf_f32x4 (&e)[8]) {
+#pragma unroll
+        for (int i = 0; i < 8; ++i) {
+          r[i] = __builtin_bit_cast(tf_f32x4, __builtin_amdgcn_raw_buffer_load_b128(ref_rs, v_ref, (ch + i) * hw * 4, 0));
+          e[i] = __builtin_bit_cast(tf_f32x4, __builtin_amdgcn_raw_buffer_load_b128(rs, v_emb, (ch + i) * hw * 4, 0));
+        }
+      };
+      auto fma_grp = [&](const tf_f32x4 (&r)[8], const tf_f32x4 (&e)[8]) {
+#pragma unroll
+        for (int i = 0; i < 8; ++i)
+#pragma unroll
+          for (int v = 0; v < 4; ++v) dot[v] = __builtin_fmaf(e[i][v], r[i][v], dot[v]);
+      };
+      load_grp(0, ra, ea);
+      for (int ch = 0; ch < c; ch += 16) {
+        const bool second = ch + 8 < c;
+        if (second) load_grp(ch + 8, rb, eb2);
+        fma_grp(ra, ea);
+        if (ch + 16 < c) load_grp(ch + 16, ra, ea);
+        if (second) fma_grp(rb, eb2);
+      }
+      if (f_ok) {
+        tf_f32x4 pr;
+#pragma unroll
+        for (int v = 0; v < 4; ++v) pr[v] = tf_sigmoidf(dot[v]);
+        *reinterpret_cast<tf_f32x4 *>(&prob_s[f0 + half][4 * j]) = pr;
+      }
+    }
+  } else {
+    const int npairs = (t + 1) >> 1;
+    const int v_ref = p_ok ? p * 4 : OOB;
+    const int v_emb = p_ok ? (int)(half * frame_bytes) + p * 4 : OOB;
+    const bool last_ok = 2 * (npairs - 1) + half < t;
+    float dot[TF_MAX_T / 2];
+#pragma unroll
+    for (int k = 0; k < TF_MAX_T / 2; ++k) dot[k] = 0.f;
+    float ra[8], rb[8], ea[TF_MAX_T / 2][8], eb2[TF_MAX_T / 2][8];
+    auto load_grp = [&](int ch, float (&r)[8], float (&e)[TF_MAX_T / 2][8]) {
+#pragma unroll
+      for (int i = 0; i < 8; ++i) r[i] = __builtin_bit_cast(float, __builtin_amdgcn_raw_buffer_load_b32(ref_rs, v_ref, (ch + i) * hw * 4, 0));
+#pragma unroll
+      for (int k = 0; k < TF_MAX_T / 2; ++k)
+        if (k < npairs) {
+          const __amdgpu_buffer_rsrc_t rs = rsrc_at(eb + (uint64_t)(2 * k * frame_bytes));
+          const int vo = (k + 1 < npairs || last_ok) ? v_emb : OOB;
+#pragma unroll
+          for (int i = 0; i < 8; ++i) e[k][i] = __builtin_bit_cast(float, __builtin_amdgcn_raw_buffer_load_b32(rs, vo, (ch + i) * hw * 4, 0));
+        }
+    };
+    auto fma_grp = [&](const float (&r)[8], const float (&e)[TF_MAX_T / 2][8]) {
+#pragma unroll
+      for (int k = 0; k < TF_MAX_T / 2; ++k)
+        if (k < npairs) {
+#pragma unroll
+          for (int i = 0; i < 8; ++i) dot[k] = __builtin_fmaf(e[k][i], r[i], dot[k]);
+        }
+    };
+    load_grp(0, ra, ea);
+    for (int ch = 0; ch < c; ch += 16) {
+      const bool second = ch + 8 < c;
+      if (second) load_grp(ch + 8, rb, eb2);
+      fma_grp(ra, ea);
+      if (ch + 16 < c) load_grp(ch + 16, ra, ea);
+      if (second) fma_grp(rb, eb2);
+    }
+#pragma unroll
+    for (int k = 0; k < TF_MAX_T / 2; ++k)
+      if (k < npairs && (k + 1 < npairs || last_ok)) prob_s[2 * k + half][wave * 32 + j] = tf_sigmoidf(dot[k]);
+  }
+
+  const uint64_t ab = uniform_ptr(a.aligned + (int64_t)img * t * c * hw);
+  const int voff = p_ok ? (4 * half * hw + p) * 4 : OOB;
+  const int real_steps = t * c / 8;
+  const int seg_mask = (1 << a.seg_shift) - 1;
+  auto load_b = [&](int s, float (&v)[4]) {
+    const int sc = __builtin_amdgcn_readfirstlane(s);
+    const int cc = 8 * sc;
+    const __amdgpu_buffer_rsrc_t rs = __builtin_amdgcn_make_buffer_rsrc(reinterpret_cast<void *>(ab + (uint64_t)((int64_t)(cc & ~seg_mask) * plane_bytes)), (short)0,
+                                                                        sc < real_steps ? 0x7fffffff : 0, RSRC_FLAGS);
+#pragma unroll
+    for (int i = 0; i < 4; ++i)
+      v[i] = __builtin_bit_cast(float, __builtin_amdgcn_raw_buffer_load_b32(rs, voff, __builtin_amdgcn_readfirstlane(((cc & seg_mask) + i) * hw * 4), 0));
+  };
+
+  tf_f32x16 acc[2][MT];
+#pragma unroll
+  for (int hd = 0; hd < 2; ++hd)
+#pragma unroll
+    for (int m = 0; m < MT; ++m)
+#pragma unroll
+      for (int r = 0; r < 16; ++r) acc[hd][m][r] = 0.f;
+  float bq[DEPTH][4];
+  w_load(0);
+#pragma unroll
+  for (int k = 0; k < DEPTH; ++k) load_b(k, bq[k]);
+  w_commit(0);
+  __syncthreads();
+
+  const int spf = c / 8;
+  int frame = 0, sf = 0;
+  float pf = prob_s[0][wave * 32 + j];
+  const int chunks = a.ci / CK;
+  auto slab = [&](auto parity, int ch) {
+    constexpr int P = decltype(parity)::value;
+    const int buf = P;
+    const bool more = ch + 1 < chunks;
+    const unsigned *ws = wsm[buf] + (half * MB2 + j) * 4;
+#pragma unroll
+    for (int s = 0; s < CK / 8; ++s) {
+      if (more && s == 0) w_load((ch + 1) * CK);
+      if (sf == spf) {
+        sf = 0;
+        frame = min(frame + 1, t - 1);
+        pf = prob_s[frame][wave * 32 + j];
+      }
+      ++sf;
+      const int slot = P * (CK / 8) + s;
+      float mv[4];
+#pragma unroll
+      for (int i = 0; i < 4; ++i) mv[i] = bq[slot][i] * pf;
+      unsigned pk[4];
+      split4_f16x2(mv, s_x, pk);
+      load_b(ch * (CK / 8) + s + DEPTH, bq[slot]);
+      tf_i32x4 b, br;
+#pragma unroll
+      for (int q = 0; q < 4; ++q) {
+        b[q] = (int)pk[q];
+        br[q] = (int)__builtin_amdgcn_alignbit(pk[q], pk[q], 16);
+      }
+#pragma unroll
+      for (int hd = 0; hd < 2; ++hd) {
+        tf_i32x4 av[MT];
+#pragma unroll
+        for (int m = 0; m < MT; ++m) av[m] = *reinterpret_cast<const tf_i32x4 *>(ws + ((2 * s) * MB2 + hd * MB + m * 32) * 4);
+#pragma unroll
+        for (int m = 0; m < MT; ++m)
+          acc[hd][m] = __builtin_amdgcn_mfma_f32_32x32x16_f16(__builtin_bit_cast(tf_f16x8, av[m]), __builtin_bit_cast(tf_f16x8, b), acc[hd][m], 0, 0, 0);
+#pragma unroll
+        for (int m = 0; m < MT; ++m)
+          acc[hd][m] = __builtin_amdgcn_mfma_f32_32x32x16_f16(__builtin_bit_cast(tf_f16x8, av[m]), __builtin_bit_cast(tf_f16x8, br), acc[hd][m], 0, 0, 0);
+      }
+    }
+    if (more) w_commit(buf ^ 1);
+    asm volatile("s_waitcnt lgkmcnt(0)\n\ts_barrier" ::: "memory");
+  };
+  static_assert(DEPTH == 2 * (CK / 8), "two slabs rotate through the register set");
+  for (int ch = 0; ch < chunks; ch += 2) {
+    slab(std::integral_constant<int, 0>{}, ch);
+    if (ch + 1 < chunks) slab(std::integral_constant<int, 1>{}, ch + 1);
+  }
+
+#pragma unroll
+  for (int hd = 0; hd < 2; ++hd) {
+    const float inv_sw = __builtin_bit_cast(float, __builtin_amdgcn_readfirstlane((int)a.wq[hd][1]));
+    const float unscale = inv_sw / s_x;
+    const int act = a.act[hd];
+    const float slope = act == EDVR_ACT_LRELU ? 0.1f : (act == EDVR_ACT_RELU ? 0.f : 1.f);
+    const bool sig = act == EDVR_ACT_SIGMOID;
+    float *y = a.y[hd] + (int64_t)img * a.co * hw;
+    const float *bias = a.bias[hd];
+    unsigned vmax = 0u;
+    if (p_ok) {
+#pragma unroll
+      for (int m = 0; m < MT; ++m)
+#pragma unroll
+        for (int r = 0; r < 16; ++r) {
+          const int co = m * 32 + (r & 3) + 8 * (r >> 2) + 4 * half;
+          if (co < a.co) {
+            float v = __builtin_fmaf(acc[hd][m][r], unscale, bias[co]);
+            v = sig ? __builtin_amdgcn_rcpf(1.f + __expf(-v)) : fmaxf(v, slope * v);
+            y[(int64_t)co * hw + p] = v;
+            vmax = max(vmax, __builtin_bit_cast(unsigned, v) & 0x7fffffffu);
+          }
+        }
+    }
+    if (a.y_amax[hd]) {
+#pragma unroll
+      for (int sh = 32; sh > 0; sh >>= 1) vmax = max(vmax, (unsigned)__shfl_xor((int)vmax, sh));
+      if (lane == 0) publish_amax(a.y_amax[hd], vmax);
+    }
+  }
+}
+
+static bool tsa_front_supported(int b, int t, int c, int h, int w, int co) {
+  if (b <= 0 || t <= 0 || c <= 0 || h <= 0 || w <= 0 || co <= 0) return false;
+  if (b > 65535 || t > TF_MAX_T || (c & 7) || co > 128) return false;
+  const int64_t hw = (int64_t)h * w;
+  return 2 * (int64_t)c * hw * 4 < ((int64_t)1 << 31) && hw * 32 < ((int64_t)1 << 31);
+}
+
+static bool tsa_front_enabled() {
+  static const bool on = []() {
+    const char *e = getenv("EDVR_TSA_FRONT");
+    return !(e && e[0] == '0');
+  }();
+  return on;
+}
+
+}
+
+extern "C" {
+
+int edvr_tsa_front_supported(int b, int t, int c, int h, int w, int co) { return edvr::tsa_front_supported(b, t, c, h, w, co) ? 1 : 0; }
+
+int edvr_tsa_front_applies(int needs_grad, int b, int t, int c, int h, int w, int co_feat, int co_attn, int ks_feat, int ks_attn, int has_bias_feat,
+                           int has_bias_attn, const void *wq_feat, const void *wq_attn, const float *x_amax) {
+  using namespace edvr;
+  if (!tsa_front_enabled() || needs_grad || co_feat != co_attn || ks_feat != 1 || ks_attn != 1 || !has_bias_feat || !has_bias_attn) return 0;
+  if (!wq_feat || !wq_attn || !x_amax || !tsa_front_supported(b, t, c, h, w, co_feat)) return 0;
+  if ((reinterpret_cast<uintptr_t>(wq_feat) & 15) || (reinterpret_cast<uintptr_t>(wq_attn) & 15)) return 0;
+  edvr_conv2d_desc d = {};
+  d.c1 = t * c; d.n = b; d.h = h; d.w = w; d.co = co_feat; d.ks = 1; d.stride = 1;
+  d.out_mode = EDVR_OUT_NCHW; d.algo = EDVR_CONV_AUTO;
+  d.wpk_f4s = wq_feat; d.x_amax = x_amax;
+  return conv2d_select(d) == CONV_1X1_SPLIT ? 1 : 0;
+}
+
+int edvr_tsa_front_f32(const float *emb, const float *emb_ref, int64_t emb_ref_img_stride, const float *aligned, const float *x_amax,
+                       const void *wq_feat, const float *bias_feat, int act_feat, float *feat, float *feat_amax, const void *wq_attn,
+                       const float *bias_attn, int act_attn, float *attn, float *attn_amax, int b, int t, int c, int h, int w, int co,
+                       edvr_stream_t stream) {
+  using namespace edvr;
+  EDVR_REQUIRE(emb && emb_ref && aligned && x_amax && wq_feat && wq_attn && bias_feat && bias_attn && feat && attn, "tsa_front: null pointer");
+  EDVR_REQUIRE(tsa_front_supported(b, t, c, h, w, co), "tsa_front: unsupported shape (b %d, t %d <= 16, c %d %% 8 == 0, %d x %d, co %d <= 128)", b, t, c, h, w, co);
+  EDVR_REQUIRE((reinterpret_cast<uintptr_t>(wq_feat) & 15) == 0 && (reinterpret_cast<uintptr_t>(wq_attn) & 15) == 0,
+               "tsa_front: packed weights must be 16-byte aligned");
+  EDVR_REQUIRE(emb_ref_img_stride >= (int64_t)c * h * w || b == 1, "tsa_front: emb_ref image stride %lld", (long long)emb_ref_img_stride);
+  TsaFrontArgs a;
+  a.emb = emb; a.emb_ref = emb_ref; a.aligned = aligned;
+  a.ref_img_stride = emb_ref_img_stride;
+  a.x_amax = x_amax;
+  a.wq[0] = static_cast<const unsigned *>(wq_feat); a.wq[1] = static_cast<const unsigned *>(wq_attn);
+  a.bias[0] = bias_feat; a.bias[1] = bias_attn;
+  a.y[0] = feat; a.y[1] = attn;
+  a.y_amax[0] = feat_amax; a.y_amax[1] = attn_amax;
+  a.act[0] = act_feat; a.act[1] = act_attn;
+  a.t = t; a.c = c; a.hw = h * w; a.co = co;
+  a.ci = (t * c + 31) / 32 * 32;
+  a.seg_shift = 30;
+  while (((int64_t)1 << a.seg_shift) * a.hw * 4 >= ((int64_t)1 << 31)) --a.seg_shift;
+  if (a.seg_shift < 3) a.seg_shift = 3;
+  const dim3 grid(cdiv(a.hw, 128), 1, b);
+  const bool v4 = (a.hw & 3) == 0 && (emb_ref_img_stride & 3) == 0 && ((reinterpret_cast<uintptr_t>(emb) | reinterpret_cast<uintptr_t>(emb_ref)) & 15) == 0;
+  if (co <= 64) {
+    if (v4) hipLaunchKernelGGL((tsa_front_split_kernel<2, true>), grid, dim3(256), 0, as_stream(stream), a);
+    else hipLaunchKernelGGL((tsa_front_split_kernel<2, false>), grid, dim3(256), 0, as_stream(stream), a);
+  } else {
+    if (v4) hipLaunchKernelGGL((tsa_front_split_kernel<4, true>), grid, dim3(256), 0, as_stream(stream), a);
+    else hipLaunchKernelGGL((tsa_front_split_kernel<4, false>), grid, dim3(256), 0, as_stream(stream), a);
+  }
+  return check_launch("tsa_front_split_kernel");
+}
+
+}
diff --git a/edvr_amd/edvr_arch.py b/edvr_amd/edvr_arch.py
--- a/edvr_amd/edvr_arch.py
+++ b/edvr_amd/edvr_arch.py
@@ -61,6 +61,21 @@
         return self.align(nbr_feat_l, ref_feat_l)
 
 
+class _TSAOperand:
+
+    def __init__(self, emb, emb_ref, aligned):
+        self.emb, self.emb_ref, self.aligned = emb, emb_ref, aligned
+
+    @property
+    def device(self):
+        return self.aligned.device
+
+    def mod(self):
+        b, t, c, h, w = self.aligned.shape
+        m = F_.tsa_temporal(self.emb, self.emb_ref, self.aligned)
+        return F_.ops.carry_bound(m.view(b, t * c, h, w), m)
+
+
 class TSAFusion(nn.Module):
 
     def __init__(self, num_feat=64, num_frame=5, center_frame_idx=2):
@@ -85,9 +100,9 @@
         self.upsample = nn.Upsample(scale_factor=2, mode='bilinear', align_corners=False)
 
     def forward(self, aligned_feat):
-        return self.spatial(self.temporal(aligned_feat))
-
-    def temporal(self, aligned_feat, pair=False):
+        return self.spatial(self.temporal(aligned_feat, lazy=True))
+
+    def temporal(self, aligned_feat, pair=False, lazy=False):
         b, t, c, h, w = aligned_feat.shape
         alias = F_.ops.carry_bound
         emb_ref = F_.conv(self.temporal_attn1, alias(aligned_feat[:, self.center_frame_idx], aligned_feat))
@@ -95,12 +110,17 @@
         if pair:
             mod, mod_rev = F_.tsa_temporal_pair(emb, emb_ref, aligned_feat)
             return alias(mod.view(b, t * c, h, w), mod), alias(mod_rev.view(b, t * c, h, w), mod_rev)
+        if lazy and F_.tsa_front_applies(self.feat_fusion, self.spatial_attn1, emb, emb_ref, aligned_feat):
+            return _TSAOperand(emb, emb_ref, aligned_feat)
         mod = F_.tsa_temporal(emb, emb_ref, aligned_feat)
         return alias(mod.view(b, t * c, h, w), mod)
 
     def spatial(self, mod):
-        feat = F_.conv(self.feat_fusion, mod, act=LRELU)
-        attn = F_.conv(self.spatial_attn1, mod, act=LRELU)
+        if isinstance(mod, _TSAOperand):
+            feat, attn = F_.tsa_front(self.feat_fusion, self.spatial_attn1, mod.emb, mod.emb_ref, mod.aligned, act=LRELU)
+        else:
+            feat = F_.conv(self.feat_fusion, mod, act=LRELU)
+            attn = F_.conv(self.spatial_attn1, mod, act=LRELU)
         attn = F_.conv(self.spatial_attn2, F_.pool_maxavg(attn), act=LRELU)
         lvl = F_.conv(self.spatial_attn_l1, attn, act=LRELU)
         lvl = F_.conv(self.spatial_attn_l2, F_.pool_maxavg(lvl), act=LRELU)
@@ -238,10 +258,13 @@
     def restore_from_features(self, pyr, x_center, b, t, out_dtype=torch.float32, out=None, keep=None, elem=None, accumulate='only', scale=1.0,
                               acc=None, bands=None):
         self._check_tail_args(out_dtype, out, keep, elem, accumulate, scale, acc, bands)
-        operand, sink = self.align_windows(pyr, b, t)
+        operand, sink = self._align_windows(pyr, b, t, lazy=self.taps is None)
         return self._restore_aligned(operand, x_center, b, t, out_dtype, out, keep, elem, accumulate, scale, acc, bands, sink)
 
     def align_windows(self, pyr, b, t, pair=False):
+        return self._align_windows(pyr, b, t, pair)
+
+    def _align_windows(self, pyr, b, t, pair=False, lazy=False):
         f1, f2, f3 = pyr
         ctr = self.center_frame_idx
         h, w = f1.shape[2], f1.shape[3]
@@ -261,7 +284,7 @@
         if self.taps is not None:
             self.taps['aligned'] = aligned
         if self.with_tsa:
-            operand = self.fusion.temporal(aligned, pair=pair)
+            operand = self.fusion.temporal(aligned, pair=pair, lazy=lazy and not pair)
             return (*operand, sink) if pair else (operand, sink)
         operand = F_.ops.carry_bound(aligned.view(b, -1, h, w), aligned)
         if not pair:
diff --git a/edvr_amd/functional.py b/edvr_amd/functional.py
--- a/edvr_amd/functional.py
+++ b/edvr_amd/functional.py
@@ -150,7 +150,8 @@
     split = 2 * om.shape[1] // 3
     bias = m.bias.detach() if m.bias is not None else None
     xb = ops.input_bound(x) if (ops.F4S_INFERENCE and hint == ops.DCN_HALO_TAPWIN and tapwin_takes(x, m)) else None
-    y = ops.dcnv2_forward(x, om[:, :split], om[:, split:], m.weight.detach(), bias, *cfg, act=act, halo_hint=hint, xm_bound=xb)
+    y = ops.dcnv2_forward(x, om[:, :split], om[:, split:], m.weight.detach(), bias, *cfg, act=act, halo_hint=hint, xm_bound=xb,
+                          w_param=m.weight)
     if ops.F4S_INFERENCE:
         ops.linear_bound(y, m.weight, m.bias, (x,))
     return y
@@ -183,6 +184,23 @@
     return ops.tsa_temporal_pair(emb, emb_ref, aligned)
 
 
+def tsa_front_applies(m_feat, m_attn, emb, emb_ref, aligned):
+    grad = _needs_grad(emb, emb_ref, aligned, m_feat.weight, m_feat.bias, m_attn.weight, m_attn.bias)
+    plain = all(tuple(m.stride) == (1, 1) and tuple(m.padding) == (0, 0) and tuple(m.dilation) == (1, 1) and m.groups == 1 and m.kernel_size[0] == m.kernel_size[1]
+                for m in (m_feat, m_attn))
+    return plain and ops.tsa_front_applies(emb, emb_ref, aligned, m_feat.weight, m_attn.weight, (m_feat.bias is not None, m_attn.bias is not None), grad)
+
+
+def tsa_front(m_feat, m_attn, emb, emb_ref, aligned, act=ACT_LRELU):
+    if tsa_front_applies(m_feat, m_attn, emb, emb_ref, aligned):
+        return ops.tsa_front(emb, emb_ref, aligned, ops.pack_conv_weight(m_feat.weight, f4s=True), m_feat.bias.detach(),
+                             ops.pack_conv_weight(m_attn.weight, f4s=True), m_attn.bias.detach(), m_feat.out_channels, act, act)
+    b, t, c, h, w = aligned.shape
+    mod = tsa_temporal(emb, emb_ref, aligned)
+    mod = ops.carry_bound(mod.view(b, t * c, h, w), mod)
+    return conv(m_feat, mod, act=act), conv(m_attn, mod, act=act)
+
+
 def tsa_combine(feat, attn, attn_add):
     if _needs_grad(feat, attn, attn_add):
         from . import autograd as ag
diff --git a/edvr_amd/ops.py b/edvr_amd/ops.py
--- a/edvr_amd/ops.py
+++ b/edvr_amd/ops.py
@@ -126,6 +126,34 @@
         out = torch.empty(L.edvr_conv2d_packed_weight_elems(co, ci, k), dtype=torch.float32, device=w.device)
         _lib.check(L.edvr_conv2d_pack_weight_f32(_ptr(w), _ptr(out), co, ci, k, 1 if transpose_flip else 0, _stream()),
                    'edvr_conv2d_pack_weight_f32')
+    ent[1][key] = (ver, out, weight.data_ptr())
+    return out
+
+
+def pack_dcn_split_weight(weight):
+    require_gpu(weight)
+    key, wid, ver = ('dcn_split',), id(weight), weight._version
+    ent = _PACKED.get(wid)
+    if ent is not None and ent[0]() is weight:
+        hit = ent[1].get(key)
+        if hit is not None and hit[0] == ver and hit[2] == weight.data_ptr():
+            return hit[1]
+    else:
+        ent = (weakref.ref(weight, lambda _r, wid=wid: _PACKED.pop(wid, None)), {})
+        _PACKED[wid] = ent
+    L = _lib.lib()
+    w = weight.detach()
+    if not w.is_contiguous():
+        w = w.contiguous()
+    co, c = w.shape[0], w.shape[1]
+    n_el = L.edvr_dcnv2_split_packed_weight_elems(co, c)
+    stale = ent[1].get(key)
+    if stale is not None and stale[1].numel() == n_el and stale[1].device == w.device and _sole_owner(stale):
+        out = stale[1]
+    else:
+        out = torch.empty(n_el, dtype=torch.int32, device=w.device)
+    _run('dcn_split_pack_weight', lambda: _lib.check(L.edvr_dcnv2_split_pack_weight_f32(_ptr(w), _ptr(out), co, c, _stream()),
+                                                     'edvr_dcnv2_split_pack_weight_f32'), 0, _nb(w) + 4.0 * n_el)
     ent[1][key] = (ver, out, weight.data_ptr())
     return out
 
@@ -683,7 +711,7 @@
     return t.stride(0) if t.shape[0] > 1 else 0
 
 
-def dcnv2_forward(x, offset, mask, weight, bias, stride, pad, dil, groups, dg, act=ACT_NONE, halo_hint=0, out=None, xm_bound=None):
+def dcnv2_forward(x, offset, mask, weight, bias, stride, pad, dil, groups, dg, act=ACT_NONE, halo_hint=0, out=None, xm_bound=None, w_param=None):
     dt = require_gpu(x, offset, mask, weight, bias, dtypes=tuple(DCN_DTYPES))
     L = _lib.lib()
     if not x.is_contiguous() or not weight.is_contiguous():
@@ -726,7 +754,13 @@
         if L.edvr_dcnv2_fwd_kernel_name(_ptr(x), *dims, int(halo_hint), buf, 64) == 0:
             name = f'dcnv2_fwd[{"dcn_tapwin_split_fwd_kernel" if split else buf.value.decode()}]'
     common = (_ptr(x), _ptr(offset), _ptr(mask), _ptr(weight), _ptr(bias), _ptr(y), *dims, _bstride(offset), _bstride(mask), act, halo_hint, _ptr(ws), nbytes)
-    if split:
+    if split and w_param is not None and w_param.data_ptr() == weight.data_ptr() and w_param.is_contiguous():
+        require_gpu(xm_bound)
+        wq = pack_dcn_split_weight(w_param)
+        launch = lambda: _lib.check(L.edvr_dcnv2_fwd_split_packed_f32(_ptr(x), _ptr(offset), _ptr(mask), _ptr(wq), _ptr(bias), _ptr(y), *dims, _bstride(offset),
+                                                                      _bstride(mask), act, halo_hint, _ptr(xm_bound), _stream()),
+                                    'edvr_dcnv2_fwd_split_packed_f32')
+    elif split:
         require_gpu(xm_bound)
         launch = lambda: _lib.check(L.edvr_dcnv2_fwd_split_f32(*common, _ptr(xm_bound), _stream()), 'edvr_dcnv2_fwd_split_f32')
     else:
@@ -784,6 +818,76 @@
                                        'edvr_tsa_temporal_f32'), 0, _nb(emb, emb_ref, aligned, out, prob))
     carry_bound(out, al_in)
     return (out, prob) if want_prob else out
+
+
+TSA_FRONT = os.environ.get('EDVR_TSA_FRONT', '1') != '0'
+
+
+def set_tsa_front(on=None):
+    global TSA_FRONT
+    prev = TSA_FRONT
+    if on is not None:
+        TSA_FRONT = bool(on)
+    return prev
+
+
+def _emb_ref_planes(emb_ref):
+    return emb_ref if _plane_contig(emb_ref) else emb_ref.contiguous()
+
+
+def tsa_front_applies(emb, emb_ref, aligned, w_feat, w_attn, has_bias=(True, True), needs_grad=False, x_amax=None):
+    if not TSA_FRONT or not F4S_INFERENCE or needs_grad or aligned.dim() != 5 or w_feat.dim() != 4 or w_attn.dim() != 4:
+        return False
+    b, t, c, h, w = aligned.shape
+    if tuple(emb.shape) != (b, t, c, h, w) or tuple(emb_ref.shape) != (b, c, h, w) or w_feat.shape[1] != t * c or w_attn.shape[1] != t * c:
+        return False
+    if x_amax is None and get_bound(aligned) is None:
+        return False
+    any_ptr = ctypes.c_void_p(16)
+    return bool(_lib.lib().edvr_tsa_front_applies(0, b, t, c, h, w, w_feat.shape[0], w_attn.shape[0], w_feat.shape[2], w_attn.shape[2],
+                                                  int(bool(has_bias[0])), int(bool(has_bias[1])), any_ptr, any_ptr, any_ptr))
+
+
+def tsa_front(emb, emb_ref, aligned, wq_feat, bias_feat, wq_attn, bias_attn, co, act_feat=ACT_LRELU, act_attn=ACT_LRELU, x_amax=None,
+              want_y_amax=True):
+    if torch.is_grad_enabled() and any(v.requires_grad for v in (emb, emb_ref, aligned)):
+        raise RuntimeError('tsa_front has no backward: call it under torch.no_grad()')
+    require_gpu(emb, emb_ref, aligned, bias_feat, bias_attn)
+    require_gpu(wq_feat, wq_attn, dtypes=(torch.int32,))
+    b, t, c, h, w = aligned.shape
+    if tuple(emb.shape) != (b, t, c, h, w) or tuple(emb_ref.shape) != (b, c, h, w):
+        raise ValueError(f'tsa_front: emb {tuple(emb.shape)} / emb_ref {tuple(emb_ref.shape)} do not match aligned {tuple(aligned.shape)}')
+    L = _lib.lib()
+    if not L.edvr_tsa_front_supported(b, t, c, h, w, co):
+        raise NotImplementedError(f'tsa_front: the kernel takes t <= 16, c % 8 == 0, co <= 128; got t {t}, c {c}, co {co}')
+    n_el = L.edvr_conv2d_packed_weight_1x1s_elems(co, t * c)
+    if wq_feat.numel() != n_el or wq_attn.numel() != n_el or bias_feat.numel() != co or bias_attn.numel() != co:
+        raise ValueError(f'tsa_front: packed weights of {n_el} dwords and biases of {co} elements expected')
+    al_in = aligned
+    emb, aligned, emb_ref = emb.contiguous(), aligned.contiguous(), _emb_ref_planes(emb_ref)
+    if x_amax is None:
+        x_amax = input_bound(al_in, aligned.view(b * t, c, h, w))
+    require_gpu(x_amax)
+    if BOUND_CHECK:
+        true = amax(aligned.view(b * t, c, h, w)).item()
+        if not (x_amax.item() >= true):
+            raise AssertionError(f'magnitude bound {x_amax.item():.6g} < max |aligned| = {true:.6g} for the TSA head on {tuple(aligned.shape)}')
+        BOUND_CHECK_LOG.extend([((b, t * c, h, w), x_amax.item() / max(true, 1e-30))] * 2)
+    feat = torch.empty(b, co, h, w, dtype=torch.float32, device=aligned.device)
+    attn = torch.empty(b, co, h, w, dtype=torch.float32, device=aligned.device)
+    yb = (_arena(aligned.device).slot(aligned.device), _arena(aligned.device).slot(aligned.device)) if want_y_amax else (None, None)
+    ci = t * c
+    _run('tsa_front_split_kernel',
+         lambda: _lib.check(L.edvr_tsa_front_f32(_ptr(emb), _ptr(emb_ref), _img_stride(emb_ref), _ptr(aligned), _ptr(x_amax),
+                                                 _ptr(wq_feat), _ptr(bias_feat), int(act_feat), _ptr(feat), _ptr(yb[0]),
+                                                 _ptr(wq_attn), _ptr(bias_attn), int(act_attn), _ptr(attn), _ptr(yb[1]),
+                                                 b, t, c, h, w, co, _stream()), 'edvr_tsa_front_f32'),
+         2.0 * b * h * w * (t * c + 2 * co * ci), _nb(emb, emb_ref, aligned, feat, attn) + 8.0 * co * ci,
+         16.0 * b * (-(-h * w // 128) * 128) * (-(-ci // 32) * 32) * (128 if co > 64 else 64))
+    if want_y_amax:
+        set_bound(feat, yb[0])
+        set_bound(attn, yb[1])
+    return feat, attn
 
 
 def tsa_temporal_pair(emb, emb_ref, aligned, out=None, out_rev=None):
diff --git a/include/edvr_amd.h b/include/edvr_amd.h
--- a/include/edvr_amd.h
+++ b/include/edvr_amd.h
@@ -125,6 +125,12 @@
                              const float *xm_amax, edvr_stream_t stream);
 int edvr_dcnv2_fwd_split_applies(const float *x, int B, int C, int H, int W, int Co, int kh, int kw, int stride, int pad, int dil, int groups,
                                  int dg, int halo_hint);
+size_t edvr_dcnv2_split_packed_weight_elems(int Co, int C);
+int edvr_dcnv2_split_pack_weight_f32(const float *weight, void *wpk, int Co, int C, edvr_stream_t stream);
+int edvr_dcnv2_fwd_split_packed_f32(const float *x, const float *offset, const float *mask, const void *wpk, const float *bias,
+                                    float *y, int B, int C, int H, int W, int Co, int kh, int kw, int stride, int pad, int dil, int groups,
+                                    int dg, int64_t offset_bstride, int64_t mask_bstride, int act, int halo_hint, const float *xm_amax,
+                                    edvr_stream_t stream);
 int edvr_dcnv2_fwd_kernel_name(const float *x, int B, int C, int H, int W, int Co, int kh, int kw, int stride, int pad, int dil,
                                int groups, int dg, int halo_hint, char *buf, size_t buf_len);
 
@@ -172,6 +178,13 @@
                           int b, int t, int c, int hw, edvr_stream_t stream);
 int edvr_tsa_temporal_pair_f32(const float *emb, const float *emb_ref, const float *aligned, float *out, float *out_rev,
                                int b, int t, int c, int hw, edvr_stream_t stream);
+int edvr_tsa_front_supported(int b, int t, int c, int h, int w, int co);
+int edvr_tsa_front_applies(int needs_grad, int b, int t, int c, int h, int w, int co_feat, int co_attn, int ks_feat, int ks_attn, int has_bias_feat,
+                           int has_bias_attn, const void *wq_feat, const void *wq_attn, const float *x_amax);
+int edvr_tsa_front_f32(const float *emb, const float *emb_ref, int64_t emb_ref_img_stride, const float *aligned, const float *x_amax,
+                       const void *wq_feat, const float *bias_feat, int act_feat, float *feat, float *feat_amax, const void *wq_attn,
+                       const float *bias_attn, int act_attn, float *attn, float *attn_amax, int b, int t, int c, int h, int w, int co,
+                       edvr_stream_t stream);
 int edvr_pool_maxavg_3x3s2_f32(const float *x, float *y, int n, int c, int h, int w, edvr_stream_t stream);
 int edvr_upsample2x_f32(const float *x, float *y, int nc, int h, int w, float scale, edvr_stream_t stream);
 int edvr_tsa_combine_f32(const float *feat, const float *attn, const float *attn_add, float *y, int64_t numel,
```
